# EthanD11/RS-VIO

Measured on AMD Instinct MI355X. Metric: stereo frames/sec (tracker+BA) on 752×480 EuRoC stream; BA ms/iter at window=10, higher is better.
Workload: dtype f32 (tracker) / f64 (BA)

## Files before the change

### rs-vio_amd/csrc/ba.hip

```cpp
#include <rccl/rccl.h>

#include <algorithm>
#include <chrono>
#include <cmath>
#include <cstdlib>
#include <cstring>
#include <string>
#include <sys/resource.h>
#include <numeric>
#include <stdexcept>
#include <vector>

#include "common.hpp"

#include "obs_pass.hpp"
#include "se3.hpp"
#include "wave.hpp"

#pragma clang fp contract(fast)

namespace rsvio {

namespace {

// ... 292 lines not shown
    __hip_atomic_store(w + 1, (b >> 32) | t, __ATOMIC_RELAXED, __HIP_MEMORY_SCOPE_SYSTEM);
}


__global__ void ba_reset(Geometry G, Work Wk, double lambda0) {
    const int i = blockIdx.x * blockDim.x + threadIdx.x;
    if (i < 7 * G.n_kf) {
        Wk.pose[0][i] = Wk.pose_init[i];
        Wk.pose[1][i] = Wk.pose_init[i];
    }
    if (i < 3 * G.n_lm) {
        Wk.pw[0][i] = Wk.pw_init[i];
        Wk.pw[1][i] = Wk.pw_init[i];
    }
    if (i == 0) {
        Wk.tick[1] = wall_clock64();
        *Wk.singular = 0;
        LmState s{};
        s.lambda = lambda0;
        s.nu = 2.0;
        *Wk.st = s;
    }
}

struct SlotLin {
    double V[6], gp[3], Wr[9], Ur[6], gr[3], cost;
};

__device__ __forceinline__ void slot_linearize(const Geometry& G, const Pose& P, const double p[3], int nobs,
                                               int cams, const double2 (&uvq)[2], bool fr, SlotLin& L) {
#pragma unroll
    for (int i = 0; i < 6; ++i) L.V[i] = 0.0;
#pragma unroll
    for (int i = 0; i < 3; ++i) L.gp[i] = 0.0;
#pragma unroll
    for (int i = 0; i < 9; ++i) L.Wr[i] = 0.0;
#pragma unroll
    for (int i = 0; i < 6; ++i) L.Ur[i] = 0.0;
#pragma unroll
    for (int i = 0; i < 3; ++i) L.gr[i] = 0.0;
    L.cost = 0.0;
#pragma unroll
    for (int o = 0; o < 2; ++o) {
        if (o >= nobs) break;
        double r[2], J[2][9];
        const double uv[2] = {uvq[o].x, uvq[o].y};
        linearize(p, P, G.TCB[(cams >> o) & 1].m, uv, r, J, true);
        double sq = r[0] * r[0] + r[1] * r[1], rho, wt;
        huber(sq, G.huber_delta, &rho, &wt);
        L.cost += 0.5 * rho;
        const double wr0 = wt * r[0], wr1 = wt * r[1];
        int k = 0;
#pragma unroll
        for (int a = 0; a < 3; ++a) {
#pragma unroll
            for (int c = a; c < 3; ++c) L.V[k++] += wt * (J[0][a] * J[0][c] + J[1][a] * J[1][c]);
            L.gp[a] += J[0][a] * wr0 + J[1][a] * wr1;
        }
        if (fr) {
            int u = 0;
#pragma unroll
            for (int a = 0; a < 3; ++a) {
#pragma unroll
                for (int c = 0; c < 3; ++c) L.Wr[a * 3 + c] += wt * (J[0][6 + a] * J[0][c] + J[1][6 + a] * J[1][c]);
#pragma unroll
                for (int c = a; c < 3; ++c) L.Ur[u++] += wt * (J[0][6 + a] * J[0][6 + c] + J[1][6 + a] * J[1][6 + c]);
                L.gr[a] += J[0][6 + a] * wr0 + J[1][6 + a] * wr1;
            }
        }
    }
}

__device__ __forceinline__ void wave_sync() {
    __builtin_amdgcn_fence(__ATOMIC_SEQ_CST, "wavefront");
    __builtin_amdgcn_wave_barrier();
}

template <bool WAVE = false>
__device__ void store_linearization(const Work& Wk, int buf, int s, int lane, bool act, bool fr, int first, int nk,
                                    int l, const SlotLin& L, double (*sh)[64]) {
    if (act && fr) {
        double rec[kRawF];
#pragma unroll
        for (int i = 0; i < 6; ++i) rec[RV + i] = L.V[i];
#pragma unroll
        for (int i = 0; i < 3; ++i) rec[RGP + i] = L.gp[i];
#pragma unroll
        for (int i = 0; i < 9; ++i) rec[RWR + i] = L.Wr[i];
#pragma unroll
        for (int i = 0; i < 6; ++i) rec[RUR + i] = L.Ur[i];
#pragma unroll
        for (int i = 0; i < 3; ++i) rec[RGR + i] = L.gr[i];
        rec[27] = 0.0;
        double2* dst = reinterpret_cast<double2*>(Wk.raws[buf] + (size_t)s * kRawF);
#pragma unroll
        for (int i = 0; i < kRawF / 2; ++i) dst[i] = make_double2(rec[2 * i], rec[2 * i + 1]);
    }
#pragma unroll
    for (int i = 0; i < 6; ++i) sh[i][lane] = L.V[i];
#pragma unroll
    for (int i = 0; i < 3; ++i) sh[6 + i][lane] = L.gp[i];
    if constexpr (WAVE) wave_sync(); else __syncthreads();
    if (act && lane == first) {
        double Vl[6] = {0, 0, 0, 0, 0, 0}, gl[3] = {0, 0, 0};
        for (int k = 0; k < nk; ++k) {
#pragma unroll
            for (int i = 0; i < 6; ++i) Vl[i] += sh[i][first + k];
#pragma unroll
            for (int i = 0; i < 3; ++i) gl[i] += sh[6 + i][first + k];
        }
        double rec[kLmF] = {Vl[0], Vl[1], Vl[2], Vl[3], Vl[4], Vl[5], gl[0], gl[1], gl[2], 0.0, 0.0, 0.0};
        double2* dst = reinterpret_cast<double2*>(Wk.rawl[buf] + (size_t)l * kLmF);
#pragma unroll
        for (int i = 0; i < kLmF / 2; ++i) dst[i] = make_double2(rec[2 * i], rec[2 * i + 1]);
    }
}

__device__ __forceinline__ bool chol_inv3(const double A[3][3], double X[3][3]) {
    const double d0 = A[0][0];
    if (!(d0 > 0.0) || !isfinite(d0)) return false;
    const double l00 = sqrt(d0), l10 = A[1][0] / l00, l20 = A[2][0] / l00;
    const double d1 = A[1][1] - l10 * l10;
    if (!(d1 > 0.0) || !isfinite(d1)) return false;
    const double l11 = sqrt(d1), l21 = (A[2][1] - l20 * l10) / l11;
    const double d2 = (A[2][2] - l20 * l20) - l21 * l21;
    if (!(d2 > 0.0) || !isfinite(d2)) return false;
    const double l22 = sqrt(d2);
    const double m00 = 1.0 / l00, m11 = 1.0 / l11, m22 = 1.0 / l22;
    const double m10 = -(l10 * m00) * m11, m21 = -(l21 * m11) * m22;
    const double m20 = -(l20 * m00 + l21 * m10) * m22;
    X[0][0] = (m00 * m00 + m10 * m10) + m20 * m20;
    X[0][1] = X[1][0] = m10 * m11 + m20 * m21;
    X[0][2] = X[2][0] = m20 * m22;
    X[1][1] = m11 * m11 + m21 * m21;
    X[1][2] = X[2][1] = m21 * m22;
    X[2][2] = m22 * m22;
    return true;
}

__device__ __forceinline__ bool landmark_inverse(const double* Vp, double lambda, double Vi[3][3], int chol) {
    double A[3][3] = {{Vp[0] + lambda, Vp[1], Vp[2]}, {Vp[1], Vp[3] + lambda, Vp[4]}, {Vp[2], Vp[4], Vp[5] + lambda}};
    const bool ok = chol ? chol_inv3(A, Vi) : inv3(A, Vi);
    if (!ok)
#pragma unroll
        for (int a = 0; a < 3; ++a)
#pragma unroll
            for (int c = 0; c < 3; ++c) Vi[a][c] = 0.0;
    return ok;
}

struct SlotSrc {
    const unsigned long long* mask;
    const int* lm_base;
    const int* wave_fill;
    const int* wave_lm;
    const unsigned* key;
    const double2* uv;
    int nb_lm, nb_pad;
    int uv32;
};
constexpr unsigned long long kEvenBits = 0x5555555555555555ull;

__device__ void build_slots_body(const Geometry& G, const Prob& Pr, const SlotSrc& S, int4* hdr, double2* huv,
                                 int b) {
    const int t = threadIdx.x;
    const double2 z2 = make_double2(0.0, 0.0);
    if (b < S.nb_lm) {
        const int l = 256 * b + t;
        if (l >= G.n_lm) return;
        const int base = S.lm_base[l];
        if (base < 0) return;
        const unsigned long long m = S.mask[l];
        unsigned long long kb = (m | (m >> 1)) & kEvenBits;
        const int ns = __popcll(kb);
        for (size_t ps = (size_t)base; kb; kb &= kb - 1, ++ps) {
            const int k = (__ffsll((long long)kb) - 1) >> 1;
            const int c0 = (int)(m >> (2 * k)) & 1, c1 = (int)(m >> (2 * k + 1)) & 1;
            const int no = c0 + c1;
            hdr[2 * ps] = make_int4(k, l, base & 63, ns);
            hdr[2 * ps + 1] = make_int4(Pr.free_idx[k], no, no == 2 ? 2 : c1, 0);
            if (no == 1) huv[2 * ps + 1] = z2;
        }
    } else if (b < S.nb_lm + S.nb_pad) {
        const int ps = 256 * (b - S.nb_lm) + t;
        if (ps >= 64 * G.n_wave || (ps & 63) < S.wave_fill[ps >> 6]) return;
        hdr[2 * (size_t)ps] = make_int4(0, 0, 0, 0);
        hdr[2 * (size_t)ps + 1] = make_int4(-1, 0, 0, 0);
        huv[2 * (size_t)ps] = z2;
        huv[2 * (size_t)ps + 1] = z2;
    } else {
        const int i = 256 * (b - S.nb_lm - S.nb_pad) + t;
        if (i >= G.n_obs) return;
        const unsigned key = S.key[i];
        const int l = (int)(key >> 6), k = (int)(key >> 1) & 31, c = (int)(key & 1);
        const unsigned long long m = S.mask[l];
        const unsigned long long below = ((m | (m >> 1)) & kEvenBits) & ((1ull << (2 * k)) - 1ull);
        const size_t q = (size_t)S.lm_base[l] + __popcll(below);
        const int sub = (c == 1 && ((m >> (2 * k)) & 1)) ? 1 : 0;
        if (S.uv32) {
            const float2 f = reinterpret_cast<const float2*>(S.uv)[i];
            huv[2 * q + sub] = make_double2((double)f.x, (double)f.y);
        } else {
            huv[2 * q + sub] = S.uv[i];
        }
    }
}

constexpr int kPairU = 8;

__device__ void build_pairs_body(const Geometry& G, const Prob& Pr, const SlotSrc& S, int4* pairs, int c) {
    __shared__ int cnt[4];
    const int pb = c / kGrp, x = c % kGrp;
    const int fa = Pr.pb_fa[pb], fb = Pr.pb_fb[pb];
    int kfa = 0, kfb = 0;
    for (int k = 0; k < G.n_kf; ++k) {
        const int f = Pr.free_idx[k];
        if (f == fa) kfa = k;
        if (f == fb) kfb = k;
    }
    const unsigned long long ma = 3ull << (2 * kfa), mb = 3ull << (2 * kfb);
    const unsigned long long below_a = (1ull << (2 * kfa)) - 1ull, below_b = (1ull << (2 * kfb)) - 1ull;
    const int tid = threadIdx.x, lane = tid & 63, wave = tid >> 6;
    const int nw = G.n_wave > x ? (G.n_wave - x + kGrp - 1) / kGrp : 0;
    const int k0 = nw * wave / 4, k1 = nw * (wave + 1) / 4;
    int4* out = pairs + (size_t)c * G.pair_stride;
    struct Round {
        int l0[kPairU], l1[kPairU], lbs[kPairU];
        unsigned long long m[kPairU];
    };
    auto load = [&](int kb, Round& R) {
#pragma unroll
        for (int u = 0; u < kPairU; ++u) {
            const int w = x + kGrp * (kb + u);
            const bool in = kb + u < k1;
            R.l0[u] = in ? S.wave_lm[w] : 0;
            R.l1[u] = in ? S.wave_lm[w + 1] : 0;
        }
#pragma unroll
        for (int u = 0; u < kPairU; ++u) {
            const bool in = R.l0[u] + lane < R.l1[u];
            R.m[u] = in ? S.mask[R.l0[u] + lane] : 0ull;
            R.lbs[u] = in ? S.lm_base[R.l0[u] + lane] : 0;
        }
    };
    auto scan = [&](const Round& R, bool write, int& acc) {
#pragma unroll
        for (int u = 0; u < kPairU; ++u) {
            for (int l = R.l0[u] + lane; l - lane < R.l1[u]; l += 64) {
                const bool first = l == R.l0[u] + lane;
                const unsigned long long mm = first ? R.m[u] : (l < R.l1[u] ? S.mask[l] : 0ull);
                const bool has = (mm & ma) && (mm & mb);
                const unsigned long long bal = __ballot(has);
                if (write && has) {
                    const unsigned long long kbits = (mm | (mm >> 1)) & kEvenBits;
                    const int lb = first ? R.lbs[u] : S.lm_base[l];
                    out[acc + __popcll(bal & ((1ull << lane) - 1ull))] =
                        make_int4(lb + __popcll(kbits & below_a), lb + __popcll(kbits & below_b), l, 0);
                }
                acc += __popcll(bal);
            }
        }
    };
    Round R0;
    load(k0, R0);
    int n = 0;
    scan(R0, false, n);
    for (int kb = k0 + kPairU; kb < k1; kb += kPairU) {
        Round R;
        load(kb, R);
        scan(R, false, n);
    }
    if (lane == 0) cnt[wave] = n;
    __syncthreads();
    int base = 0;
    for (int v = 0; v < wave; ++v) base += cnt[v];
    const int total = cnt[0] + cnt[1] + cnt[2] + cnt[3];
    scan(R0, true, base);
    for (int kb = k0 + kPairU; kb < k1; kb += kPairU) {
        Round R;
        load(kb, R);
        scan(R, true, base);
    }
    for (int i = total + tid; i < G.pair_stride; i += 256) out[i] = make_int4(-1, 0, 0, 0);
}

__global__ __launch_bounds__(256) void ba_stage_in(const uint4* src, uint4* __restrict__ dst, int n_words) {
    const int t = (int)(blockIdx.x * 256 + threadIdx.x), st = (int)(gridDim.x * 256);
    const int i0 = t, i1 = t + st;
    uint4 a, b;
    host_load2x16(src + min(i0, n_words - 1), src + min(i1, n_words - 1), a, b);
    if (i0 < n_words) dst[i0] = a;
    if (i1 < n_words) dst[i1] = b;
}

__global__ __launch_bounds__(256) void ba_build_layout(Geometry G, Prob Pr, SlotSrc S, int nb_slots, int4* hdr,
                                                       double2* huv, int4* pairs) {
    const int b = blockIdx.x;
    if (b < nb_slots)
        build_slots_body(G, Pr, S, hdr, huv, b);
    else
        build_pairs_body(G, Pr, S, pairs, b - nb_slots);
}

__device__ void linearize_body(const Geometry& G, const Prob& Pr, const Work& Wk, int w, int with_reset,
                               double lambda0) {
    __shared__ double sh[10][64];
    const int lane = threadIdx.x;
    const int s = 64 * w + lane;
    if (with_reset) {
        const int nt = G.n_wave * 64;
        for (int i = s; i < 7 * G.n_kf; i += nt) {
            Wk.pose[0][i] = Wk.pose_init[i];
            Wk.pose[1][i] = Wk.pose_init[i];
        }
        for (int i = s; i < 3 * G.n_lm; i += nt) {
            Wk.pw[0][i] = Wk.pw_init[i];
            Wk.pw[1][i] = Wk.pw_init[i];
        }
        if (s == 0) {
            Wk.tick[1] = wall_clock64();
            *Wk.singular = 0;
            LmState st{};
            st.lambda = lambda0;
            st.nu = 2.0;
            *Wk.st = st;
        }
    }
    const double* pose0 = with_reset ? Wk.pose_init : Wk.pose[0];
    const double* pw0 = with_reset ? Wk.pw_init : Wk.pw[0];
    const int4 h0 = Pr.slot_hdr[2 * s], h1 = Pr.slot_hdr[2 * s + 1];
    const double2 uvq[2] = {Pr.slot_uv[2 * s], Pr.slot_uv[2 * s + 1]};
    STAMP(11);
    const bool act = h1.y > 0;
    const int kf = h0.x, l = h0.y, first = act ? h0.z : lane, nk = act ? h0.w : 1;
    const bool fr = h1.x >= 0;
    SlotLin L;
    if (act) {
        const Pose P = pose_from7(pose0 + 7 * kf);
        const double* pwp = pw0 + 3 * l;
        const double p[3] = {pwp[0], pwp[1], pwp[2]};
        slot_linearize(G, P, p, h1.y, h1.z, uvq, fr, L);
    } else {
        const Pose P{};
        const double p[3] = {0.0, 0.0, 1.0};
        slot_linearize(G, P, p, 0, 0, uvq, false, L);
    }
    STAMP(12);
    store_linearization(Wk, 0, s, lane, act, fr, first, nk, l, L, sh);
    const double c = wave_sum_det(L.cost);
    if (lane == 0) {
        Wk.partA[w * kPartA] = c;
        Wk.partA[w * kPartA + 1] = 0.0;
    }
    STAMP(14);
}

__global__ __launch_bounds__(64) void ba_linearize(Geometry G, Prob Pr, Work Wk, double lambda0) {
    linearize_body(G, Pr, Wk, blockIdx.x, 1, lambda0);
}

__device__ void trial_scalars_wave(const Geometry& G, const Prob& Pr, const Work& Wk, const LmState& s,
                                   int include_poses, double out[4]) {
    const int lane = threadIdx.x & 63;
    constexpr int kU = 8;
    double4 pv[kU];
    const int wl = max(G.n_wave - 1, 0), el = 7 * G.n_kf - 1;
#pragma unroll
    for (int k = 0; k < kU; ++k)
        pv[k] = *reinterpret_cast<const double4*>(Wk.partD + (size_t)min(lane + 64 * k, wl) * kPartD);
    double p0[3], p1[3];
    int fi[3];
#pragma unroll
    for (int k = 0; k < 3; ++k) {
        const int e = min(lane + 64 * k, el);
        fi[k] = Pr.free_idx[e / 7];
        p0[k] = Wk.pose[0][e];
        p1[k] = Wk.pose[1][e];
    }
#pragma unroll
    for (int k = 0; k < kU; ++k)
        if (lane + 64 * k >= G.n_wave) pv[k] = make_double4(0.0, 0.0, 0.0, 0.0);
    bool fr[3];
#pragma unroll
    for (int k = 0; k < 3; ++k) fr[k] = include_poses && lane + 64 * k <= el && fi[k] >= 0;
    double acc[kPartD] = {0.0, 0.0, 0.0, 0.0};
#pragma unroll
    for (int k = 0; k < kU; ++k) {
        acc[0] += pv[k].x;
        acc[1] += pv[k].y;
        acc[2] += pv[k].z;
        acc[3] += pv[k].w;
    }
    for (int i = lane + 64 * kU; i < G.n_wave; i += 64) {
        const double4 v = *reinterpret_cast<const double4*>(Wk.partD + (size_t)i * kPartD);
        acc[0] += v.x;
        acc[1] += v.y;
        acc[2] += v.z;
        acc[3] += v.w;
    }
    double sq[2] = {0.0, 0.0};
#pragma unroll
    for (int k = 0; k < 3; ++k)
        if (fr[k]) {
            sq[0] += p0[k] * p0[k];
            sq[1] += p1[k] * p1[k];
        }
    if (!s.solve_ok)
#pragma unroll
        for (int k = 0; k < kPartD; ++k) acc[k] = 0.0;
    acc[3] += sq[s.cur];
#pragma unroll
    for (int k = 0; k < kPartD; ++k) out[k] = wave_sum_det(acc[k]);
}

__device__ void trial_scalars_p2p(const Geometry& G, const Prob& Pr, const Work& Wk, const LmState& s, const P2P& P,
                                  unsigned long long gen, int* err, double out[4]) {
    const int lane = threadIdx.x & 63, par = (int)(gen & 1);
    double* own = P.peer[P.rank];
    const int el = 7 * G.n_kf - 1;
    double p0[3], p1[3];
    int fi[3];
#pragma unroll
    for (int k = 0; k < 3; ++k) {
        const int e = min(lane + 64 * k, el);
        fi[k] = Pr.free_idx[e / 7];
        p0[k] = Wk.pose[0][e];
        p1[k] = Wk.pose[1][e];
    }
    double sq[2] = {0.0, 0.0};
#pragma unroll
    for (int k = 0; k < 3; ++k)
        if (lane + 64 * k <= el && fi[k] >= 0) {
            sq[0] += p0[k] * p0[k];
            sq[1] += p1[k] * p1[k];
        }
    for (int j = 0; j < 4; ++j) out[j] = 0.0;
    bool late = false;
    for (int r = 0; r < P.nranks; ++r) {
        const int nw = P.xnw[r];
        double acc[kPartD] = {0.0, 0.0, 0.0, 0.0};
        for (int w = lane; w < max(nw, 512); w += 64) {
            double4 v = make_double4(0.0, 0.0, 0.0, 0.0);
            if (w < nw) {
                const unsigned long long* f = p2p_tflag(own, par, r, w);
                long long spins = 0;
                while (__hip_atomic_load(f, __ATOMIC_RELAXED, __HIP_MEMORY_SCOPE_SYSTEM) < gen) {
                    __builtin_amdgcn_s_sleep(1);
                    if (++spins > (1ll << 25)) {
                        late = true;
                        break;
                    }
                }
                __builtin_amdgcn_fence(__ATOMIC_ACQUIRE, "");
                const double* q = p2p_tval(own, par, r, w);
                v.x = __hip_atomic_load(q, __ATOMIC_RELAXED, __HIP_MEMORY_SCOPE_SYSTEM);
                v.y = __hip_atomic_load(q + 1, __ATOMIC_RELAXED, __HIP_MEMORY_SCOPE_SYSTEM);
                v.z = __hip_atomic_load(q + 2, __ATOMIC_RELAXED, __HIP_MEMORY_SCOPE_SYSTEM);
                v.w = __hip_atomic_load(q + 3, __ATOMIC_RELAXED, __HIP_MEMORY_SCOPE_SYSTEM);
            }
            acc[0] += v.x;
            acc[1] += v.y;
            acc[2] += v.z;
            acc[3] += v.w;
        }
        if (r == 0) acc[3] += sq[s.cur];
#pragma unroll
        for (int k = 0; k < kPartD; ++k) out[k] += wave_sum_det(acc[k]);
    }
    if (late) atomicExch(err, 1);
}

__device__ void lm_update(LmState& s, double cost, const double tv[4], int max_iter, double cost_tol,
                          double param_tol) {
    if (s.iter == 0) s.initial_cost = cost;
    s.cost = cost;
    s.iter += 1;
    s.accepted = 0;
    if (!isfinite(cost)) {
        s.status = RSVIO_LM_NUMERICAL_FAILURE;
        s.done = 1;
    } else if (!s.solve_ok) {
        s.status = RSVIO_LM_LINEAR_SOLVE_FAILED;
        s.done = 1;
    } else {
        s.new_cost = tv[0];
        s.dp2 = tv[1];
        s.gpdp = tv[2];
        s.x2 = tv[3];
        const double dx2 = s.dc2 + s.dp2;
        const double dxn = sqrt(dx2), xn = sqrt(s.x2);
        if (dxn <= param_tol * (xn + param_tol)) {
            s.status = RSVIO_LM_PARAMETER_TOLERANCE;
            s.done = 1;
        } else {
            const double pred = 0.5 * (s.lambda * dx2 - (s.gcdc + s.gpdp));
            const double dcost = cost - s.new_cost;
            const double rho = dcost / pred;
            if (isfinite(s.new_cost) && fabs(dcost) <= cost_tol * cost) {
                s.status = RSVIO_LM_COST_TOLERANCE;
                s.done = 1;
            } else if (isfinite(s.new_cost) && rho > 0.0) {
                s.accepted = 1;
                s.cur = 1 - s.cur;
                const double f = 2.0 * rho - 1.0;
                s.lambda *= fmax(1.0 / 3.0, 1.0 - f * f * f);
                s.nu = 2.0;
                s.cost = s.new_cost;
            } else {
                s.lambda *= s.nu;
                s.nu *= 2.0;
                if (s.lambda > 1e32) {
                    s.status = RSVIO_LM_TRUST_REGION;
                    s.done = 1;
                }
            }
        }
    }
    if (!s.done && s.iter >= max_iter) {
        s.status = RSVIO_LM_MAX_ITERATIONS;
        s.done = 1;
    }
}

struct LmArgs {
    int max_iter;
    double cost_tol, param_tol;
};

__device__ LmState lm_decide(const Geometry& G, const Prob& Pr, const Work& Wk, const LmState* src, int pre_reduced,
                             const LmArgs& la, const P2P* PP = nullptr, const unsigned long long* xgen = nullptr,
                             int* err = nullptr) {
    LmState s = *src;
    double tv[4];
    if (pre_reduced == 4) {
        const int lane = threadIdx.x & 63, r = lane >> 2, i = lane & 3, nr = PP->nranks;
        const unsigned long long gen = *xgen;
        const unsigned g32 = (unsigned)gen;
        const unsigned long long* wv = p2p_ll(PP->peer[PP->rank], (int)(gen & 1), min(r, nr - 1)) + 2 * i;
        unsigned long long a = __hip_atomic_load(wv, __ATOMIC_RELAXED, __HIP_MEMORY_SCOPE_SYSTEM);
        unsigned long long b = __hip_atomic_load(wv + 1, __ATOMIC_RELAXED, __HIP_MEMORY_SCOPE_SYSTEM);
        for (int k = 0; k < 4; ++k) tv[k] = 0.0;
        if (s.pending && !s.done && s.solve_ok) {
            long long spins = 0;
            bool late = false;
            while (r < nr && !((unsigned)(a >> 32) == g32 && (unsigned)(b >> 32) == g32)) {
                if (++spins > (1ll << 25)) {
                    late = true;
                    break;
                }
                __builtin_amdgcn_s_sleep(1);
                a = __hip_atomic_load(wv, __ATOMIC_RELAXED, __HIP_MEMORY_SCOPE_SYSTEM);
                b = __hip_atomic_load(wv + 1, __ATOMIC_RELAXED, __HIP_MEMORY_SCOPE_SYSTEM);
            }
            if (late) atomicExch(err, 1);
            const double got = late ? 0.0 : __longlong_as_double((long long)((a & 0xffffffffull) | (b << 32)));
            for (int k = 0; k < 4; ++k) {
                double v = 0.0;
                for (int q = 0; q < nr; ++q) v += rl64(got, 4 * q + k);
                tv[k] = v;
            }
        }
    } else if (pre_reduced == 2) {
        const unsigned long long gen = *xgen;
        for (int k = 0; k < 4; ++k) tv[k] = 0.0;
        if (s.pending && !s.done && s.solve_ok) trial_scalars_p2p(G, Pr, Wk, s, *PP, gen, err, tv);
    } else if (pre_reduced) {
        for (int k = 0; k < 4; ++k) tv[k] = Wk.trial4[k];
    } else {
        trial_scalars_wave(G, Pr, Wk, s, 1, tv);
    }
    const double cost0 = Wk.sys[(size_t)G.n_pb * 36 + 12 * G.n_free];
    __asm__ volatile("" ::"v"(tv[0]), "v"(tv[1]), "v"(tv[2]), "v"(tv[3]), "v"(cost0));
    STAMP(29);
    if (s.pending && !s.done) {
        const double cost = s.iter == 0 ? cost0 : s.cost;
        lm_update(s, cost, tv, la.max_iter, la.cost_tol, la.param_tol);
        s.pending = 0;
    }
    return s;
}

__device__ __forceinline__ void slot_w(const double* rec, double W[18]) {
    const double* v = rec + RV;
    const double Vs[9] = {v[0], v[1], v[2], v[1], v[3], v[4], v[2], v[4], v[5]};
#pragma unroll
    for (int i = 0; i < 9; ++i) W[i] = Vs[i];
#pragma unroll
    for (int i = 0; i < 9; ++i) W[9 + i] = rec[RWR + i];
}

template <bool DIAG>
__device__ __forceinline__ void schur_pair(const Work& Wk, int cur, double lambda, int chol, int sa, int sb, int l,
                                           double (&acc)[kBlockF]) {
    const double2* ra = reinterpret_cast<const double2*>(Wk.raws[cur] + (size_t)sa * kRawF);
    const double2* rb = reinterpret_cast<const double2*>(Wk.raws[cur] + (size_t)sb * kRawF);
    const double2* rl = reinterpret_cast<const double2*>(Wk.rawl[cur] + (size_t)l * kLmF);
    constexpr int NA = DIAG ? kRawF / 2 : 9;
    double Ra[2 * NA], Rb[18], Lm[10];
#pragma unroll
    for (int i = 0; i < NA; ++i) {
        const double2 x = ra[i];
        Ra[2 * i] = x.x; Ra[2 * i + 1] = x.y;
    }
    if constexpr (!DIAG)
#pragma unroll
        for (int i = 0; i < 9; ++i) {
            const double2 y = rb[i];
            Rb[2 * i] = y.x; Rb[2 * i + 1] = y.y;
        }
#pragma unroll
    for (int i = 0; i < 5; ++i) {
        const double2 x = rl[i];
        Lm[2 * i] = x.x; Lm[2 * i + 1] = x.y;
    }
    double Wa[18], Wb[18];
    slot_w(Ra, Wa);
    if constexpr (DIAG) {
#pragma unroll
        for (int i = 0; i < 18; ++i) Wb[i] = Wa[i];
    } else {
        slot_w(Rb, Wb);
    }
    double Vi[3][3];
    if (!landmark_inverse(Lm + LV, lambda, Vi, chol)) *Wk.singular = 1;
    double Ya[18];
#pragma unroll
    for (int a = 0; a < 6; ++a)
#pragma unroll
        for (int k = 0; k < 3; ++k)
            Ya[a * 3 + k] = fma(Wa[a * 3 + 2], Vi[2][k], fma(Wa[a * 3 + 1], Vi[1][k], Wa[a * 3] * Vi[0][k]));
#pragma unroll
    for (int a = 0; a < 6; ++a)
#pragma unroll
        for (int k = 0; k < 6; ++k)
            acc[a * 6 + k] -= fma(Ya[a * 3 + 2], Wb[k * 3 + 2], fma(Ya[a * 3 + 1], Wb[k * 3 + 1], Ya[a * 3] * Wb[k * 3]));
    if constexpr (DIAG) {
        double U[36];
#pragma unroll
        for (int a = 0; a < 3; ++a)
#pragma unroll
            for (int c = 0; c < 3; ++c) {
                U[a * 6 + c] = Wa[a * 3 + c];
                U[(3 + a) * 6 + c] = Wa[(3 + a) * 3 + c];
                U[c * 6 + 3 + a] = Wa[(3 + a) * 3 + c];
            }
        const double* ur = Ra + RUR;
        const double Ur[9] = {ur[0], ur[1], ur[2], ur[1], ur[3], ur[4], ur[2], ur[4], ur[5]};
#pragma unroll
        for (int a = 0; a < 3; ++a)
#pragma unroll
            for (int c = 0; c < 3; ++c) U[(3 + a) * 6 + 3 + c] = Ur[a * 3 + c];
#pragma unroll
        for (int i = 0; i < 36; ++i) acc[i] += U[i];
#pragma unroll
        for (int a = 0; a < 6; ++a) {
            const double gca = a < 3 ? Ra[RGP + a] : Ra[RGR + a - 3];
            const double yg = fma(Ya[a * 3 + 2], Lm[LG + 2], fma(Ya[a * 3 + 1], Lm[LG + 1], Ya[a * 3] * Lm[LG]));
            acc[36 + a] += yg - gca;
            acc[42 + a] += gca;
        }
    }
}

template <bool DIAG>
__device__ __forceinline__ void schur_chunk_pairs(const Geometry& G, const Work& Wk, const LmState& s, const int4* pr,
                                                  int4 p1, int tid, double (&acc)[kBlockF]) {
    if (p1.x >= 0) schur_pair<DIAG>(Wk, s.cur, s.lambda, G.chol, p1.x, p1.y, p1.z, acc);
    for (int p = tid + kSchurThreads; p < G.pair_stride; p += kSchurThreads) {
        const int4 q = pr[p];
        if (q.x >= 0) schur_pair<DIAG>(Wk, s.cur, s.lambda, G.chol, q.x, q.y, q.z, acc);
    }
}

__device__ void schur_chunks_body(const Geometry& G, const Prob& Pr, const Work& Wk, const LmArgs& la,
                                  int pre_reduced, int c, const P2P* PP = nullptr,
                                  const unsigned long long* xgen = nullptr, int* err = nullptr) {
    __shared__ double red[kSchurThreads / 64][kBlockF];
    const int tid = threadIdx.x, lane = tid & 63, wave = tid >> 6;
    const int pb = c / kGrp, x = c % kGrp;
    RTSTAMP(0);
    STAMP(26);
    if (G.env_on) {
        int a = 0, r = pb;
        while (a < G.n_free && r >= G.n_free - a) {
            r -= G.n_free - a;
            ++a;
        }
        if (a < G.n_free && a + r > (int)G.env[a]) {
            if (tid < 36) Wk.cpart[(size_t)x * sys_len(G) + pb * 36 + tid] = 0.0;
            return;
        }
    }
    const int4* pr = Pr.pairs + (size_t)c * G.pair_stride;
    const int4 p1 = tid < G.pair_stride ? pr[tid] : make_int4(-1, 0, 0, 0);
    const int fa = Pr.pb_fa[pb];
    const bool diag = fa == Pr.pb_fb[pb];
    __shared__ LmState sd;
    STAMP(27);
    if (wave == 0) {
        const LmState d = lm_decide(G, Pr, Wk, Wk.st_prev, pre_reduced, la, PP, xgen, err);
        STAMP(28);
        if (lane == 0) {
            sd = d;
            if (c == 0) *Wk.st = d;
        }
    }
    __syncthreads();
    const LmState s = sd;
    if (s.done) return;
    STAMP(16);
    RTSTAMP(1);
    double acc[kBlockF];
#pragma unroll
    for (int i = 0; i < kBlockF; ++i) acc[i] = 0.0;
    if (diag)
        schur_chunk_pairs<true>(G, Wk, s, pr, p1, tid, acc);
    else
        schur_chunk_pairs<false>(G, Wk, s, pr, p1, tid, acc);
    STAMP(17);
    wave_reduce_scatter<3>(acc, lane);
    if ((lane & 3) == 0)
#pragma unroll
        for (int j = 0; j < 3; ++j) red[wave][3 * (lane >> 2) + j] = acc[j];
    __syncthreads();
    if (tid < (diag ? kBlockF : 36)) {
        double v = red[0][tid];
#pragma unroll
        for (int w = 1; w < kSchurThreads / 64; ++w) v += red[w][tid];
        const int SB0 = G.n_pb * 36, SG0 = SB0 + 6 * G.n_free;
        const int e = tid < 36 ? pb * 36 + tid : (tid < 42 ? SB0 + 6 * fa + tid - 36 : SG0 + 6 * fa + tid - 42);
        Wk.cpart[(size_t)x * sys_len(G) + e] = v;
    }
    STAMP(18);
    RTSTAMP(2);
}

__global__ __launch_bounds__(kSchurThreads) void ba_schur_chunks(Geometry G, Prob Pr, Work Wk, LmArgs la,
                                                                  int pre_reduced) {
    schur_chunks_body(G, Pr, Wk, la, pre_reduced, blockIdx.x);
}

__global__ __launch_bounds__(kSchurThreads) void ba_schur_chunks_p2p(Geometry G, Prob Pr, Work Wk, LmArgs la, P2P P,
                                                                      const unsigned long long* xgen, int* err,
                                                                      int mode) {
    schur_chunks_body(G, Pr, Wk, la, mode, blockIdx.x, &P, xgen, err);
}

template <int T>
__device__ void combine_system(const Geometry& G, const Prob& Pr, const Work& Wk, double* dst, double lambda,
                               bool add_lambda) {
    const int n_e = G.n_pb * 36 + 12 * G.n_free;
    const size_t L = sys_len(G);
    constexpr int kU = 16;
    const int lane = threadIdx.x;
    double pa[kU];
    int sing = 0;
    if (lane < 64) {
#pragma unroll
        for (int k = 0; k < kU; ++k) pa[k] = lane + 64 * k < G.n_wave ? Wk.partA[(lane + 64 * k) * kPartA] : 0.0;
        sing = *Wk.singular;
    }
    constexpr int kE = 8;
    for (int e0 = 0; e0 < n_e; e0 += T * kE) {
        double v[kE][kGrp];
#pragma unroll
        for (int i = 0; i < kE; ++i) {
            const int e = e0 + threadIdx.x + T * i;
#pragma unroll
            for (int x = 0; x < kGrp; ++x) v[i][x] = e < n_e ? Wk.cpart[(size_t)x * L + e] : 0.0;
        }
#pragma unroll
        for (int i = 0; i < kE; ++i) {
            const int e = e0 + threadIdx.x + T * i;
            if (e >= n_e) break;
            double a = v[i][0];
#pragma unroll
            for (int x = 1; x < kGrp; ++x) a += v[i][x];
            dst[e] = a;
        }
    }
    if (add_lambda) {
        __syncthreads();
        for (int t = threadIdx.x; t < 6 * G.n_free; t += T) {
            const int f = t / 6, k = t % 6;
            dst[(f * G.n_free - f * (f - 1) / 2) * 36 + 7 * k] += lambda;
        }
    }
    if (lane < 64) {
        double c = 0.0;
#pragma unroll
        for (int k = 0; k < kU; ++k) c += pa[k];
        for (int w = lane + 64 * kU; w < G.n_wave; w += 64) c += Wk.partA[w * kPartA];
        c = wave_sum_det(c);
        if (lane == 0) {
            dst[n_e] = c;
            dst[n_e + 1] = sing ? 1.0 : 0.0;
            Wk.sys[n_e] = c;
        }
    }
}

__global__ __launch_bounds__(256) void ba_schur_combine(Geometry G, Prob Pr, Work Wk, int lambda_owner) {
    const LmState* st = Wk.st;
    if (st->done) return;
    STAMP(19);
    combine_system<256>(G, Pr, Wk, Wk.sys, st->lambda, lambda_owner != 0);
    __syncthreads();
    if (threadIdx.x == 0) *Wk.singular = 0;
}

__global__ __launch_bounds__(256) void ba_schur_combine_wide(Geometry G, Prob Pr, Work Wk) {
    const LmState* st = Wk.st;
    if (st->done) return;
    const int n_e = G.n_pb * 36 + 12 * G.n_free;
    const size_t L = sys_len(G);
    const int e = blockIdx.x * 256 + threadIdx.x;
    constexpr int kU = 16;
    const int lane = threadIdx.x;
    double pa[kU];
    int sing = 0;
    if (blockIdx.x == 0 && lane < 64) {
#pragma unroll
        for (int k = 0; k < kU; ++k) pa[k] = lane + 64 * k < G.n_wave ? Wk.partA[(lane + 64 * k) * kPartA] : 0.0;
        sing = *Wk.singular;
    }
    const double lambda = st->lambda;
    if (e < n_e) {
        double v[kGrp];
#pragma unroll
        for (int x = 0; x < kGrp; ++x) v[x] = Wk.cpart[(size_t)x * L + e];
        double a = v[0];
#pragma unroll
        for (int x = 1; x < kGrp; ++x) a += v[x];
        const int pb = e / 36, k = e % 36;
        if (pb < G.n_pb && k % 7 == 0 && Pr.pb_fa[pb] == Pr.pb_fb[pb]) a += lambda;
        Wk.sys[e] = a;
    }
    if (blockIdx.x == 0 && lane < 64) {
        double c = 0.0;
#pragma unroll
        for (int k = 0; k < kU; ++k) c += pa[k];
        for (int w = lane + 64 * kU; w < G.n_wave; w += 64) c += Wk.partA[w * kPartA];
        c = wave_sum_det(c);
        if (lane == 0) {
            Wk.sys[n_e] = c;
            Wk.sys[n_e + 1] = sing ? 1.0 : 0.0;
        }
    }
}





constexpr int kLcLd = 65;

template <int NP, int CW, int WV, int K>
__device__ __forceinline__ void chol_pipe_step(double (&a)[CW], int lane, double* Lc, double* Uc, int* progress,
                                               int& seen, bool& bad, double inv, double (&uq)[CW], double lp) {
    constexpr int c0 = WV * CW;
    constexpr int c1 = (c0 + CW < NP) ? c0 + CW : NP;
    constexpr int KN = (K + 1 < c0) ? K + 2 : K + 1;
    if constexpr (K < c0) {
        if (seen < KN) {
            do {
                seen = __hip_atomic_load(progress, __ATOMIC_ACQUIRE, __HIP_MEMORY_SCOPE_WORKGROUP);
                if (seen >= KN) break;
                __builtin_amdgcn_s_sleep(1);
            } while (true);
        }
        const double lr = Lc[K * kLcLd + lane];
        const double* u = Uc + K * kLcLd;
        if constexpr (KN == K + 2) {
            const double lr2 = Lc[(K + 1) * kLcLd + lane];
            const double* u2 = Uc + (K + 1) * kLcLd;
            double v1[CW], v2[CW];
#pragma unroll
            for (int jj = 0; jj < CW; ++jj) {
                v1[jj] = u[c0 + jj];
                v2[jj] = u2[c0 + jj];
            }
#pragma unroll
            for (int jj = 0; jj < CW; ++jj)
                if (c0 + jj < NP) a[jj] = fma(-lr2, v2[jj], fma(-lr, v1[jj], a[jj]));
        } else {
#pragma unroll
            for (int jj = 0; jj < CW; ++jj)
                if (c0 + jj < NP) a[jj] = fma(-lr, u[c0 + jj], a[jj]);
        }
        if constexpr (KN == c0) {
            const double piv = rl64(a[0], c0);
            bad |= !(piv > 0.0) || !isfinite(piv);
            inv = rcp_f64(piv);
        }
    } else if constexpr (K < c1) {
        constexpr int j = K - c0;
#ifdef RSVIO_STAMPS
        if (K == c0 && lane == 0) g_dbg[28 + WV] = (unsigned long long)clock64();
#endif
        if constexpr (K > c0) {
            __asm__ volatile("" ::: "memory");
            __hip_atomic_store(progress, K, __ATOMIC_RELAXED, __HIP_MEMORY_SCOPE_WORKGROUP);
        }
        const double uk = a[j];
        const double l = uk * inv;
        a[j] = l;
        Lc[K * kLcLd + lane] = l;
        Uc[K * kLcLd + lane] = uk;
        double piv = 1.0;
        if constexpr (j + 1 < CW && K + 1 < NP) {
            a[j + 1] = fma(-l, rl64(uk, K + 1), a[j + 1]);
            piv = rl64(a[j + 1], K + 1);
        }
        if constexpr (j + 2 < CW && K + 2 < NP) a[j + 2] = fma(-l, rl64(uk, K + 2), a[j + 2]);
        if constexpr (j + 1 < CW && K + 1 < NP) {
            bad |= !(piv > 0.0) || !isfinite(piv);
            inv = rcp_f64(piv);
        }
        __builtin_amdgcn_sched_barrier(0);
        if constexpr (K > c0) {
#pragma unroll
            for (int jj = j + 2; jj < CW; ++jj)
                if (c0 + jj < NP) a[jj] = fma(-lp, uq[jj], a[jj]);
        }
        {
            const double* uK = Uc + K * kLcLd;
#pragma unroll
            for (int jj = j + 3; jj < CW; ++jj) uq[jj] = c0 + jj < NP ? uK[c0 + jj] : 0.0;
        }
        lp = l;
        if constexpr (K + 1 == c1) {
            __asm__ volatile("" ::: "memory");
            __hip_atomic_store(progress, K + 1, __ATOMIC_RELAXED, __HIP_MEMORY_SCOPE_WORKGROUP);
        }
    }
    if constexpr (K < c0) {
#pragma unroll
        for (int jj = 0; jj < CW; ++jj) __asm__ volatile("" : "+v"(a[jj]));
    }
    constexpr int KNEXT = (K < c0) ? KN : K + 1;
    if constexpr (KNEXT < c1) chol_pipe_step<NP, CW, WV, KNEXT>(a, lane, Lc, Uc, progress, seen, bad, inv, uq, lp);
}

template <int NF>
__device__ __forceinline__ const double* sys_lower(const double* sys, int r, int c) {
    constexpr int n = 6 * NF;
    if (r == n) return sys + (NF * (NF + 1) / 2) * 36 + c;
    const int a = c / 6, b = r / 6;
    const int pb = a * NF - a * (a - 1) / 2 + (b - a);
    const int k = (a == b) ? (r % 6) * 6 + (c % 6) : (c % 6) * 6 + (r % 6);
    return sys + pb * 36 + k;
}

template <int NP, int CW, int WV>
__device__ void chol_pipe(const double* sys, double* Lc, double* Uc, int* progress, int* badw, int lane) {
    constexpr int c0 = WV * CW;
    double a[CW];
#pragma unroll
    for (int jj = 0; jj < CW; ++jj) {
        const int c = c0 + jj;
        a[jj] = (c < NP && lane <= NP && (c <= lane || lane == NP)) ? *sys_lower<NP / 6>(sys, lane, c) : 0.0;
    }
    bool bad = false;
    if constexpr (c0 < NP) {
        double inv = 0.0;
        if constexpr (c0 == 0) {
            const double piv = rl64(a[0], 0);
            bad = !(piv > 0.0) || !isfinite(piv);
            inv = rcp_f64(piv);
        }
        int seen = 0;
        double uq[CW];
#pragma unroll
        for (int jj = 0; jj < CW; ++jj) uq[jj] = 0.0;
        chol_pipe_step<NP, CW, WV, 0>(a, lane, Lc, Uc, progress, seen, bad, inv, uq, 0.0);
    }
    if (lane == 0) badw[WV] = bad ? 1 : 0;
#ifdef RSVIO_STAMPS
    if (lane == 0) g_dbg[24 + WV] = (unsigned long long)clock64();
#endif
}

__device__ __forceinline__ void k5_result(LmState* st, int ok, double d2, double gd) {
    st->solve_ok = ok;
    st->dc2 = d2;
    st->gcdc = gd;
    st->pending = 1;
}

template <int NF>
__device__ void k5_finish(const Geometry& G, const Work& Wk, double* A, double x, double gcl_v, int n, int lane,
                          const double (&p7)[7], int fidx) {
    LmState* st = Wk.st;
    const double d2 = wave_sum_det(x * x);
    const double gd = wave_sum_det(lane < n ? gcl_v * x : 0.0);
    __builtin_amdgcn_wave_barrier();
    if (lane < n) {
        Wk.dc[lane] = x;
        A[lane] = x;
    }
    __builtin_amdgcn_s_waitcnt(0xc07f);
    __builtin_amdgcn_wave_barrier();
    STAMP(4);
    if (lane < G.n_kf) {
        double* q = Wk.pose[1 - st->cur] + 7 * lane;
        if (fidx < 0) {
#pragma unroll
            for (int i = 0; i < 7; ++i) q[i] = p7[i];
        } else {
            double qv[7];
            se3_plus(p7, A + 6 * fidx, qv);
#pragma unroll
            for (int i = 0; i < 7; ++i) q[i] = qv[i];
        }
    }
    STAMP(5);
    if (lane == 0) k5_result(st, 1, d2, gd);
    STAMP(6);
}

template <int NF>
__device__ void camera_solve_w4(const Geometry& G, const Prob& Pr, const Work& Wk, const double* sys, double* A,
                                int* badw, int* progress, int n, int tid, const double (&p7)[7], int fidx) {
    constexpr int NP = 6 * NF, CW = (NP + 3) / 4;
    const int lane = tid & 63, wave = tid >> 6;
    LmState* st = Wk.st;
    const double gcl_v = (wave == 0 && lane < n) ? sys[(NF * (NF + 1) / 2) * 36 + 6 * NF + lane] : 0.0;
    double* Lc = A + 128;
    double* Uc = Lc + NP * kLcLd;
    switch (wave) {
        case 0: chol_pipe<NP, CW, 0>(sys, Lc, Uc, progress, badw, lane); break;
        case 1: chol_pipe<NP, CW, 1>(sys, Lc, Uc, progress, badw, lane); break;
        case 2: chol_pipe<NP, CW, 2>(sys, Lc, Uc, progress, badw, lane); break;
        default: chol_pipe<NP, CW, 3>(sys, Lc, Uc, progress, badw, lane); break;
    }
    __syncthreads();
    if (wave != 0) return;
    if (badw[0] | badw[1] | badw[2] | badw[3]) {
        if (lane == 0) k5_result(st, 0, 0.0, 0.0);
        return;
    }
// ... 1057 lines not shown
    double x[2];
#pragma unroll
    for (int q = 0; q < 2; ++q) x[q] = lane + 64 * q < n ? yv[q] : 0.0;
    const double d2 = wave_sum_det(x[0] * x[0] + x[1] * x[1]);
    const double gd = wave_sum_det(gcl[0] * x[0] + gcl[1] * x[1]);
#pragma unroll
    for (int q = 0; q < 2; ++q) {
        const int i = lane + 64 * q;
        if (i < n) {
            Wk.dc[i] = x[q];
            dcs[i] = x[q];
        }
    }
    __builtin_amdgcn_s_waitcnt(0xc07f);
    __builtin_amdgcn_wave_barrier();
    if (lane < G.n_kf) {
        double* qd = Wk.pose[1 - cur] + 7 * lane;
        if (fidx < 0) {
#pragma unroll
            for (int i = 0; i < 7; ++i) qd[i] = p7[i];
        } else {
            double qv[7];
            se3_plus(p7, dcs + 6 * fidx, qv);
#pragma unroll
            for (int i = 0; i < 7; ++i) qd[i] = qv[i];
        }
    }
    if (lane == 0) k5_result(st, 1, d2, gd);
    STAMP(5);
}

template <int NF>
__global__ __launch_bounds__(64 * kBkWaves) void ba_camera_solve_blk(Geometry G, Prob Pr, Work Wk, int combine) {
    camera_solve_blk_body<NF>(G, Pr, Wk, combine);
}

constexpr int kX2Waves = 8;
constexpr int kUcLd = kMaxN + 1;

__device__ __forceinline__ const double* sys_lower_rt(const double* sys, int nf, int r, int c) {
    const int n = 6 * nf;
    if (r == n) return sys + (nf * (nf + 1) / 2) * 36 + c;
    const int a = c / 6, b = r / 6;
    const int pb = a * nf - a * (a - 1) / 2 + (b - a);
    const int k = (a == b) ? (r % 6) * 6 + (c % 6) : (c % 6) * 6 + (r % 6);
    return sys + pb * 36 + k;
}

template <int NP, int CW, int WV, int K>
__device__ __forceinline__ void chol2_step(double (&a)[2][CW], int lane, double* Uc, double* dinv, double* sink,
                                           int* progress, int& seen, bool& bad, double inv) {
    constexpr int c0 = WV * CW;
    constexpr int c1 = (c0 + CW < NP) ? c0 + CW : NP;
    constexpr int Q0 = (c0 < 64) ? 0 : 1;
    constexpr int KN = (K + 1 < c0) ? K + 2 : K + 1;
    if constexpr (K < c0) {
        if (seen < KN) {
            do {
                seen = __hip_atomic_load(progress, __ATOMIC_ACQUIRE, __HIP_MEMORY_SCOPE_WORKGROUP);
                if (seen >= KN) break;
                __builtin_amdgcn_s_sleep(1);
            } while (true);
        }
        const double* u = Uc + K * kUcLd;
        const double di = dinv[K];
        double lr[2];
#pragma unroll
        for (int q = Q0; q < 2; ++q) lr[q] = u[min(lane + 64 * q, NP)] * di;
        if constexpr (KN == K + 2) {
            const double* u2 = Uc + (K + 1) * kUcLd;
            const double di2 = dinv[K + 1];
            double lr2[2];
#pragma unroll
            for (int q = Q0; q < 2; ++q) lr2[q] = u2[min(lane + 64 * q, NP)] * di2;
            double v1[CW], v2[CW];
#pragma unroll
            for (int jj = 0; jj < CW; ++jj) {
                v1[jj] = u[c0 + jj];
                v2[jj] = u2[c0 + jj];
            }
#pragma unroll
            for (int q = Q0; q < 2; ++q)
#pragma unroll
                for (int jj = 0; jj < CW; ++jj)
                    if (c0 + jj < NP) a[q][jj] = fma(-lr2[q], v2[jj], fma(-lr[q], v1[jj], a[q][jj]));
        } else {
#pragma unroll
            for (int q = Q0; q < 2; ++q)
#pragma unroll
                for (int jj = 0; jj < CW; ++jj)
                    if (c0 + jj < NP) a[q][jj] = fma(-lr[q], u[c0 + jj], a[q][jj]);
        }
        if constexpr (KN == c0) {
            const double piv = rl64(a[c0 >> 6][0], c0 & 63);
            bad |= !(piv > 0.0) || !isfinite(piv);
            inv = rcp_f64(piv);
        }
    } else if constexpr (K < c1) {
        constexpr int j = K - c0;
        if constexpr (K > c0) __hip_atomic_store(progress, K, __ATOMIC_RELEASE, __HIP_MEMORY_SCOPE_WORKGROUP);
        double uk[2], l[2];
#pragma unroll
        for (int q = Q0; q < 2; ++q) {
            uk[q] = a[q][j];
            l[q] = uk[q] * inv;
            a[q][j] = l[q];
            double* dst = (q == 0 || lane + 64 <= NP) ? Uc + K * kUcLd + lane + 64 * q : sink + lane;
            *dst = uk[q];
        }
        dinv[K] = inv;
        double piv = 1.0;
        if constexpr (j + 1 < CW && K + 1 < NP) {
            constexpr int qn = (K + 1) >> 6, ln = (K + 1) & 63;
            const double ukn = rl64(uk[qn], ln);
#pragma unroll
            for (int q = Q0; q < 2; ++q) a[q][j + 1] = fma(-l[q], ukn, a[q][j + 1]);
            piv = rl64(a[qn][j + 1], ln);
        }
#pragma unroll
        for (int jj = j + 2; jj < CW; ++jj) {
            if (c0 + jj < NP) {
                const double v = rl64(uk[(c0 + jj) >> 6], (c0 + jj) & 63);
#pragma unroll
                for (int q = Q0; q < 2; ++q) a[q][jj] = fma(-l[q], v, a[q][jj]);
            }
        }
        if constexpr (j + 1 < CW && K + 1 < NP) {
            bad |= !(piv > 0.0) || !isfinite(piv);
            inv = rcp_f64(piv);
        }
        if constexpr (K + 1 == c1) __hip_atomic_store(progress, K + 1, __ATOMIC_RELEASE, __HIP_MEMORY_SCOPE_WORKGROUP);
    }
    if constexpr (K < c0) {
#pragma unroll
        for (int q = Q0; q < 2; ++q)
#pragma unroll
            for (int jj = 0; jj < CW; ++jj) __asm__ volatile("" : "+v"(a[q][jj]));
    }
    constexpr int KNEXT = (K < c0) ? KN : K + 1;
    if constexpr (KNEXT < c1) chol2_step<NP, CW, WV, KNEXT>(a, lane, Uc, dinv, sink, progress, seen, bad, inv);
}

template <int NP, int CW, int WV>
__device__ __forceinline__ void chol2_pipe(const double* sys, int nf, double* Uc, double* dinv, double* sink, int* progress,
                                           int* badw, int lane) {
    constexpr int c0 = WV * CW;
    constexpr int Q0 = (c0 < 64) ? 0 : 1;
    const int n = 6 * nf;
    double a[2][CW];
#pragma unroll
    for (int q = 0; q < 2; ++q) {
        const int r = lane + 64 * q;
#pragma unroll
        for (int jj = 0; jj < CW; ++jj) {
            const int c = c0 + jj;
            double v = 0.0;
            if (q >= Q0 && c < NP && r <= NP && (c <= r || r == NP)) {
                if (r == NP) v = c < n ? *sys_lower_rt(sys, nf, n, c) : 0.0;
                else if (r < n) v = *sys_lower_rt(sys, nf, r, c);
                else v = (r == c) ? 1.0 : 0.0;
            }
            a[q][jj] = v;
        }
    }
    bool bad = false;
    if constexpr (c0 < NP) {
        double inv = 0.0;
        if constexpr (c0 == 0) {
            const double piv = rl64(a[0][0], 0);
            bad = !(piv > 0.0) || !isfinite(piv);
            inv = rcp_f64(piv);
        }
        int seen = 0;
        chol2_step<NP, CW, WV, 0>(a, lane, Uc, dinv, sink + 64 * WV, progress, seen, bad, inv);
    }
    if (lane == 0) badw[WV] = bad ? 1 : 0;
}

template <int NF>
__global__ __launch_bounds__(64 * kX2Waves) void ba_camera_solve_x2(Geometry G, Prob Pr, Work Wk, int combine) {
    constexpr int NP = 6 * NF, CW = (NP + kX2Waves - 1) / kX2Waves;
    static_assert(NP <= kMaxN && NP + 1 <= kUcLd && NP < 128, "padded system too large");
    __shared__ double Uc[NP * kUcLd];
    __shared__ double dinv[NP];
    __shared__ double dcs[128];
    __shared__ double sink[64 * kX2Waves];
    __shared__ int badw[kX2Waves];
    __shared__ int progress;
    __shared__ int fail;
    LmState* st = Wk.st;
    if (st->done) return;
    const int tid = threadIdx.x, lane = tid & 63, wave = tid >> 6;
    const int nF = G.n_free, n = 6 * nF;
    const double* sys = Wk.sys;
    const int SG0 = G.n_pb * 36 + 6 * nF, SC0 = SG0 + 6 * nF;
    const int cur = st->cur;
    double p7[7] = {0, 0, 0, 1, 0, 0, 0};
    int fidx = -1;
    double gcl[2] = {0.0, 0.0};
    if (wave == 0 && lane < G.n_kf) {
        fidx = Pr.free_idx[lane];
#pragma unroll
        for (int i = 0; i < 7; ++i) p7[i] = Wk.pose[cur][7 * lane + i];
    }
    if (combine) {
        combine_system<64 * kX2Waves>(G, Pr, Wk, Wk.sys, st->lambda, true);
        __builtin_amdgcn_s_waitcnt(0);
        __syncthreads();
    }
    if (wave == 0)
#pragma unroll
        for (int q = 0; q < 2; ++q)
            if (lane + 64 * q < n) gcl[q] = sys[SG0 + lane + 64 * q];
    if (tid == 0) {
        fail = (sys[SC0 + 1] != 0.0 || *Wk.singular) ? 1 : 0;
        *Wk.singular = 0;
        progress = 0;
    }
    __syncthreads();
    if (fail) {
        if (tid == 0) k5_result(st, 0, 0.0, 0.0);
        return;
    }
    switch (wave) {
        case 0: chol2_pipe<NP, CW, 0>(sys, nF, Uc, dinv, sink, &progress, badw, lane); break;
        case 1: chol2_pipe<NP, CW, 1>(sys, nF, Uc, dinv, sink, &progress, badw, lane); break;
        case 2: chol2_pipe<NP, CW, 2>(sys, nF, Uc, dinv, sink, &progress, badw, lane); break;
        case 3: chol2_pipe<NP, CW, 3>(sys, nF, Uc, dinv, sink, &progress, badw, lane); break;
        case 4: chol2_pipe<NP, CW, 4>(sys, nF, Uc, dinv, sink, &progress, badw, lane); break;
        case 5: chol2_pipe<NP, CW, 5>(sys, nF, Uc, dinv, sink, &progress, badw, lane); break;
        case 6: chol2_pipe<NP, CW, 6>(sys, nF, Uc, dinv, sink, &progress, badw, lane); break;
        default: chol2_pipe<NP, CW, 7>(sys, nF, Uc, dinv, sink, &progress, badw, lane); break;
    }
    __syncthreads();
    if (wave != 0) return;
    bool anybad = false;
#pragma unroll
    for (int w = 0; w < kX2Waves; ++w) anybad |= badw[w] != 0;
    if (anybad) {
        if (lane == 0) k5_result(st, 0, 0.0, 0.0);
        return;
    }
    double yv[2], di[2];
#pragma unroll
    for (int q = 0; q < 2; ++q) {
        const int i = min(lane + 64 * q, NP - 1);
        di[q] = dinv[i];
        yv[q] = Uc[i * kUcLd + NP] * di[q];
    }
    constexpr int kBs = 8;
    for (int j0 = n - 1; j0 >= 0; j0 -= kBs) {
        double lt[kBs][2];
#pragma unroll
        for (int t = 0; t < kBs; ++t) {
            const int j = max(j0 - t, 0);
#pragma unroll
            for (int q = 0; q < 2; ++q) lt[t][q] = Uc[min(lane + 64 * q, NP - 1) * kUcLd + j];
        }
#pragma unroll
        for (int t = 0; t < kBs; ++t) {
            const int j = j0 - t;
            if (j < 0) break;
            const double xj = j >= 64 ? rl64(yv[1], j - 64) : rl64(yv[0], j);
#pragma unroll
            for (int q = 0; q < 2; ++q) {
                const double l = lt[t][q] * di[q];
                const double upd = fma(-l, xj, yv[q]);
                yv[q] = lane + 64 * q < j ? upd : yv[q];
            }
        }
    }
    STAMP(4);
    double x[2];
#pragma unroll
    for (int q = 0; q < 2; ++q) x[q] = lane + 64 * q < n ? yv[q] : 0.0;
    const double d2 = wave_sum_det(x[0] * x[0] + x[1] * x[1]);
    const double gd = wave_sum_det(gcl[0] * x[0] + gcl[1] * x[1]);
#pragma unroll
    for (int q = 0; q < 2; ++q) {
        const int i = lane + 64 * q;
        if (i < n) {
            Wk.dc[i] = x[q];
            dcs[i] = x[q];
        }
    }
    __builtin_amdgcn_s_waitcnt(0xc07f);
    __builtin_amdgcn_wave_barrier();
    if (lane < G.n_kf) {
        double* qd = Wk.pose[1 - st->cur] + 7 * lane;
        if (fidx < 0) {
#pragma unroll
            for (int i = 0; i < 7; ++i) qd[i] = p7[i];
        } else {
            double qv[7];
            se3_plus(p7, dcs + 6 * fidx, qv);
#pragma unroll
            for (int i = 0; i < 7; ++i) qd[i] = qv[i];
        }
    }
    if (lane == 0) k5_result(st, 1, d2, gd);
    STAMP(5);
}

template <bool FUSED>
__device__ void k6_body(const Geometry& G, const Prob& Pr, const Work& Wk, int w, int lane, double (*sh)[64],
                        double (*shp)[64], double (*shs)[64], const P2P* PP = nullptr,
                        unsigned long long gen = 0, unsigned long long* k6tag = nullptr,
                        unsigned long long* k6part = nullptr) {
    const int s = 64 * w + lane;
    const int4 h0 = Pr.slot_hdr[2 * s], h1 = Pr.slot_hdr[2 * s + 1];
    const double2 uvq[2] = {Pr.slot_uv[2 * s], Pr.slot_uv[2 * s + 1]};
    const LmState* st = Wk.st;
    const bool act = h1.y > 0;
    const int kf = h0.x, l = h0.y, first = act ? h0.z : lane, nk = act ? h0.w : 1;
    const bool fr = h1.x >= 0;
    const int kfc = act ? kf : 0, lc = act ? l : 0, fc = (act && fr) ? h1.x : 0;
    double recb[2][18], Lmb[2][10], pcb[2][3], p7b[2][7], d6[6];
#pragma unroll
    for (int b = 0; b < 2; ++b) {
        const double2* wr = reinterpret_cast<const double2*>(Wk.raws[b] + (size_t)s * kRawF);
#pragma unroll
        for (int i = 0; i < 9; ++i) {
            const double2 x = wr[i];
            recb[b][2 * i] = x.x; recb[b][2 * i + 1] = x.y;
        }
        const double2* lr = reinterpret_cast<const double2*>(Wk.rawl[b] + (size_t)lc * kLmF);
#pragma unroll
        for (int i = 0; i < 5; ++i) {
            const double2 x = lr[i];
            Lmb[b][2 * i] = x.x; Lmb[b][2 * i + 1] = x.y;
        }
#pragma unroll
        for (int i = 0; i < 3; ++i) pcb[b][i] = Wk.pw[b][3 * lc + i];
#pragma unroll
        for (int i = 0; i < 7; ++i) p7b[b][i] = Wk.pose[b][7 * kfc + i];
    }
#pragma unroll
    for (int i = 0; i < 6; ++i) d6[i] = Wk.dc[6 * fc + i];
    const int done = st->done, solve_ok = st->solve_ok, cur = st->cur;
    const double lambda = st->lambda;
#pragma unroll
    for (int b = 0; b < 2; ++b) {
#pragma unroll
        for (int i = 0; i < 18; ++i) __asm__ volatile("" ::"v"(recb[b][i]));
#pragma unroll
        for (int i = 0; i < 10; ++i) __asm__ volatile("" ::"v"(Lmb[b][i]));
#pragma unroll
        for (int i = 0; i < 3; ++i) __asm__ volatile("" ::"v"(pcb[b][i]));
#pragma unroll
        for (int i = 0; i < 7; ++i) __asm__ volatile("" ::"v"(p7b[b][i]));
    }
    if (done || !solve_ok) return;
    STAMP(20);
    RTSTAMP(7);
    double Wv[18], Lm[10], pc[3], p7[7];
    {
        double rec[18];
#pragma unroll
        for (int i = 0; i < 18; ++i) rec[i] = cur ? recb[1][i] : recb[0][i];
        slot_w(rec, Wv);
#pragma unroll
        for (int i = 0; i < 10; ++i) Lm[i] = cur ? Lmb[1][i] : Lmb[0][i];
#pragma unroll
        for (int i = 0; i < 3; ++i) pc[i] = cur ? pcb[1][i] : pcb[0][i];
#pragma unroll
        for (int i = 0; i < 7; ++i) p7[i] = cur ? p7b[0][i] : p7b[1][i];
    }
    double t3[3] = {0.0, 0.0, 0.0};
    if (act && fr) {
#pragma unroll
        for (int c = 0; c < 3; ++c) {
            double acc = 0.0;
#pragma unroll
            for (int a = 0; a < 6; ++a) acc += Wv[a * 3 + c] * d6[a];
            t3[c] = acc;
        }
    }
#pragma unroll
    for (int c = 0; c < 3; ++c) sh[c][lane] = t3[c];
#pragma unroll
    for (int i = 0; i < 4; ++i) shs[i][lane] = 0.0;
    if constexpr (FUSED) wave_sync(); else __syncthreads();
    STAMP(22);
    if (act && lane == first) {
        double Vi[3][3];
        landmark_inverse(Lm + LV, lambda, Vi, G.chol);
        double rhs[3] = {-Lm[LG], -Lm[LG + 1], -Lm[LG + 2]};
        for (int k = 0; k < nk; ++k)
#pragma unroll
            for (int c = 0; c < 3; ++c) rhs[c] -= sh[c][first + k];
        double* pt = Wk.pw[1 - cur] + 3 * l;
        double dp2 = 0.0, gpdp = 0.0, p2 = 0.0;
#pragma unroll
        for (int c = 0; c < 3; ++c) {
            const double dp = (Vi[c][0] * rhs[0] + Vi[c][1] * rhs[1]) + Vi[c][2] * rhs[2];
            const double p = pc[c];
            const double q = p + dp;
            shp[c][lane] = q;
            pt[c] = q;
            dp2 += dp * dp;
            gpdp += Lm[LG + c] * dp;
            p2 += p * p;
        }
        shs[1][lane] = dp2;
        shs[2][lane] = gpdp;
        shs[3][lane] = p2;
    }
    if constexpr (FUSED) wave_sync(); else __syncthreads();
    STAMP(23);
    SlotLin L;
    if (act) {
        const Pose P = pose_from7(p7);
        const double q[3] = {shp[0][first], shp[1][first], shp[2][first]};
        slot_linearize(G, P, q, h1.y, h1.z, uvq, fr, L);
    } else {
        const Pose P{};
        const double q[3] = {0.0, 0.0, 1.0};
        slot_linearize(G, P, q, 0, 0, uvq, false, L);
    }
    shs[0][lane] = L.cost;
    if constexpr (FUSED) wave_sync(); else __syncthreads();
    STAMP(24);
    store_linearization<FUSED>(Wk, 1 - cur, s, lane, act, fr, first, nk, l, L, sh);
    STAMP(25);
    {
        double v[kPartD];
#pragma unroll
        for (int i = 0; i < kPartD; ++i) v[i] = wave_sum_det(shs[i][lane]);
        if (lane == 0)
#pragma unroll
            for (int i = 0; i < kPartD; ++i) Wk.partD[w * kPartD + i] = v[i];
        if (k6tag && lane < kPartD) {
            double vl = v[0];
#pragma unroll
            for (int i = 1; i < kPartD; ++i) vl = lane == i ? v[i] : vl;
            const unsigned long long b = (unsigned long long)__double_as_longlong(vl), t = gen << 32;
            const size_t nw = (size_t)G.n_wave;
            __hip_atomic_store(k6tag + (2 * lane) * nw + w, (b & 0xffffffffull) | t, __ATOMIC_RELAXED,
                               __HIP_MEMORY_SCOPE_AGENT);
            __hip_atomic_store(k6tag + (2 * lane + 1) * nw + w, (b >> 32) | t, __ATOMIC_RELAXED,
                               __HIP_MEMORY_SCOPE_AGENT);
        }
        if (k6part && lane < kPartD) {
            double vl = v[0];
#pragma unroll
            for (int i = 1; i < kPartD; ++i) vl = lane == i ? v[i] : vl;
            __hip_atomic_store(k6part + (size_t)w * kPartD + lane, (unsigned long long)__double_as_longlong(vl),
                               __ATOMIC_RELAXED, __HIP_MEMORY_SCOPE_AGENT);
        }
        if (PP && lane < PP->nranks) {
            const int par = (int)(gen & 1);
            double* q = p2p_tval(PP->peer[lane], par, PP->rank, w);
            q[0] = v[0]; q[1] = v[1]; q[2] = v[2]; q[3] = v[3];
            __threadfence_system();
            __hip_atomic_store(p2p_tflag(PP->peer[lane], par, PP->rank, w), gen, __ATOMIC_RELEASE,
                               __HIP_MEMORY_SCOPE_SYSTEM);
        }
    }
    STAMP(21);
    RTSTAMP(8);
}

__global__ __launch_bounds__(64) void ba_backsub_relinearize(Geometry G, Prob Pr, Work Wk) {
    __shared__ double sh[10][64];
    __shared__ double shp[3][64];
    __shared__ double shs[4][64];
    RTSTAMP(6);
    k6_body<false>(G, Pr, Wk, blockIdx.x, threadIdx.x, sh, shp, shs);
    RTSTAMP(9);
}

__global__ __launch_bounds__(64) void ba_backsub_relinearize_p2p(Geometry G, Prob Pr, Work Wk, P2P P,
                                                                 const unsigned long long* xgen) {
    __shared__ double sh[10][64];
    __shared__ double shp[3][64];
    __shared__ double shs[4][64];
    unsigned long long gen = *xgen;
    __asm__ volatile("" : "+s"(gen));
    k6_body<false>(G, Pr, Wk, blockIdx.x, threadIdx.x, sh, shp, shs, &P, gen);
}

template <int KU>
__device__ void k6_reduce_p2p(const Geometry& G, const Prob& Pr, const Work& Wk, const P2P& P,
                              unsigned long long* xgen, int* err, const unsigned long long* k6tag) {
    const int lane = threadIdx.x & 63;
    const LmState s = *Wk.st;
    const unsigned long long gen = *xgen + 1;
    if (s.done) return;
    const unsigned g32 = (unsigned)gen;
    const int nr = P.nranks, me = P.rank, par = (int)(gen & 1);
    const int el = 7 * G.n_kf - 1;
    double p0[3], p1[3];
    int fi[3];
#pragma unroll
    for (int k = 0; k < 3; ++k) {
        const int e = min(lane + 64 * k, el);
        fi[k] = Pr.free_idx[e / 7];
        p0[k] = Wk.pose[0][e];
        p1[k] = Wk.pose[1][e];
    }
    constexpr int kU = KU;
    double acc[kPartD] = {0.0, 0.0, 0.0, 0.0};
    bool late = false;
    if (s.solve_ok) {
        for (int i0 = 0; i0 < max(G.n_wave, 64 * kU); i0 += 64 * kU) {
            unsigned long long wd[kU][kPartD][2];
            unsigned pend = 0;
#pragma unroll
            for (int k = 0; k < kU; ++k)
                if (i0 + lane + 64 * k < G.n_wave) pend |= 1u << k;
            long long spins = 0;
            const size_t nw = (size_t)G.n_wave;
            for (;;) {
#pragma unroll
                for (int k = 0; k < kU; ++k)
                    if (pend & (1u << k)) {
                        const unsigned long long* a = k6tag + (i0 + lane + 64 * k);
#pragma unroll
                        for (int j = 0; j < kPartD; ++j) {
                            wd[k][j][0] = __hip_atomic_load(a + (2 * j) * nw, __ATOMIC_RELAXED, __HIP_MEMORY_SCOPE_AGENT);
                            wd[k][j][1] = __hip_atomic_load(a + (2 * j + 1) * nw, __ATOMIC_RELAXED, __HIP_MEMORY_SCOPE_AGENT);
                        }
                    }
#pragma unroll
                for (int k = 0; k < kU; ++k)
                    if (pend & (1u << k)) {
                        bool ok = true;
#pragma unroll
                        for (int j = 0; j < kPartD; ++j)
                            ok &= (unsigned)(wd[k][j][0] >> 32) == g32 && (unsigned)(wd[k][j][1] >> 32) == g32;
                        if (ok) pend &= ~(1u << k);
                    }
                if (__all(pend == 0)) break;
                if (++spins > (1ll << 25)) {
                    late = true;
                    break;
                }
                __builtin_amdgcn_s_sleep(1);
            }
#pragma unroll
            for (int k = 0; k < kU; ++k)
                if (i0 + lane + 64 * k < G.n_wave)
#pragma unroll
                    for (int j = 0; j < kPartD; ++j)
                        acc[j] += __longlong_as_double((long long)((wd[k][j][0] & 0xffffffffull) | (wd[k][j][1] << 32)));
        }
    }
    double sq[2] = {0.0, 0.0};
#pragma unroll
    for (int k = 0; k < 3; ++k)
        if (me == 0 && lane + 64 * k <= el && fi[k] >= 0) {
            sq[0] += p0[k] * p0[k];
            sq[1] += p1[k] * p1[k];
        }
    acc[3] += sq[s.cur];
    double out[kPartD];
#pragma unroll
    for (int k = 0; k < kPartD; ++k) out[k] = wave_sum_det(acc[k]);
    const int r = lane >> 2, i = lane & 3;
    double mv = out[0];
#pragma unroll
    for (int k = 1; k < kPartD; ++k) mv = i == k ? out[k] : mv;
    double got = mv;
    if (r < nr && r != me) {
        ll_put(p2p_ll(P.peer[r], par, me) + 2 * i, mv, g32);
        const unsigned long long* w = p2p_ll(P.peer[me], par, r) + 2 * i;
        long long spins = 0;
        for (;;) {
            const unsigned long long a = __hip_atomic_load(w, __ATOMIC_RELAXED, __HIP_MEMORY_SCOPE_SYSTEM);
            const unsigned long long b = __hip_atomic_load(w + 1, __ATOMIC_RELAXED, __HIP_MEMORY_SCOPE_SYSTEM);
            if ((unsigned)(a >> 32) == g32 && (unsigned)(b >> 32) == g32) {
                got = __longlong_as_double((long long)((a & 0xffffffffull) | (b << 32)));
                break;
            }
            if (++spins > (1ll << 25)) {
                late = true;
                got = 0.0;
                break;
            }
            __builtin_amdgcn_s_sleep(1);
        }
    }
    if (late) atomicExch(err, 1);
    double v4[kPartD];
#pragma unroll
    for (int k = 0; k < kPartD; ++k) {
        double v = 0.0;
        for (int q = 0; q < nr; ++q) v += rl64(got, 4 * q + k);
        v4[k] = v;
    }
    if (lane == 0) {
#pragma unroll
        for (int k = 0; k < kPartD; ++k) Wk.trial4[k] = v4[k];
        *xgen = gen;
    }
}

__global__ __launch_bounds__(64) void ba_backsub_relinearize_p2p3(Geometry G, Prob Pr, Work Wk, P2P P,
                                                                  unsigned long long* xgen, int* err,
                                                                  unsigned long long* k6tag) {
    __shared__ double sh[10][64];
    __shared__ double shp[3][64];
    __shared__ double shs[4][64];
    if ((int)blockIdx.x == G.n_wave) {
        if (G.n_wave <= 256)
            k6_reduce_p2p<4>(G, Pr, Wk, P, xgen, err, k6tag);
        else
            k6_reduce_p2p<8>(G, Pr, Wk, P, xgen, err, k6tag);
        return;
    }
    unsigned long long gen = *xgen + 1;
    __asm__ volatile("" : "+s"(gen));
    k6_body<false>(G, Pr, Wk, blockIdx.x, threadIdx.x, sh, shp, shs, nullptr, gen, k6tag);
}

__device__ void k6_last_push(const Geometry& G, const Prob& Pr, const Work& Wk, const P2P& P,
                             unsigned long long* xgen, unsigned long long gen, const unsigned long long* k6part,
                             const LmState& s) {
    const int lane = threadIdx.x & 63;
    constexpr int kU = 8;
    const int wl = max(G.n_wave - 1, 0), el = 7 * G.n_kf - 1;
    unsigned long long pw[kU][kPartD];
#pragma unroll
    for (int k = 0; k < kU; ++k)
#pragma unroll
        for (int j = 0; j < kPartD; ++j)
            pw[k][j] = __hip_atomic_load(k6part + (size_t)min(lane + 64 * k, wl) * kPartD + j, __ATOMIC_RELAXED,
                                         __HIP_MEMORY_SCOPE_AGENT);
    double p0[3], p1[3];
    int fi[3];
#pragma unroll
    for (int k = 0; k < 3; ++k) {
        const int e = min(lane + 64 * k, el);
        fi[k] = Pr.free_idx[e / 7];
        p0[k] = Wk.pose[0][e];
        p1[k] = Wk.pose[1][e];
    }
    double acc[kPartD] = {0.0, 0.0, 0.0, 0.0};
#pragma unroll
    for (int k = 0; k < kU; ++k)
#pragma unroll
        for (int j = 0; j < kPartD; ++j)
            acc[j] += lane + 64 * k < G.n_wave ? __longlong_as_double((long long)pw[k][j]) : 0.0;
    for (int i = lane + 64 * kU; i < G.n_wave; i += 64)
#pragma unroll
        for (int j = 0; j < kPartD; ++j)
            acc[j] += __longlong_as_double((long long)__hip_atomic_load(k6part + (size_t)i * kPartD + j, __ATOMIC_RELAXED,
                                                                        __HIP_MEMORY_SCOPE_AGENT));
    double sq[2] = {0.0, 0.0};
#pragma unroll
    for (int k = 0; k < 3; ++k)
        if (P.rank == 0 && lane + 64 * k <= el && fi[k] >= 0) {
            sq[0] += p0[k] * p0[k];
            sq[1] += p1[k] * p1[k];
        }
    acc[3] += sq[s.cur];
    double out[kPartD];
#pragma unroll
    for (int k = 0; k < kPartD; ++k) out[k] = wave_sum_det(acc[k]);
    const int r = lane >> 2, i = lane & 3, par = (int)(gen & 1);
    double mv = out[0];
#pragma unroll
    for (int k = 1; k < kPartD; ++k) mv = i == k ? out[k] : mv;
    if (r < P.nranks) ll_put(p2p_ll(P.peer[r], par, P.rank) + 2 * i, mv, (unsigned)gen);
    if (lane == 0) *xgen = gen;
}

__global__ __launch_bounds__(64) void ba_backsub_relinearize_p2p4(Geometry G, Prob Pr, Work Wk, P2P P,
                                                                  unsigned long long* xgen, unsigned* k6cnt,
                                                                  unsigned long long* k6part) {
    __shared__ double sh[10][64];
    __shared__ double shp[3][64];
    __shared__ double shs[4][64];
    unsigned long long gen = *xgen + 1;
    __asm__ volatile("" : "+s"(gen));
    if (G.n_wave > 0) {
        k6_body<false>(G, Pr, Wk, blockIdx.x, threadIdx.x, sh, shp, shs, nullptr, gen, nullptr, k6part);
        const LmState s = *Wk.st;
        if (s.done || !s.solve_ok) return;
        __builtin_amdgcn_s_waitcnt(kWaitStores);
        __builtin_amdgcn_fence(__ATOMIC_RELEASE, "agent");
        unsigned t = 0;
        if (threadIdx.x == 0) t = __hip_atomic_fetch_add(k6cnt, 1u, __ATOMIC_ACQ_REL, __HIP_MEMORY_SCOPE_AGENT);
        t = __builtin_amdgcn_readfirstlane(t);
        if (t != (unsigned)G.n_wave - 1) return;
        __builtin_amdgcn_fence(__ATOMIC_ACQUIRE, "agent");
        if (threadIdx.x == 0) __hip_atomic_store(k6cnt, 0u, __ATOMIC_RELAXED, __HIP_MEMORY_SCOPE_AGENT);
        k6_last_push(G, Pr, Wk, P, xgen, gen, k6part, s);
    } else {
        const LmState s = *Wk.st;
        if (s.done || !s.solve_ok) return;
        k6_last_push(G, Pr, Wk, P, xgen, gen, k6part, s);
    }
}

__global__ __launch_bounds__(64) void ba_reduce_trial(Geometry G, Prob Pr, Work Wk, int include_poses) {
    const LmState s = *Wk.st;
    if (s.done) return;
    double v[4];
    trial_scalars_wave(G, Pr, Wk, s, include_poses, v);
    if (threadIdx.x == 0)
        for (int k = 0; k < 4; ++k) Wk.trial4[k] = v[k];
}

constexpr int kK7Threads = 256;
#ifndef RSVIO_K7_BLOCKS
#define RSVIO_K7_BLOCKS 16
#endif
constexpr int kK7Blocks = RSVIO_K7_BLOCKS;
__device__ __forceinline__ void lm_decide_body(const Geometry& G, const Prob& Pr, const Work& Wk, int pre_reduced,
                                               const LmArgs& la, LmState* host, unsigned long long* htick,
                                               double* hout, const P2P* PP = nullptr,
                                               const unsigned long long* xgen = nullptr, int* err = nullptr) {
    STAMP(8);
    __shared__ LmState sd;
    if (threadIdx.x < 64) {
        const LmState d = lm_decide(G, Pr, Wk, Wk.st_prev, pre_reduced, la, PP, xgen, err);
        if (threadIdx.x == 0) {
            sd = d;
            if (blockIdx.x == 0) {
                LmState h = d;
                h.p2p_err = Wk.p2p_err ? *Wk.p2p_err : 0;
                *Wk.st = d;
                *host = h;
            }
        }
    }
    __syncthreads();
    const LmState s = sd;
    if (hout && s.done) {
        const double* pose = Wk.pose[s.cur];
        const double* pw = Wk.pw[s.cur];
        const int np = 7 * G.n_kf, n = np + 3 * G.n_lm;
        const int per = (((n + (int)gridDim.x - 1) / (int)gridDim.x) + 1) & ~1;
        const int i0 = (int)blockIdx.x * per, i1 = min(n, i0 + per);
        for (int i = i0 + 2 * (int)threadIdx.x; i < i1; i += 2 * kK7Threads) {
            const double a = i < np ? pose[i] : pw[i - np];
            if (i + 1 < i1) {
                const double b = i + 1 < np ? pose[i + 1] : pw[i + 1 - np];
                *reinterpret_cast<double2*>(hout + i) = make_double2(a, b);
            } else {
                hout[i] = a;
            }
        }
        __threadfence_system();
        __syncthreads();
        if (threadIdx.x == 0)
            __hip_atomic_store(htick + 4 + blockIdx.x, Wk.tick[1], __ATOMIC_RELEASE, __HIP_MEMORY_SCOPE_SYSTEM);
    }
    if (blockIdx.x == 0 && threadIdx.x == 0) {
        const unsigned long long t = Wk.tick[0] + 1;
        Wk.tick[0] = t;
        htick[1] = Wk.tick[1];
        htick[2] = wall_clock64();
        __threadfence_system();
        __hip_atomic_store(htick, t, __ATOMIC_RELEASE, __HIP_MEMORY_SCOPE_SYSTEM);
    }
    STAMP(10);
}

__global__ __launch_bounds__(kK7Threads) void ba_lm_decide(Geometry G, Prob Pr, Work Wk, int pre_reduced, LmArgs la,
                                                           LmState* host, unsigned long long* htick, double* hout) {
    lm_decide_body(G, Pr, Wk, pre_reduced, la, host, htick, hout);
}

__global__ __launch_bounds__(kK7Threads) void ba_lm_decide_p2p(Geometry G, Prob Pr, Work Wk, LmArgs la, LmState* host,
                                                               unsigned long long* htick, double* hout, P2P P,
                                                               const unsigned long long* xgen, int* err, int mode) {
    lm_decide_body(G, Pr, Wk, mode, la, host, htick, hout, &P, xgen, err);
}

struct WinDesc {
    Geometry G;
    Prob Pr;
    Work W[4];
    int skip;
};

__device__ __forceinline__ void desc_touch1(const void* p) { __asm__ volatile("" ::"s"(p)); }
template <class... T>
__device__ __forceinline__ void desc_touch(const T*... p) {
    (desc_touch1(p), ...);
}


__global__ __launch_bounds__(64) void bab_linearize(const WinDesc* __restrict__ D, double lambda0) {
    const WinDesc& d = D[blockIdx.y];
    const int skip = d.skip, bound = d.G.n_wave;
    const Prob Pr = d.Pr;
    const Work& Wk = d.W[2];
    desc_touch(Pr.slot_hdr, Pr.slot_uv, Wk.pose_init, Wk.pw_init, Wk.st);
    if (skip | ((int)blockIdx.x >= bound)) return;
    linearize_body(d.G, Pr, Wk, blockIdx.x, 1, lambda0);
}

__global__ __launch_bounds__(kSchurThreads) void bab_schur_chunks(const WinDesc* __restrict__ D, int wi, LmArgs la) {
    const WinDesc& d = D[blockIdx.y];
    const int skip = d.skip, bound = d.G.n_chunk;
    const Prob Pr = d.Pr;
    const Work& Wk = d.W[wi];
    desc_touch(Pr.pairs, Wk.partD, Wk.pose[0], Wk.pose[1], Wk.st_prev, Wk.st);
    if (skip | ((int)blockIdx.x >= bound)) return;
    schur_chunks_body(d.G, Pr, Wk, la, 0, blockIdx.x);
}

template <int NF>
__global__ __launch_bounds__(kK5Threads) void bab_camera_solve(const WinDesc* __restrict__ D, int wi) {
    const WinDesc& d = D[blockIdx.x];
    const int skip = d.skip, nkf = d.G.n_kf, nf = d.G.n_free, npb = d.G.n_pb, nw = d.G.n_wave;
    const Prob Pr = d.Pr;
    const Work& Wk = d.W[wi];
    desc_touch(Pr.free_idx, Pr.dmap, Wk.pose[0], Wk.pose[1], Wk.cpart, Wk.partA, Wk.singular, Wk.st);
    __asm__ volatile("" ::"s"(nkf), "s"(nf), "s"(npb), "s"(nw));
    if (skip) return;
    camera_solve_mfma_body<NF>(d.G, Pr, Wk, 1);
}

template <int NF>
__global__ __launch_bounds__(64 * kBkWaves) void bab_camera_solve_blk(const WinDesc* __restrict__ D, int wi) {
    const WinDesc& d = D[blockIdx.x];
    const int skip = d.skip;
    const Prob Pr = d.Pr;
    const Work& Wk = d.W[wi];
    desc_touch(Pr.free_idx, Pr.dmap, Wk.pose[0], Wk.pose[1], Wk.cpart, Wk.partA, Wk.singular, Wk.st);
    if (skip) return;
    camera_solve_blk_body<NF>(d.G, Pr, Wk, 1);
}

__global__ __launch_bounds__(64) void bab_backsub_relinearize(const WinDesc* __restrict__ D, int wi) {
    const WinDesc& d = D[blockIdx.y];
    const int skip = d.skip, bound = d.G.n_wave;
    const Prob Pr = d.Pr;
    const Work& Wk = d.W[wi];
    desc_touch(Pr.slot_hdr, Pr.slot_uv, Wk.st, Wk.raws[0], Wk.raws[1], Wk.rawl[0], Wk.rawl[1], Wk.pw[0], Wk.pw[1],
               Wk.pose[0], Wk.pose[1], Wk.dc);
    if (skip | ((int)blockIdx.x >= bound)) return;
    __shared__ double sh[10][64];
    __shared__ double shp[3][64];
    __shared__ double shs[4][64];
    k6_body<false>(d.G, Pr, Wk, blockIdx.x, threadIdx.x, sh, shp, shs);
}

__global__ __launch_bounds__(kK7Threads) void bad_lm_decide(const WinDesc* __restrict__ D, int wi, LmArgs la,
                                                            LmState* host, unsigned long long* htick, double* hout) {
    const WinDesc& d = D[0];
    const Prob Pr = d.Pr;
    const Work& Wk = d.W[wi];
    lm_decide_body(d.G, Pr, Wk, 0, la, host, htick, hout);
}

__global__ __launch_bounds__(64) void bab_lm_decide(const WinDesc* __restrict__ D, int wi, LmArgs la, LmState* host) {
    const WinDesc& d = D[blockIdx.x];
    if (d.skip) return;
    const LmState s = lm_decide(d.G, d.Pr, d.W[wi], d.W[wi].st, 0, la);
    if (threadIdx.x == 0) {
        *d.W[wi].st = s;
        host[blockIdx.x] = s;
    }
}


__device__ void p2p_exchange(const double* msg, int n, const P2P& P, unsigned long long* xgen, int* err, double* out,
                             unsigned long long gen_pre = 0) {
    __shared__ unsigned long long sgen;
    const int tid = threadIdx.x, nr = P.nranks, me = P.rank;
    if (!gen_pre) {
        if (tid == 0) sgen = *xgen + 1;
        __syncthreads();
    }
    const unsigned long long gen = gen_pre ? gen_pre : sgen;
    const int par = (int)(gen & 1);
    if (n <= kP2PLLMax) {
        const unsigned g32 = (unsigned)gen;
        const int r = tid / kP2PLLMax, i = tid % kP2PLLMax;
        if (r < nr && i < n) ll_put(p2p_ll(P.peer[r], par, me) + 2 * i, msg[i], g32);
        __shared__ double got[kP2PMax][kP2PLLMax];
        if (r < nr && i < n) {
            const unsigned long long* w = p2p_ll(P.peer[me], par, r) + 2 * i;
            long long spins = 0;
            for (;;) {
                const unsigned long long a = __hip_atomic_load(w, __ATOMIC_RELAXED, __HIP_MEMORY_SCOPE_SYSTEM);
                const unsigned long long b = __hip_atomic_load(w + 1, __ATOMIC_RELAXED, __HIP_MEMORY_SCOPE_SYSTEM);
                if ((unsigned)(a >> 32) == g32 && (unsigned)(b >> 32) == g32) {
                    got[r][i] = __longlong_as_double((long long)((a & 0xffffffffull) | (b << 32)));
                    break;
                }
                if (++spins > (1ll << 25)) {
                    atomicExch(err, 1);
                    got[r][i] = 0.0;
                    break;
                }
                __builtin_amdgcn_s_sleep(1);
            }
        }
        __syncthreads();
        if (tid < n) {
            double v = 0.0;
            for (int q = 0; q < nr; ++q) v += got[q][tid];
            out[tid] = v;
        }
        if (tid == 0) *xgen = gen;
        return;
    }
    for (int r = 0; r < nr; ++r) {
        double* dst = P.peer[r] + (size_t)(par * kP2PMax + me) * kP2PMsg;
        for (int i = tid; i < n; i += 256) dst[i] = msg[i];
    }
    __threadfence_system();
    __syncthreads();
    if (tid < nr)
        __hip_atomic_store(p2p_flags(P.peer[tid]) + par * kP2PMax + me, gen, __ATOMIC_RELEASE,
                           __HIP_MEMORY_SCOPE_SYSTEM);
    if (tid < nr) {
        const unsigned long long* f = p2p_flags(P.peer[me]) + par * kP2PMax + tid;
        long long spins = 0;
        while (__hip_atomic_load(f, __ATOMIC_RELAXED, __HIP_MEMORY_SCOPE_SYSTEM) < gen) {
            __builtin_amdgcn_s_sleep(2);
            if (++spins > (1ll << 25)) {
                atomicExch(err, 1);
                break;
            }
        }
        __builtin_amdgcn_fence(__ATOMIC_ACQUIRE, "");
    }
    __syncthreads();
    const double* mine = P.peer[me] + (size_t)(par * kP2PMax) * kP2PMsg;
    for (int i0 = tid; i0 < n; i0 += 4 * 256) {
        double v[4][kP2PMax];
#pragma unroll
        for (int q = 0; q < 4; ++q)
#pragma unroll
            for (int r = 0; r < kP2PMax; ++r)
                v[q][r] = __hip_atomic_load(mine + (size_t)min(r, nr - 1) * kP2PMsg + min(i0 + 256 * q, n - 1),
                                            __ATOMIC_RELAXED, __HIP_MEMORY_SCOPE_SYSTEM);
#pragma unroll
        for (int q = 0; q < 4; ++q) {
            double a = 0.0;
#pragma unroll
            for (int r = 0; r < kP2PMax; ++r)
                if (r < nr) a += v[q][r];
            if (i0 + 256 * q < n) out[i0 + 256 * q] = a;
        }
    }
    if (tid == 0) *xgen = gen;
}

__global__ __launch_bounds__(256) void ba_p2p_allreduce(double* buf, int n, P2P P, unsigned long long* xgen,
                                                        int* err) {
    p2p_exchange(buf, n, P, xgen, err, buf);
}

__global__ __launch_bounds__(256) void ba_p2p_sys(Geometry G, Prob Pr, Work Wk, P2P P, unsigned long long* xgen,
                                                  int* err) {
    __shared__ double msg[kP2PMsg];
    const LmState* st = Wk.st;
    if (st->done) return;
    combine_system<256>(G, Pr, Wk, msg, st->lambda, P.rank == 0);
    __syncthreads();
    if (threadIdx.x == 0) *Wk.singular = 0;
    p2p_exchange(msg, (int)sys_len(G), P, xgen, err, Wk.sys);
}

__global__ __launch_bounds__(256) void ba_p2p_trial(Geometry G, Prob Pr, Work Wk, P2P P, unsigned long long* xgen,
                                                    int* err) {
    __shared__ double msg[4];
    const unsigned long long gen = *xgen + 1;
    const LmState s = *Wk.st;
    if (s.done) return;
    if (threadIdx.x < 64) {
        double v[4];
        trial_scalars_wave(G, Pr, Wk, s, P.rank == 0 ? 1 : 0, v);
        if (threadIdx.x == 0)
            for (int k = 0; k < 4; ++k) msg[k] = v[k];
    }
    __syncthreads();
    p2p_exchange(msg, 4, P, xgen, err, Wk.trial4, gen);
}

}

RSVIO_DBG_READER(rsvio_dbg_ba_stamps)
RSVIO_RT_READER(rsvio_dbg_ba_rt)

using rsvio_obs::observation_pass;

__attribute__((target("popcnt"))) static inline int slot_count(unsigned long long m) {
    return __builtin_popcountll((m | (m >> 1)) & kEvenBits);
}

struct BundleAdjuster {
    rsvio_ba_params P{};
    hipStream_t stream = nullptr;
    bool own_stream = true;
    hipEvent_t ev0 = nullptr, ev1 = nullptr;
    Geometry G{};
    bool has_problem = false;
    int iter_chunk = 2;
    struct GraphSlot {
        hipGraphExec_t exec = nullptr;
        int k = -1;
        rsvio_lm_cfg cfg{};
        bool exp = false, stale = false;
        int nf = -1, coll = -1, wcap = 0, chunk = -1;
        const void* dptr = nullptr;
        hipEvent_t ev_launch = nullptr;
    };
    GraphSlot gv, gd;
    int solves_of_problem = 0;
    bool graphs_ok = true;
    int k5_variant = 2;
    std::vector<hipGraphExec_t> retired;
    void drop_slot(GraphSlot& sl) {
        if (sl.exec) {
            if (!settled) {
                if (hipStreamQuery(stream) == hipSuccess)
                    settled = true;
                else
                    (void)hipGetLastError();
            }
            if (settled) {
                destroy_retired();
                (void)hipGraphExecDestroy(sl.exec);
            } else {
                retired.push_back(sl.exec);
                if (retired.size() > 4) settle();
            }
        }
        sl.exec = nullptr;
        sl.k = -1;
        sl.stale = false;
    }
    void drop_graph() {
        drop_slot(gv);
        drop_slot(gd);
    }
    void destroy_retired() {
        for (hipGraphExec_t g : retired) (void)hipGraphExecDestroy(g);
        retired.clear();
    }
    static bool same_cfg(const rsvio_lm_cfg& a, const rsvio_lm_cfg& b) {
        return a.max_iterations == b.max_iterations && a.cost_tolerance == b.cost_tolerance &&
               a.parameter_tolerance == b.parameter_tolerance && a.huber_delta == b.huber_delta &&
               a.lambda_init == b.lambda_init && a.linear_solver == b.linear_solver;
    }
    bool graph_update = true;
    bool desc_on = true;
    WinDesc hdesc{};
    double desc_huber = std::nan("");
    int desc_chol = -1;
    HostBuf<WinDesc> h_desc1;
    hipEvent_t ev_desc = nullptr;
    bool desc_pending = false;
    bool desc_mode() const { return desc_on && coll == 0 && k5_variant == 2 && G.n_free <= 10 && G.n_wave > 0; }
    int fold_lvl = 3;
    int fold_req = 3;
    bool p2p_shared_gpu = false;
    bool p2p_fold() const { return fold_lvl >= 1 && coll == 2 && k5_variant == 2 && G.n_free <= 10; }
    bool p2p_fold2() const { return fold_lvl == 2 && p2p_fold(); }
    bool p2p_fold3() const { return fold_lvl == 3 && p2p_fold() && k6_fits(); }
    int k6_cap = 0;
    bool k6_fits() const { return G.n_wave + 1 <= k6_cap; }
    int p2p_share = 1;
    bool p2p_fold4() const { return fold_lvl == 4 && p2p_fold(); }
    const WinDesc* dptr() const { return reinterpret_cast<const WinDesc*>(d_arena.p + lay.desc); }
    void fill_desc(WinDesc& d) const {
        d = WinDesc{};
        d.G = G;
        d.G.huber_delta = desc_huber;
        d.G.chol = desc_chol;
        d.Pr = prob();
        d.W[0] = work(0);
        d.W[1] = work(1);
        d.W[2] = work_at(0);
        d.W[3] = work_at(1);
        d.skip = 0;
    }
    void refresh_desc() {
        if (desc_pending && hipEventQuery(ev_desc) != hipSuccess) {
            (void)hipGetLastError();
            RSVIO_HIP(hipEventSynchronize(ev_desc));
        }
        desc_pending = false;
        desc_huber = G.huber_delta;
        desc_chol = G.chol;
        hdesc.G.huber_delta = desc_huber;
        hdesc.G.chol = desc_chol;
        if (!h_desc1.p) h_desc1.alloc(1);
        *h_desc1.p = hdesc;
        settled = false;
        RSVIO_HIP(hipMemcpyAsync(d_arena.p + lay.desc, h_desc1.p, sizeof(WinDesc), hipMemcpyHostToDevice, stream));
        RSVIO_HIP(hipEventRecord(ev_desc, stream));
        desc_pending = true;
    }
    bool start_graph(const rsvio_lm_cfg& cfg, int& k) {
        if (coll == 1 || !graphs_ok) return false;
        const bool dm = desc_mode() && solves_of_problem == 0;
        ++solves_of_problem;
        GraphSlot& sl = dm ? gd : gv;
        if (dm && (G.huber_delta != desc_huber || G.chol != desc_chol)) refresh_desc();
        const int wcap = (G.n_wave + G.n_wave / 4 + kGrp - 1) / kGrp * kGrp;
        const bool k_ok = sl.k == k || (dm && sl.k > k && sl.k <= k + 2);
        const bool topo = sl.exec && k_ok && same_cfg(sl.cfg, cfg) && sl.exp == export_on && sl.nf == G.n_free &&
                          sl.coll == coll;
        const bool hit = topo && (dm ? (sl.dptr == dptr() && sl.chunk == G.n_chunk && G.n_wave <= sl.wcap &&
                                        2 * G.n_wave > sl.wcap)
                                     : !sl.stale);
        if (hit) k = sl.k;
        if (!hit) {
            const auto tg0 = std::chrono::steady_clock::now();
            bool try_update = topo && sl.k == k && graph_update;
            if (try_update && hipEventQuery(sl.ev_launch) != hipSuccess) {
                (void)hipGetLastError();
                try_update = false;
            }
            if (!try_update) drop_slot(sl);
            if (hipStreamBeginCapture(stream, hipStreamCaptureModeThreadLocal) != hipSuccess) {
                (void)hipGetLastError();
                graphs_ok = false;
                return false;
            }
            bool ok = true;
            try {
                if (dm) {
                    enqueue_start_d(cfg.lambda_init, wcap);
                    for (int i = 0; i < k; ++i) enqueue_iteration_d(cfg, i, wcap);
                    enqueue_decide_d(cfg, k);
                } else {
                    enqueue_start(cfg.lambda_init);
                    for (int i = 0; i < k; ++i) enqueue_iteration(cfg, i);
                    enqueue_decide(cfg, k);
                }
            } catch (...) {
                ok = false;
            }
            hipGraph_t g = nullptr;
            if (hipStreamEndCapture(stream, &g) != hipSuccess) ok = false;
            const auto tg1 = std::chrono::steady_clock::now();
            bool updated = false;
            if (ok && try_update) {
                hipGraphNode_t err_node = nullptr;
                hipGraphExecUpdateResult r = hipGraphExecUpdateError;
                updated = hipGraphExecUpdate(sl.exec, g, &err_node, &r) == hipSuccess && r == hipGraphExecUpdateSuccess;
                if (!updated) {
                    (void)hipGetLastError();
                    drop_slot(sl);
                }
            }
            if (ok && !updated && hipGraphInstantiate(&sl.exec, g, nullptr, nullptr, 0) != hipSuccess) {
                sl.exec = nullptr;
                ok = false;
            }
            const auto tg2 = std::chrono::steady_clock::now();
            if (g) (void)hipGraphDestroy(g);
            if (prof_env)
                fprintf(stderr, "[rsvio] graph us (%s): drop+capture %.1f %s %.1f destroy %.1f\n", dm ? "desc" : "value",
                        std::chrono::duration<double, std::micro>(tg1 - tg0).count(),
                        updated ? "update" : "instantiate",
                        std::chrono::duration<double, std::micro>(tg2 - tg1).count(),
                        std::chrono::duration<double, std::micro>(std::chrono::steady_clock::now() - tg2).count());
            if (!ok) {
                (void)hipGetLastError();
                graphs_ok = false;
                return false;
            }
            sl.k = k;
            sl.cfg = cfg;
            sl.exp = export_on;
            sl.nf = G.n_free;
            sl.coll = coll;
            sl.stale = false;
            sl.wcap = wcap;
            sl.chunk = G.n_chunk;
            sl.dptr = dm ? static_cast<const void*>(dptr()) : nullptr;
        }
        settled = false;
        RSVIO_HIP(hipGraphLaunch(sl.exec, stream));
        if (graph_update) RSVIO_HIP(hipEventRecord(sl.ev_launch, stream));
        return true;
    }
    int last_iterations = 3;
    DevBuf<double> d_pose2, d_pw2;
    DevBuf<uint8_t> d_arena;
    HostBuf<uint8_t> h_arena;
    bool up_pending = false;
    struct ArenaLayout {
        size_t desc, pose_init, pw_init, free_idx, pb_fa, pb_fb, dmap, mask, lm_base, wave_fill, wave_lm, key, ouv, upload;
        size_t hdr, uv, pairs, total;
    } lay{};
    bool prof_env = false;
    bool prof_slow = false;
    std::string prof_maps;
    bool uv_env = true;
    bool early_env = false;
    bool stage_kernel = true;
    bool stage_split = true;
    const void* h_arena_dev = nullptr;
    HostBuf<double> h_out;
    bool state_export = false, export_on = false;
    bool state_fresh = false;
    std::vector<int> hs_free, hs_pb_fa, hs_pb_fb;
    DevBuf<double> d_raws, d_rawl, d_partA, d_partD, d_cpart, d_sys, d_dc, d_trial4;
    DevBuf<int> d_singular;
    size_t n_pad = 0;
    DevBuf<LmState> d_state;
    HostBuf<LmState> h_state;
    DevBuf<unsigned long long> d_tick;
    unsigned long long* h_tick = nullptr;
    unsigned long long n_tick = 0;
    bool settled = true, tick_wait = true;
    double wclk_khz = 1.0e5;
    ncclComm_t comm = nullptr;
    int nranks = 1, rank = 0;
    int coll = 0;
    bool sharded() const { return coll != 0; }
    double* xbuf = nullptr;
    P2P p2p{};
    bool p2p_opened[kP2PMax] = {};
    DevBuf<int> d_p2p_err;
    DevBuf<unsigned long long> d_xgen;
    DevBuf<int> d_xnw;
    DevBuf<unsigned long long> d_k6tag;
    DevBuf<unsigned> d_k6cnt;

    void init(const rsvio_ba_params& p) {
        P = p;
        if (P.max_keyframes < 2 || P.max_keyframes > kMaxFree + 1 || P.max_landmarks < 1 ||
            P.max_landmarks > (1 << 26) || P.max_observations < 1)
            throw std::invalid_argument("invalid BA capacities (max_keyframes in [2, 21], max_landmarks <= 2^26)");
        RSVIO_HIP(hipSetDevice(P.device));
        RSVIO_HIP(hipStreamCreateWithFlags(&stream, hipStreamNonBlocking));
        RSVIO_HIP(hipEventCreate(&ev0));
        RSVIO_HIP(hipEventCreate(&ev1));
        RSVIO_HIP(hipEventCreateWithFlags(&gv.ev_launch, hipEventDisableTiming));
        RSVIO_HIP(hipEventCreateWithFlags(&gd.ev_launch, hipEventDisableTiming));
        RSVIO_HIP(hipEventCreateWithFlags(&ev_desc, hipEventDisableTiming));
        const char* fv = std::getenv("RSVIO_P2P_FOLD");
        if (fv && fv[0] >= '0' && fv[0] <= '4') fold_lvl = fold_req = fv[0] - '0';
        const char* dv = std::getenv("RSVIO_BA_DESC");
        desc_on = !(dv && dv[0] == '0');
        const char* gu = std::getenv("RSVIO_BA_GRAPH_UPDATE");
        graph_update = !(gu && gu[0] == '0');
        h_state.alloc(1, hipHostMallocCoherent);
        h_out.alloc((size_t)7 * P.max_keyframes + (size_t)3 * P.max_landmarks, hipHostMallocCoherent);
        d_tick.alloc(2);
        RSVIO_HIP(hipMemset(d_tick.p, 0, 2 * sizeof(unsigned long long)));
        RSVIO_HIP(hipHostMalloc(reinterpret_cast<void**>(&h_tick), (4 + kK7Blocks) * sizeof(unsigned long long),
                                hipHostMallocCoherent));
        std::memset(h_tick, 0, (4 + kK7Blocks) * sizeof(unsigned long long));
        {
            int khz = 0;
            if (hipDeviceGetAttribute(&khz, hipDeviceAttributeWallClockRate, P.device) == hipSuccess && khz > 0)
                wclk_khz = khz;
        }
        const char* wv = std::getenv("RSVIO_BA_WAIT");
        tick_wait = !(wv && std::strcmp(wv, "sync") == 0);
        const char* ge = std::getenv("RSVIO_BA_GRAPHS");
        graphs_ok = !(ge && ge[0] == '0');
        const char* pv = std::getenv("RSVIO_BA_PROFILE");
        prof_env = pv != nullptr;
        prof_slow = pv && std::strcmp(pv, "slow") == 0;
        const char* u32v = std::getenv("RSVIO_BA_UV32");
        uv_env = !(u32v && u32v[0] == '0');
        const char* ecv = std::getenv("RSVIO_BA_EARLY_COPY");
        early_env = ecv && ecv[0] == '1';
        const char* stv = std::getenv("RSVIO_BA_STAGE");
        stage_kernel = !(stv && std::strcmp(stv, "sdma") == 0);
        if (stage_kernel) early_env = false;
        const char* ssv = std::getenv("RSVIO_BA_STAGE_SPLIT");
        stage_split = stage_kernel && !(ssv && ssv[0] == '0');
        const char* kv = std::getenv("RSVIO_K5");
        if (kv && std::strcmp(kv, "gj1") == 0) k5_variant = 1;
        if (kv && std::strcmp(kv, "pipe4") == 0) k5_variant = 0;
        if (kv && std::strcmp(kv, "mfma") == 0) k5_variant = 2;
    }
    ~BundleAdjuster() {
        if (stream) (void)hipStreamSynchronize(stream);
        settled = true;
        if (h_tick) (void)hipHostFree(h_tick);
        drop_graph();
        destroy_retired();
        if (comm) ncclCommDestroy(comm);
        for (int r = 0; r < kP2PMax; ++r)
            if (p2p_opened[r]) (void)hipIpcCloseMemHandle(p2p.peer[r]);
        if (xbuf) (void)hipFree(xbuf);
        if (ev0) (void)hipEventDestroy(ev0);
        if (ev1) (void)hipEventDestroy(ev1);
        if (gv.ev_launch) (void)hipEventDestroy(gv.ev_launch);
        if (gd.ev_launch) (void)hipEventDestroy(gd.ev_launch);
        if (ev_desc) (void)hipEventDestroy(ev_desc);
        if (stream && own_stream) (void)hipStreamDestroy(stream);
    }

    template <class T>
    static void grow(DevBuf<T>& b, size_t n) {
        if (b.n < n) b.alloc(std::max<size_t>(n, 1));
    }
    Prob prob() const {
        Prob p;
        p.free_idx = reinterpret_cast<const int*>(d_arena.p + lay.free_idx);
        p.slot_hdr = reinterpret_cast<const int4*>(d_arena.p + lay.hdr);
        p.slot_uv = reinterpret_cast<const double2*>(d_arena.p + lay.uv);
        p.pairs = reinterpret_cast<const int4*>(d_arena.p + lay.pairs);
        p.pb_fa = reinterpret_cast<const int*>(d_arena.p + lay.pb_fa);
        p.pb_fb = reinterpret_cast<const int*>(d_arena.p + lay.pb_fb);
        p.dmap = reinterpret_cast<const int*>(d_arena.p + lay.dmap);
        return p;
    }
    Work work(int it) const {
        Work w = work_at((it + 1) & 1);
        w.st_prev = d_state.p + (it & 1);
        return w;
    }
    Work work_at(int si) const {
        Work w;
        w.pose[0] = d_pose2.p; w.pose[1] = d_pose2.p + 7 * (size_t)G.n_kf;
        w.pw[0] = d_pw2.p; w.pw[1] = d_pw2.p + 3 * (size_t)std::max(G.n_lm, 1);
        w.pose_init = reinterpret_cast<const double*>(d_arena.p + lay.pose_init);
        w.pw_init = reinterpret_cast<const double*>(d_arena.p + lay.pw_init);
        w.raws[0] = d_raws.p; w.raws[1] = d_raws.p + (size_t)kRawF * std::max<size_t>(n_pad, 1);
        w.rawl[0] = d_rawl.p; w.rawl[1] = d_rawl.p + (size_t)kLmF * std::max(G.n_lm, 1);
        w.singular = d_singular.p;
        w.p2p_err = coll == 2 ? d_p2p_err.p : nullptr;
        w.partA = d_partA.p; w.partD = d_partD.p;
        w.cpart = d_cpart.p;
        w.sys = d_sys.p; w.dc = d_dc.p; w.trial4 = d_trial4.p;
        w.st = d_state.p + si;
        w.st_prev = w.st;
        w.tick = d_tick.p;
        return w;
    }

    void grow_buffers() {
        const int n_kf = G.n_kf, n_lm = G.n_lm, n_pb = G.n_pb, n_free = G.n_free, n_wave = G.n_wave;
        grow(d_pose2, 14 * (size_t)n_kf);
        grow(d_pw2, 6 * (size_t)std::max(n_lm, 1));
        {
            const size_t nc = (size_t)kGrp * ((size_t)36 * n_pb + 12 * n_free + 2);
            if (d_cpart.n < nc) {
                grow(d_cpart, nc);
                RSVIO_HIP(hipMemsetAsync(d_cpart.p, 0, sizeof(double) * d_cpart.n, stream));
            }
        }
        grow(d_raws, (size_t)2 * kRawF * std::max<size_t>(n_pad, 1));
        grow(d_rawl, (size_t)2 * kLmF * std::max(n_lm, 1));
        grow(d_singular, 1);
        grow(d_partA, (size_t)kPartA * std::max(n_wave, 1));
        grow(d_partD, (size_t)kPartD * std::max(n_wave, 1));
        grow(d_sys, (size_t)36 * n_pb + 12 * n_free + 2);
        grow(d_dc, (size_t)6 * n_free);
        grow(d_trial4, 4);
        grow(d_state, 2);
        if (d_k6tag.n < (size_t)2 * kPartD * std::max(n_wave, 1)) {
            grow(d_k6tag, (size_t)2 * kPartD * std::max(n_wave, 1));
            RSVIO_HIP(hipMemsetAsync(d_k6tag.p, 0, sizeof(unsigned long long) * d_k6tag.n, stream));
        }
        if (d_k6cnt.n < 1) {
            grow(d_k6cnt, 1);
            RSVIO_HIP(hipMemsetAsync(d_k6cnt.p, 0, sizeof(unsigned), stream));
        }
    }

    void set_problem(int n_kf, const double* pose7, const uint8_t* kf_fixed, int n_lm, const double* pW, int n_obs,
                     const int32_t* obs_lm, const int32_t* obs_kf, const uint8_t* obs_cam, const double* obs_uv,
                     const double* TCB2) {
        const bool prof = prof_env;
        auto tp0 = std::chrono::steady_clock::now();
        double tms[12];
        long flt[12];
        int ntm = 0;
        auto faults = [] {
            struct rusage ru;
            getrusage(RUSAGE_THREAD, &ru);
            return (long)ru.ru_minflt;
        };
        long f0 = prof ? faults() : 0;
        auto mark = [&] {
            if (!prof) return;
            const auto t = std::chrono::steady_clock::now();
            const long f = faults();
            tms[ntm] = std::chrono::duration<double, std::micro>(t - tp0).count();
            flt[ntm++] = f - f0;
            tp0 = t;
            f0 = f;
        };
        if (pend.active) throw CallOrderError("set_problem: a solve is in flight (call rsvio_ba_wait first)");
        if (graph_update && gv.exec)
            gv.stale = true;
        else
            drop_slot(gv);
        solves_of_problem = 0;
        state_export = false;
        if (n_kf < 1 || n_kf > P.max_keyframes || n_lm < 0 || n_lm > P.max_landmarks || n_obs < 0 ||
            n_obs > P.max_observations)
            throw std::invalid_argument("problem exceeds the handle's capacities");
        auto& free_idx = hs_free;
        free_idx.assign(n_kf, -1);
        int n_free = 0;
        for (int k = 0; k < n_kf; ++k)
            if (!kf_fixed[k]) free_idx[k] = n_free++;
        if (n_free > kMaxFree) throw std::invalid_argument("too many free keyframes");
        if (n_free < 1) throw std::invalid_argument("no free keyframe");
        auto &pb_fa = hs_pb_fa, &pb_fb = hs_pb_fb;
        pb_fa.clear();
        pb_fb.clear();
        for (int a = 0; a < n_free; ++a)
            for (int b = a; b < n_free; ++b) {
                pb_fa.push_back(a);
                pb_fb.push_back(b);
            }
        const int n_pb = (int)pb_fa.size();
        const int n_chunk = kGrp * n_pb;
        auto al = [](size_t b) { return (b + 255) & ~(size_t)255; };
        const size_t nl1 = (size_t)std::max(n_lm, 1);
        ArenaLayout L{};
        size_t off = 0;
        L.desc = off;      off += al(sizeof(WinDesc));
        L.pose_init = off; off += al(sizeof(double) * 7 * (size_t)n_kf);
        L.pw_init = off;   off += al(sizeof(double) * 3 * nl1);
        L.free_idx = off;  off += al(sizeof(int) * (size_t)n_kf);
        L.pb_fa = off;     off += al(sizeof(int) * (size_t)n_pb);
        L.pb_fb = off;     off += al(sizeof(int) * (size_t)n_pb);
        L.dmap = off;      off += al(sizeof(int) * ((size_t)36 * n_pb + 12 * n_free));
        L.lm_base = off;   off += al(sizeof(int) * nl1);
        L.wave_fill = off; off += al(sizeof(int) * nl1);
        L.wave_lm = off;   off += al(sizeof(int) * (nl1 + 1));
        L.mask = off;      off += al(sizeof(unsigned long long) * nl1);
        L.key = off;       off += al(sizeof(unsigned) * std::max(n_obs, 1));
        L.ouv = off;       off += al(sizeof(double2) * std::max(n_obs, 1));
        L.upload = off;
        mark();
        if (up_pending) settle();
        if (h_arena.n < L.upload) {
            h_arena.alloc(L.upload + L.upload / 4, hipHostMallocCoherent);
            void* dp = nullptr;
            RSVIO_HIP(hipHostGetDevicePointer(&dp, h_arena.p, 0));
            h_arena_dev = dp;
        }
        uint8_t* hb = h_arena.p;
        mark();
        auto* m2 = reinterpret_cast<unsigned long long*>(hb + L.mask);
        auto* key = reinterpret_cast<unsigned*>(hb + L.key);
        bool uv32 = false;
        if (!observation_pass(n_obs, obs_lm, obs_kf, obs_cam, obs_uv, n_lm, n_kf, key, m2,
                              uv_env ? reinterpret_cast<float*>(hb + L.ouv) : nullptr, &uv32)) {
            std::memset(m2, 0, sizeof(unsigned long long) * (size_t)n_lm);
            int cl = -1;
            unsigned long long cm = 0;
            for (int i = 0; i < n_obs; ++i) {
                const int l = obs_lm[i], k = obs_kf[i], c = obs_cam[i];
                if (l < 0 || l >= n_lm || k < 0 || k >= n_kf || c > 1)
                    throw std::invalid_argument("observation index out of range");
                if (l != cl) {
                    if (cl >= 0) m2[cl] = cm;
                    cl = l;
                    cm = m2[l];
                }
                const unsigned long long b = 1ull << (2 * k + c);
                if (cm & b)
                    throw std::invalid_argument("more than one observation of a landmark per camera and keyframe");
                cm |= b;
                key[i] = (unsigned)l << 6 | (unsigned)k << 1 | (unsigned)c;
            }
            if (cl >= 0) m2[cl] = cm;
            uv32 = uv_env && rsvio_obs::uv_narrow(2 * (size_t)n_obs, obs_uv, reinterpret_cast<float*>(hb + L.ouv));
        }
        if (!uv32) std::memcpy(hb + L.ouv, obs_uv, sizeof(double2) * (size_t)n_obs);
        L.upload = L.ouv + al((uv32 ? sizeof(float2) : sizeof(double2)) * std::max(n_obs, 1));
        if (d_arena.n < L.upload) {
            d_arena.alloc(2 * L.upload);
        }
        settled = false;
        auto stage = [&](size_t off0, size_t off1) {
            const int nw = (int)((off1 - off0) / 16);
            if (nw <= 0) return;
            hipLaunchKernelGGL(ba_stage_in, dim3((nw + 511) / 512), dim3(256), 0, stream,
                               reinterpret_cast<const uint4*>(static_cast<const uint8_t*>(h_arena_dev) + off0),
                               reinterpret_cast<uint4*>(d_arena.p + off0), nw);
            RSVIO_HIP(hipGetLastError());
        };
        if (stage_split) stage(L.mask, L.upload);
        if (early_env)
            RSVIO_HIP(hipMemcpyAsync(d_arena.p + L.mask, hb + L.mask, L.upload - L.mask, hipMemcpyHostToDevice, stream));
        mark();
        auto* lm_base = reinterpret_cast<int*>(hb + L.lm_base);
        auto* wave_fill = reinterpret_cast<int*>(hb + L.wave_fill);
        auto* wave_lm = reinterpret_cast<int*>(hb + L.wave_lm);
        int n_wave = 0, fill = 0;
        int gl[kGrp] = {0, 0, 0, 0, 0, 0, 0, 0};
        const bool want_env = n_free > 10;
        unsigned long long freebits = 0;
        for (int k = 0; k < n_kf; ++k)
            if (free_idx[k] >= 0) freebits |= 1ull << (2 * k);
        int cand[kMaxFree];
        for (int k = 0; k < kMaxFree; ++k) cand[k] = -1;
        for (int l = 0; l < n_lm; ++l) {
            const int ns = slot_count(m2[l]);
            if (!ns) {
                lm_base[l] = -1;
                continue;
            }
            if (want_env) {
                const unsigned long long kb = (m2[l] | (m2[l] >> 1)) & freebits;
                if (kb) {
                    const int a = free_idx[__builtin_ctzll(kb) >> 1], b = free_idx[(63 - __builtin_clzll(kb)) >> 1];
                    cand[a] = std::max(cand[a], b);
                }
            }
            if (n_wave == 0 || fill + ns > 64) {
                if (n_wave) wave_fill[n_wave - 1] = fill;
                wave_lm[n_wave] = l;
                ++n_wave;
                fill = 0;
            }
            lm_base[l] = 64 * (n_wave - 1) + fill;
            gl[(n_wave - 1) % kGrp] += 1;
            fill += ns;
        }
        if (n_wave) wave_fill[n_wave - 1] = fill;
        wave_lm[n_wave] = n_lm;
        int stride = 1;
        for (int x = 0; x < kGrp; ++x) stride = std::max(stride, gl[x]);
        n_pad = (size_t)64 * n_wave;
        if (coll == 2 && fold_lvl == 2 && n_wave > kP2PWaves)
            throw std::invalid_argument("shard exceeds the folded P2P trial exchange (16384 waves): RSVIO_P2P_FOLD=1");
        mark();
        L.hdr = off;   off += al(sizeof(int4) * 2 * std::max<size_t>(n_pad, 1));
        L.uv = off;    off += al(sizeof(double2) * 2 * std::max<size_t>(n_pad, 1));
        L.pairs = off; off += al(sizeof(int4) * (size_t)n_chunk * stride);
        L.total = off;
        if (d_arena.n < L.total) {
            d_arena.alloc(L.total + L.total / 4);
            if (stage_split) stage(L.mask, L.upload);
            if (early_env)
                RSVIO_HIP(hipMemcpyAsync(d_arena.p + L.mask, hb + L.mask, L.upload - L.mask, hipMemcpyHostToDevice,
                                         stream));
        }
        lay = L;
        std::memcpy(hb + L.pose_init, pose7, sizeof(double) * 7 * (size_t)n_kf);
        if (n_lm) std::memcpy(hb + L.pw_init, pW, sizeof(double) * 3 * (size_t)n_lm);
        std::memcpy(hb + L.free_idx, free_idx.data(), sizeof(int) * (size_t)n_kf);
        std::memcpy(hb + L.pb_fa, pb_fa.data(), sizeof(int) * (size_t)n_pb);
        std::memcpy(hb + L.pb_fb, pb_fb.data(), sizeof(int) * (size_t)n_pb);
        if (n_free <= 10)
            mf_dense_map(n_free, n_pb, pb_fa.data(), pb_fb.data(), reinterpret_cast<int*>(hb + L.dmap));
        else
            mf_dense_map(n_free, n_pb, pb_fa.data(), pb_fb.data(), reinterpret_cast<int*>(hb + L.dmap),
                         6 * bk_template_nf(n_free), kBkLd);
        G.n_kf = n_kf; G.n_free = n_free; G.n_lm = n_lm; G.n_obs = n_obs; G.n_slot = (int)n_pad;
        G.n_pb = n_pb; G.n_wave = n_wave; G.n_chunk = n_chunk; G.pair_stride = stride;
        for (int k = 0, run = -1; k < kMaxFree; ++k) {
            run = std::max(run, cand[k]);
            G.env[k] = (unsigned char)(k >= n_free ? k : want_env ? std::max(k, run) : n_free - 1);
        }
        G.env_on = want_env ? 1 : 0;
        for (int c = 0; c < 2; ++c)
            for (int i = 0; i < 16; ++i) G.TCB[c].m[i] = TCB2[16 * c + i];
        grow_buffers();
        fill_desc(hdesc);
        std::memcpy(hb + L.desc, &hdesc, sizeof(WinDesc));
        mark();
        if (stage_kernel) {
            stage(0, stage_split ? L.mask : L.upload);
        } else {
            RSVIO_HIP(hipMemcpyAsync(d_arena.p, hb, early_env ? L.mask : L.upload, hipMemcpyHostToDevice, stream));
        }
        up_pending = true;
        {
            SlotSrc S;
            S.mask = reinterpret_cast<const unsigned long long*>(d_arena.p + L.mask);
            S.lm_base = reinterpret_cast<const int*>(d_arena.p + L.lm_base);
            S.wave_fill = reinterpret_cast<const int*>(d_arena.p + L.wave_fill);
            S.key = reinterpret_cast<const unsigned*>(d_arena.p + L.key);
            S.uv = reinterpret_cast<const double2*>(d_arena.p + L.ouv);
            S.uv32 = uv32 ? 1 : 0;
            S.wave_lm = reinterpret_cast<const int*>(d_arena.p + L.wave_lm);
            S.nb_lm = (n_lm + 255) / 256;
            S.nb_pad = (int)((n_pad + 255) / 256);
            const int nb = S.nb_lm + S.nb_pad + (n_obs + 255) / 256;
            hipLaunchKernelGGL(ba_build_layout, dim3(nb + n_chunk), dim3(256), 0, stream, G, prob(), S, nb,
                               reinterpret_cast<int4*>(d_arena.p + L.hdr), reinterpret_cast<double2*>(d_arena.p + L.uv),
                               reinterpret_cast<int4*>(d_arena.p + L.pairs));
            RSVIO_HIP(hipGetLastError());
        }
        mark();
        *h_state.p = LmState{};
        state_fresh = true;
        has_problem = true;
        mark();
        if (prof) {
            double tot = 0.0;
            long ftot = 0;
            for (int i = 0; i < ntm; ++i) tot += tms[i], ftot += flt[i];
            if (!prof_slow || tot > 1000.0 || ftot > 100)
                fprintf(stderr, "[rsvio] set_problem us: checks+layout %.1f upload wait %.1f observations %.1f waves %.1f "
                        "tables %.1f enqueue %.1f grow %.1f (upload %zu B, arena %zu B); minor faults %ld %ld %ld %ld "
                        "%ld %ld %ld\n",
                        tms[0], tms[1], tms[2], tms[3], tms[4], tms[5], tms[6], L.upload, L.total, flt[0], flt[1],
                        flt[2], flt[3], flt[4], flt[5], flt[6]);
            if (prof_slow && (tot > 1000.0 || ftot > 100)) {
                std::string maps;
                if (FILE* fm = std::fopen("/proc/self/maps", "r")) {
                    char buf[4096];
                    size_t n;
                    while ((n = std::fread(buf, 1, sizeof buf, fm)) > 0) maps.append(buf, n);
                    std::fclose(fm);
                }
                std::vector<std::string> now, was;
                auto split = [](const std::string& t, std::vector<std::string>& out) {
                    size_t a = 0;
                    while (a < t.size()) {
                        size_t b = t.find('\n', a);
                        if (b == std::string::npos) b = t.size();
                        out.emplace_back(t, a, b - a);
                        a = b + 1;
                    }
                };
                split(maps, now);
                split(prof_maps, was);
                std::sort(was.begin(), was.end());
                for (const auto& l : now)
                    if (!std::binary_search(was.begin(), was.end(), l)) fprintf(stderr, "[rsvio]   new map: %s\n", l.c_str());
                prof_maps.swap(maps);
            }
        }
    }

    void allreduce(double* buf, size_t n) {
        if (!sharded() || n == 0) return;
        if (coll == 2) {
            if (n > kP2PMsg) throw std::runtime_error("message exceeds the P2P slot");
            hipLaunchKernelGGL(ba_p2p_allreduce, dim3(1), dim3(256), 0, stream, buf, (int)n, p2p, d_xgen.p,
                               d_p2p_err.p);
            RSVIO_HIP(hipGetLastError());
            return;
        }
        if (ncclAllReduce(buf, buf, n, ncclDouble, ncclSum, comm, stream) != ncclSuccess)
            throw std::runtime_error("RCCL all-reduce failed");
    }

    void enqueue_reset(double lambda0) {
        settled = false;
        const int n = std::max(std::max(7 * G.n_kf, 3 * G.n_lm), 1);
        hipLaunchKernelGGL(ba_reset, dim3((n + 255) / 256), dim3(256), 0, stream, G, work_at(0), lambda0);
        RSVIO_HIP(hipGetLastError());
    }

    void enqueue_start(double lambda0) {
        settled = false;
        if (G.n_wave)
            hipLaunchKernelGGL(ba_linearize, dim3(G.n_wave), dim3(64), 0, stream, G, prob(), work_at(0), lambda0);
        else
            enqueue_reset(lambda0);
        RSVIO_HIP(hipGetLastError());
    }

    void enqueue_linear_system(int it, const LmArgs& la, bool materialise) {
        const Prob pr = prob();
        const Work wk = work(it);
        hipLaunchKernelGGL(ba_schur_chunks, dim3(G.n_chunk), dim3(kSchurThreads), 0, stream, G, pr, wk, la,
                           sharded() ? 1 : 0);
        RSVIO_HIP(hipGetLastError());
        if (!sharded() && !materialise) {
            if (wide_combine()) {
                hipLaunchKernelGGL(ba_schur_combine_wide, dim3((36 * G.n_pb + 12 * G.n_free + 255) / 256), dim3(256),
                                   0, stream, G, pr, wk);
                RSVIO_HIP(hipGetLastError());
            }
            return;
        }
        if (coll == 2) {
            hipLaunchKernelGGL(ba_p2p_sys, dim3(1), dim3(256), 0, stream, G, pr, wk, p2p, d_xgen.p, d_p2p_err.p);
            RSVIO_HIP(hipGetLastError());
            return;
        }
        hipLaunchKernelGGL(ba_schur_combine, dim3(1), dim3(256), 0, stream, G, pr, wk, rank == 0 ? 1 : 0);
        RSVIO_HIP(hipGetLastError());
        allreduce(d_sys.p, (size_t)36 * G.n_pb + 12 * G.n_free + 2);
    }

    bool wide_combine() const { return !sharded() && k5_variant == 2 && G.n_free > 10; }
    void launch_camera_solve(const Prob& pr, const Work& wk, int combine) {
        if (combine && wide_combine()) combine = 0;
        const dim3 g(1), b(kK5Threads);
        if (k5_variant == 2 && G.n_free <= 10) {
            switch (G.n_free) {
#define RSVIO_CAMM(NF) \
    case NF: hipLaunchKernelGGL(ba_camera_solve_mfma<NF>, g, b, 0, stream, G, pr, wk, combine); break;
                RSVIO_CAMM(1) RSVIO_CAMM(2) RSVIO_CAMM(3) RSVIO_CAMM(4) RSVIO_CAMM(5)
                RSVIO_CAMM(6) RSVIO_CAMM(7) RSVIO_CAMM(8) RSVIO_CAMM(9) RSVIO_CAMM(10)
#undef RSVIO_CAMM
                default: break;
            }
            RSVIO_HIP(hipGetLastError());
            return;
        }
        switch (G.n_free <= 10 ? G.n_free : 0) {
#define RSVIO_CAM(NF) \
    case NF: hipLaunchKernelGGL(ba_camera_solve<NF>, g, b, 0, stream, G, pr, wk, combine, k5_variant); break;
            RSVIO_CAM(1) RSVIO_CAM(2) RSVIO_CAM(3) RSVIO_CAM(4) RSVIO_CAM(5)
            RSVIO_CAM(6) RSVIO_CAM(7) RSVIO_CAM(8) RSVIO_CAM(9) RSVIO_CAM(10)
#undef RSVIO_CAM
            default: {
                if (k5_variant == 2) {
                    const dim3 b3(64 * kBkWaves);
                    switch (bk_template_nf(G.n_free)) {
                        case 13: hipLaunchKernelGGL(ba_camera_solve_blk<13>, g, b3, 0, stream, G, pr, wk, combine); break;
                        case 16: hipLaunchKernelGGL(ba_camera_solve_blk<16>, g, b3, 0, stream, G, pr, wk, combine); break;
                        default: hipLaunchKernelGGL(ba_camera_solve_blk<20>, g, b3, 0, stream, G, pr, wk, combine); break;
                    }
                    break;
                }
                const dim3 b2(64 * kX2Waves);
                if (G.n_free <= 13) hipLaunchKernelGGL(ba_camera_solve_x2<13>, g, b2, 0, stream, G, pr, wk, combine);
                else if (G.n_free <= 16) hipLaunchKernelGGL(ba_camera_solve_x2<16>, g, b2, 0, stream, G, pr, wk, combine);
                else hipLaunchKernelGGL(ba_camera_solve_x2<20>, g, b2, 0, stream, G, pr, wk, combine);
                break;
            }
        }
        RSVIO_HIP(hipGetLastError());
    }

    static LmArgs lm_args(const rsvio_lm_cfg& cfg) {
        return LmArgs{cfg.max_iterations, cfg.cost_tolerance, cfg.parameter_tolerance};
    }

    void enqueue_iteration(const rsvio_lm_cfg& cfg, int it) {
        const Prob pr = prob();
        const Work wk = work(it);
        if (p2p_fold()) {
            if (p2p_fold2() || p2p_fold4())
                hipLaunchKernelGGL(ba_schur_chunks_p2p, dim3(G.n_chunk), dim3(kSchurThreads), 0, stream, G, pr, wk,
                                   lm_args(cfg), p2p, d_xgen.p, d_p2p_err.p, p2p_fold4() ? 4 : 2);
            else
                hipLaunchKernelGGL(ba_schur_chunks, dim3(G.n_chunk), dim3(kSchurThreads), 0, stream, G, pr, wk,
                                   lm_args(cfg), 1);
            RSVIO_HIP(hipGetLastError());
            switch (G.n_free) {
#define RSVIO_CAMP(NF) \
    case NF:                                                                                                            \
        if (p2p.ll)                                                                                                     \
            hipLaunchKernelGGL((ba_camera_solve_mfma_p2p<NF, true>), dim3(1), dim3(kK5Threads), 0, stream, G, pr, wk,  \
                               p2p, d_xgen.p, d_p2p_err.p);                                                            \
        else                                                                                                            \
            hipLaunchKernelGGL((ba_camera_solve_mfma_p2p<NF, false>), dim3(1), dim3(kK5Threads), 0, stream, G, pr, wk, \
                               p2p, d_xgen.p, d_p2p_err.p);                                                            \
        break;
                RSVIO_CAMP(1) RSVIO_CAMP(2) RSVIO_CAMP(3) RSVIO_CAMP(4) RSVIO_CAMP(5)
                RSVIO_CAMP(6) RSVIO_CAMP(7) RSVIO_CAMP(8) RSVIO_CAMP(9) RSVIO_CAMP(10)
#undef RSVIO_CAMP
                default: throw std::logic_error("p2p_fold: more than 10 free keyframes");
            }
            RSVIO_HIP(hipGetLastError());
        } else {
            enqueue_linear_system(it, lm_args(cfg), false);
            launch_camera_solve(pr, wk, sharded() ? 0 : 1);
        }
        if (p2p_fold2()) {
            if (G.n_wave)
                hipLaunchKernelGGL(ba_backsub_relinearize_p2p, dim3(G.n_wave), dim3(64), 0, stream, G, pr, wk, p2p,
                                   d_xgen.p);
            RSVIO_HIP(hipGetLastError());
            return;
        }
        if (p2p_fold4()) {
            hipLaunchKernelGGL(ba_backsub_relinearize_p2p4, dim3(std::max(G.n_wave, 1)), dim3(64), 0, stream, G, pr,
                               wk, p2p, d_xgen.p, d_k6cnt.p, d_k6tag.p);
            RSVIO_HIP(hipGetLastError());
            return;
        }
        if (p2p_fold3()) {
            hipLaunchKernelGGL(ba_backsub_relinearize_p2p3, dim3(G.n_wave + 1), dim3(64), 0, stream, G, pr, wk, p2p,
                               d_xgen.p, d_p2p_err.p, d_k6tag.p);
            RSVIO_HIP(hipGetLastError());
            return;
        }
        if (G.n_wave) hipLaunchKernelGGL(ba_backsub_relinearize, dim3(G.n_wave), dim3(64), 0, stream, G, pr, wk);
        RSVIO_HIP(hipGetLastError());
        if (coll == 2) {
            hipLaunchKernelGGL(ba_p2p_trial, dim3(1), dim3(256), 0, stream, G, pr, wk, p2p, d_xgen.p, d_p2p_err.p);
            RSVIO_HIP(hipGetLastError());
        } else if (sharded()) {
            hipLaunchKernelGGL(ba_reduce_trial, dim3(1), dim3(64), 0, stream, G, pr, wk, rank == 0 ? 1 : 0);
            RSVIO_HIP(hipGetLastError());
            allreduce(d_trial4.p, 4);
        }
    }

    void enqueue_decide(const rsvio_lm_cfg& cfg, int it) {
        if (p2p_fold2() || p2p_fold4()) {
            hipLaunchKernelGGL(ba_lm_decide_p2p, dim3(export_on ? kK7Blocks : 1), dim3(kK7Threads), 0, stream, G,
                               prob(), work(it), lm_args(cfg), h_state.p, h_tick, export_on ? h_out.p : nullptr, p2p,
                               d_xgen.p, d_p2p_err.p, p2p_fold4() ? 4 : 2);
            RSVIO_HIP(hipGetLastError());
            return;
        }
        hipLaunchKernelGGL(ba_lm_decide, dim3(export_on ? kK7Blocks : 1), dim3(kK7Threads), 0, stream, G, prob(),
                           work(it), sharded() ? 1 : 0, lm_args(cfg), h_state.p, h_tick, export_on ? h_out.p : nullptr);
        RSVIO_HIP(hipGetLastError());
    }

    void enqueue_start_d(double lambda0, int wcap) {
        hipLaunchKernelGGL(bab_linearize, dim3(wcap, 1), dim3(64), 0, stream, dptr(), lambda0);
        RSVIO_HIP(hipGetLastError());
    }
    void enqueue_iteration_d(const rsvio_lm_cfg& cfg, int it, int wcap) {
        const int wi = it & 1;
        hipLaunchKernelGGL(bab_schur_chunks, dim3(G.n_chunk, 1), dim3(kSchurThreads), 0, stream, dptr(), wi, lm_args(cfg));
        RSVIO_HIP(hipGetLastError());
        switch (G.n_free) {
#define RSVIO_CAMD(NF) \
    case NF: hipLaunchKernelGGL(bab_camera_solve<NF>, dim3(1), dim3(kK5Threads), 0, stream, dptr(), wi); break;
            RSVIO_CAMD(1) RSVIO_CAMD(2) RSVIO_CAMD(3) RSVIO_CAMD(4) RSVIO_CAMD(5)
            RSVIO_CAMD(6) RSVIO_CAMD(7) RSVIO_CAMD(8) RSVIO_CAMD(9) RSVIO_CAMD(10)
#undef RSVIO_CAMD
            default: throw std::logic_error("descriptor mode: more than 10 free keyframes");
        }
        RSVIO_HIP(hipGetLastError());
        hipLaunchKernelGGL(bab_backsub_relinearize, dim3(wcap, 1), dim3(64), 0, stream, dptr(), wi);
        RSVIO_HIP(hipGetLastError());
    }
    void enqueue_decide_d(const rsvio_lm_cfg& cfg, int it) {
        hipLaunchKernelGGL(bad_lm_decide, dim3(export_on ? kK7Blocks : 1), dim3(kK7Threads), 0, stream, dptr(), it & 1,
                           lm_args(cfg), h_state.p, h_tick, export_on ? h_out.p : nullptr);
        RSVIO_HIP(hipGetLastError());
    }

    struct Pending {
        bool active = false, skipped = false;
        bool by_tick = false;
        rsvio_lm_cfg cfg{};
        int enq = 0, max_it = 0;
    } pend;

    void enqueue_chunk(int k) {
        settled = false;
        for (int i = 0; i < k; ++i) enqueue_iteration(pend.cfg, pend.enq + i);
        pend.enq += k;
        enqueue_decide(pend.cfg, pend.enq);
        ++n_tick;
        if (!pend.by_tick) RSVIO_HIP(hipEventRecord(ev1, stream));
    }

    void resync_ticks() noexcept {
        (void)hipStreamSynchronize(stream);
        (void)hipGetLastError();
        settled = true;
        unsigned long long t = 0;
        if (hipMemcpy(&t, d_tick.p, sizeof t, hipMemcpyDeviceToHost) == hipSuccess) n_tick = t;
        pend.active = false;
    }

    void start(const rsvio_lm_cfg& cfg) {
        if (!has_problem) throw std::invalid_argument("no problem uploaded");
        if (pend.active) throw CallOrderError("a solve is already in flight (call finish first)");
        try {
            start_impl(cfg);
        } catch (...) {
            resync_ticks();
            throw;
        }
    }

    void start_impl(const rsvio_lm_cfg& cfg) {
        G.huber_delta = cfg.huber_delta;
        G.chol = cfg.linear_solver == RSVIO_SOLVER_CHOLESKY ? 1 : 0;
        pend = Pending{};
        pend.active = true;
        pend.cfg = cfg;
        pend.by_tick = by_tick();
        state_export = false;
        if (!sharded() && (G.n_obs < 6 || G.n_obs < G.n_kf + G.n_lm)) {
            pend.skipped = true;
            return;
        }
        pend.max_it = std::max(cfg.max_iterations, 1);
        settled = false;
        state_fresh = false;
        if (!pend.by_tick) RSVIO_HIP(hipEventRecord(ev0, stream));
        int k = std::min(std::max(last_iterations, 1), pend.max_it);
        if (start_graph(cfg, k)) {
            ++n_tick;
            pend.enq += k;
            if (!pend.by_tick) RSVIO_HIP(hipEventRecord(ev1, stream));
        } else {
            enqueue_start(cfg.lambda_init);
            enqueue_chunk(k);
        }
    }

    void finish(rsvio_ba_result* res) {
        if (!pend.active) throw CallOrderError("no solve in flight");
        try {
            finish_impl(res);
        } catch (...) {
            resync_ticks();
            throw;
        }
    }

    void finish_impl(rsvio_ba_result* res) {
        pend.active = false;
        res->iterations = 0;
        if (pend.skipped) {
            res->status = RSVIO_LM_SKIPPED;
            res->initial_cost = res->final_cost = 0.0;
            res->solve_ms = 0.0;
            return;
        }
        const bool by_tick = pend.by_tick;
        while (true) {
            if (by_tick)
                wait_tick();
            else
                RSVIO_HIP(hipStreamSynchronize(stream));
            if (h_state.p->done || pend.enq >= pend.max_it) break;
            enqueue_chunk(std::min(iter_chunk, pend.max_it - pend.enq));
        }
        up_pending = false;
        last_iterations = h_state.p->iter;
        if (coll == 2) {
            if (by_tick) {
                if (h_state.p->p2p_err) {
                    settle();
                    throw std::runtime_error("P2P all-reduce: a peer did not arrive");
                }
            } else {
                p2p_check();
            }
        }
        state_export = export_on && h_state.p->done != 0;
        float ms = 0.0f;
        if (by_tick) {
            ms = (float)((double)(h_tick[2] - h_tick[1]) / wclk_khz);
        } else {
            settled = true;
            RSVIO_HIP(hipEventElapsedTime(&ms, ev0, ev1));
        }
        const LmState& s = *h_state.p;
        res->status = s.status;
        res->iterations = s.iter;
        res->initial_cost = s.initial_cost;
        res->final_cost = s.cost;
        res->solve_ms = ms;
    }

    void p2p_export(int nr, hipIpcMemHandle_t* h) {
        if (nr < 1 || nr > kP2PMax) throw std::invalid_argument("P2P: 1..8 ranks");
        if (!xbuf) {
            const size_t bytes = kP2PBytes;
            RSVIO_HIP(hipExtMallocWithFlags(reinterpret_cast<void**>(&xbuf), bytes, hipDeviceMallocUncached));
            RSVIO_HIP(hipMemset(xbuf, 0, bytes));
            d_p2p_err.alloc(1);
            RSVIO_HIP(hipMemset(d_p2p_err.p, 0, sizeof(int)));
            d_xgen.alloc(1);
            RSVIO_HIP(hipMemset(d_xgen.p, 0, sizeof(unsigned long long)));
            d_xnw.alloc(kP2PMax);
            RSVIO_HIP(hipMemset(d_xnw.p, 0, sizeof(int) * kP2PMax));
        }
        RSVIO_HIP(hipIpcGetMemHandle(h, xbuf));
    }

    void p2p_check() {
        int err = 0;
        RSVIO_HIP(hipMemcpy(&err, d_p2p_err.p, sizeof(int), hipMemcpyDeviceToHost));
        if (err) throw std::runtime_error("P2P all-reduce: a peer did not arrive");
    }

    void p2p_attach(int nr, int rk, const hipIpcMemHandle_t* hs) {
        require_idle("rsvio_ba_attach_p2p");
        if (nr < 1 || nr > kP2PMax || rk < 0 || rk >= nr) throw std::invalid_argument("P2P: bad rank layout");
        if (!xbuf) throw CallOrderError("P2P: export the buffer first");
        P2P P{};
        P.nranks = nr;
        P.rank = rk;
        P.xnw = d_xnw.p;
        const char* llv = std::getenv("RSVIO_P2P_LL");
        P.ll = llv && llv[0] == '1';
        for (int r = 0; r < nr; ++r) {
            if (r == rk) {
                P.peer[r] = xbuf;
                continue;
            }
            void* ptr = nullptr;
            RSVIO_HIP(hipIpcOpenMemHandle(&ptr, hs[r], hipIpcMemLazyEnablePeerAccess));
            P.peer[r] = static_cast<double*>(ptr);
            p2p_opened[r] = true;
        }
        int pci_dom = 0, pci_bus = 0, pci_dev = 0;
        RSVIO_HIP(hipDeviceGetAttribute(&pci_dom, hipDeviceAttributePciDomainID, this->P.device));
        RSVIO_HIP(hipDeviceGetAttribute(&pci_bus, hipDeviceAttributePciBusId, this->P.device));
        RSVIO_HIP(hipDeviceGetAttribute(&pci_dev, hipDeviceAttributePciDeviceId, this->P.device));
        constexpr int kSelf = 6 + kP2PMax;
        static_assert(kSelf <= kP2PLLMax, "the self-test is one flag-in-word message");
        double tv[kSelf] = {};
        const double fl = (double)fold_req, lv = P.ll ? 1.0 : 0.0;
        tv[0] = rk + 1; tv[1] = 1.0; tv[2] = fl; tv[3] = fl * fl; tv[4] = lv; tv[5] = lv * lv;
        tv[6 + rk] = 1.0 + (double)(((long long)pci_dom << 16) | (pci_bus << 8) | pci_dev);
        const int n_self = 6 + nr;
        DevBuf<double> t(kSelf);
        RSVIO_HIP(hipMemcpy(t.p, tv, sizeof(double) * n_self, hipMemcpyHostToDevice));
        hipLaunchKernelGGL(ba_p2p_allreduce, dim3(1), dim3(256), 0, stream, t.p, n_self, P, d_xgen.p, d_p2p_err.p);
        RSVIO_HIP(hipGetLastError());
        double out[kSelf] = {};
        RSVIO_HIP(hipMemcpyAsync(out, t.p, sizeof(double) * n_self, hipMemcpyDeviceToHost, stream));
        RSVIO_HIP(hipStreamSynchronize(stream));
        p2p_check();
        if (out[0] != nr * (nr + 1) / 2.0 || out[1] != (double)nr)
            throw std::runtime_error("P2P all-reduce self-test returned wrong sums");
        if (out[2] != nr * fl || out[3] != nr * fl * fl || out[4] != nr * lv || out[5] != nr * lv)
            throw std::runtime_error("P2P: the ranks disagree on RSVIO_P2P_FOLD / RSVIO_P2P_LL");
        bool shared_gpu = false;
        for (int a = 0; a < nr; ++a)
            for (int b = a + 1; b < nr; ++b) shared_gpu |= out[6 + a] == out[6 + b];
        const char* fsv = std::getenv("RSVIO_P2P_FOLD_SHARED");
        const bool keep2 = fsv && fsv[0] == '1';
        fold_lvl = shared_gpu && !keep2 && (fold_req == 2 || fold_req == 4) ? fold_req - 1 : fold_req;
        p2p_shared_gpu = shared_gpu;
        p2p_share = 0;
        for (int a = 0; a < nr; ++a) p2p_share += out[6 + a] == out[6 + rk];
        refresh_k6_cap();
        p2p = P;
        nranks = nr;
        rank = rk;
        coll = 2;
        drop_graph();
    }

    void refresh_k6_cap() {
        int per_cu = 0;
        RSVIO_HIP(hipOccupancyMaxActiveBlocksPerMultiprocessor(
            &per_cu, reinterpret_cast<const void*>(ba_backsub_relinearize_p2p3), 64, 0));
        int n_cu = 0;
        RSVIO_HIP(hipDeviceGetAttribute(&n_cu, hipDeviceAttributeMultiprocessorCount, P.device));
        uint32_t mask[32] = {};
        if (hipExtStreamGetCUMask(stream, 32, mask) == hipSuccess) {
            int c = 0;
            for (uint32_t w : mask) c += __builtin_popcount(w);
            if (c > 0) n_cu = std::min(n_cu, c);
        } else {
            (void)hipGetLastError();
        }
        const char* ov = std::getenv("RSVIO_K6_CAP");
        k6_cap = per_cu * n_cu / std::max(p2p_share, 1);
        if (ov && ov[0]) k6_cap = std::min(k6_cap, std::atoi(ov));
    }
    int p2p_level() const {
        if (coll != 2) return -1;
        if (!p2p_fold()) return 0;
        return p2p_fold2() ? 2 : p2p_fold3() ? 3 : p2p_fold4() ? 4 : 1;
    }

    double p2p_latency(int reps, int n) {
        require_idle("rsvio_ba_p2p_latency");
        if (coll != 2) throw CallOrderError("P2P latency: the P2P exchange is not attached");
        if (reps < 1 || n < 1 || n > kP2PMsg) throw std::invalid_argument("P2P latency: bad reps or size");
        DevBuf<double> t(n);
        RSVIO_HIP(hipMemsetAsync(t.p, 0, (size_t)n * sizeof(double), stream));
        hipEvent_t a, b;
        RSVIO_HIP(hipEventCreate(&a));
        RSVIO_HIP(hipEventCreate(&b));
        for (int k = 0; k <= reps; ++k) {
            if (k == 1) RSVIO_HIP(hipEventRecord(a, stream));
            hipLaunchKernelGGL(ba_p2p_allreduce, dim3(1), dim3(256), 0, stream, t.p, n, p2p, d_xgen.p, d_p2p_err.p);
        }
        RSVIO_HIP(hipGetLastError());
        RSVIO_HIP(hipEventRecord(b, stream));
        RSVIO_HIP(hipEventSynchronize(b));
        float ms = 0.f;
        RSVIO_HIP(hipEventElapsedTime(&ms, a, b));
        RSVIO_HIP(hipEventDestroy(a));
        RSVIO_HIP(hipEventDestroy(b));
        p2p_check();
        return 1e3 * (double)ms / reps;
    }

    void p2p_detach() {
        require_idle("rsvio_ba_detach_p2p");
        if (coll == 2) coll = comm ? 1 : 0;
        drop_graph();
    }

    void set_stream(hipStream_t s) {
        if (pend.active) throw CallOrderError("a solve is in flight");
        RSVIO_HIP(hipStreamSynchronize(stream));
        if (s) {
            if (own_stream) RSVIO_HIP(hipStreamDestroy(stream));
            stream = s;
            own_stream = false;
        } else if (!own_stream) {
            RSVIO_HIP(hipStreamCreateWithFlags(&stream, hipStreamNonBlocking));
            own_stream = true;
        }
        if (coll == 2) {
            refresh_k6_cap();
            drop_graph();
        }
    }

    void run(const rsvio_lm_cfg& cfg, rsvio_ba_result* res) {
        start(cfg);
        finish(res);
    }

    bool by_tick() const { return tick_wait; }

    void require_idle(const char* what) {
        if (pend.active) throw CallOrderError(std::string(what) + ": a solve is in flight (call rsvio_ba_wait first)");
        settle();
    }

    void settle() {
        if (!settled) {
            RSVIO_HIP(hipStreamSynchronize(stream));
            settled = true;
        }
        up_pending = false;
        destroy_retired();
    }

    void wait_tick() {
        const unsigned long long want = n_tick;
// ... 496 lines not shown
```

### rs-vio_amd/csrc/obs_pass.hpp

```cpp
#pragma once

#include <immintrin.h>

#include <algorithm>
#include <atomic>
#include <chrono>
#include <condition_variable>
#include <cstdint>
#include <cstdlib>
#include <cstring>
#include <mutex>
#include <thread>
#include <vector>

namespace rsvio_obs {

__attribute__((target("avx2"))) static bool uv_narrow_avx2(size_t n2, const double* uv, float* out) {
    size_t i = 0;
    __m256d bad = _mm256_setzero_pd();
    for (; i + 4 <= n2; i += 4) {
        const __m256d d = _mm256_loadu_pd(uv + i);
        const __m128 f = _mm256_cvtpd_ps(d);
        bad = _mm256_or_pd(bad, _mm256_cmp_pd(_mm256_cvtps_pd(f), d, _CMP_NEQ_UQ));
        _mm_storeu_ps(out + i, f);
    }
    bool ok = _mm256_movemask_pd(bad) == 0;
    for (; i < n2; ++i) {
        out[i] = (float)uv[i];
        ok &= (double)out[i] == uv[i];
    }
    return ok;
}
static bool uv_narrow(size_t n2, const double* uv, float* out) {
    static const bool avx2 = __builtin_cpu_supports("avx2");
    if (avx2) return uv_narrow_avx2(n2, uv, out);
    bool ok = true;
    for (size_t i = 0; i < n2; ++i) {
        out[i] = (float)uv[i];
        ok &= (double)out[i] == uv[i];
    }
    return ok;
}

__attribute__((target("avx2"))) static bool obs_keys_avx2(int n_obs, const int32_t* lm, const int32_t* kf,
                                                        const uint8_t* cam, int n_lm, int n_kf, unsigned* key) {
    const __m256i nl1 = _mm256_set1_epi32(n_lm - 1), nk1 = _mm256_set1_epi32(n_kf - 1), one = _mm256_set1_epi32(1);
    __m256i bad = _mm256_setzero_si256();
    int i = 0;
    for (; i + 8 <= n_obs; i += 8) {
        const __m256i l = _mm256_loadu_si256(reinterpret_cast<const __m256i*>(lm + i));
        const __m256i k = _mm256_loadu_si256(reinterpret_cast<const __m256i*>(kf + i));
        const __m256i c = _mm256_cvtepu8_epi32(_mm_loadl_epi64(reinterpret_cast<const __m128i*>(cam + i)));
        bad = _mm256_or_si256(bad, _mm256_xor_si256(_mm256_max_epu32(l, nl1), nl1));
        bad = _mm256_or_si256(bad, _mm256_xor_si256(_mm256_max_epu32(k, nk1), nk1));
        bad = _mm256_or_si256(bad, _mm256_xor_si256(_mm256_max_epu32(c, one), one));
        const __m256i kk = _mm256_or_si256(_mm256_or_si256(_mm256_slli_epi32(l, 6), _mm256_slli_epi32(k, 1)), c);
        _mm256_storeu_si256(reinterpret_cast<__m256i*>(key + i), kk);
    }
    unsigned bad_t = 0;
    for (; i < n_obs; ++i) {
        const unsigned l = (unsigned)lm[i], k = (unsigned)kf[i], c = cam[i];
        bad_t |= (unsigned)(l >= (unsigned)n_lm) | (unsigned)(k >= (unsigned)n_kf) | (unsigned)(c > 1);
        key[i] = l << 6 | k << 1 | c;
    }
    return _mm256_testz_si256(bad, bad) && !bad_t;
}

static bool obs_keys(int n_obs, const int32_t* lm, const int32_t* kf, const uint8_t* cam, int n_lm, int n_kf,
                     unsigned* key) {
    if (n_lm <= 0 || n_kf <= 0) return false;
    static const bool avx2 = __builtin_cpu_supports("avx2");
    if (avx2) return obs_keys_avx2(n_obs, lm, kf, cam, n_lm, n_kf, key);
    unsigned bad = 0;
    for (int i = 0; i < n_obs; ++i) {
        const unsigned l = (unsigned)lm[i], k = (unsigned)kf[i], c = cam[i];
        bad |= (unsigned)(l >= (unsigned)n_lm) | (unsigned)(k >= (unsigned)n_kf) | (unsigned)(c > 1);
        key[i] = l << 6 | k << 1 | c;
    }
    return !bad;
}

static void masks_of_runs(int a, int b, const unsigned* key, unsigned long long* m2) {
    const int n = b - a;
    if (n <= 0) return;
    int cut[5];
    cut[0] = a;
    cut[4] = b;
    for (int q = 1; q < 4; ++q) {
        int c = std::max(a + (int)((long long)q * n / 4), cut[q - 1]);
        while (c > a && c < b && (key[c] >> 6) == (key[c - 1] >> 6)) ++c;
        cut[q] = c;
    }
    int len = n;
    for (int q = 0; q < 4; ++q) len = std::min(len, cut[q + 1] - cut[q]);
    unsigned cl[4] = {~0u, ~0u, ~0u, ~0u};
    unsigned long long cm[4] = {0, 0, 0, 0};
    auto step = [&](int q, int i) {
        const unsigned kj = key[i], l = kj >> 6;
        const unsigned long long bit = 1ull << (kj & 63);
        cm[q] = l == cl[q] ? (cm[q] | bit) : bit;
        cl[q] = l;
        __atomic_store_n(m2 + l, cm[q], __ATOMIC_RELAXED);
    };
    for (int j = 0; j < len; ++j) {
        step(0, cut[0] + j);
        step(1, cut[1] + j);
        step(2, cut[2] + j);
        step(3, cut[3] + j);
    }
    for (int q = 0; q < 4; ++q)
        for (int i = cut[q] + len; i < cut[q + 1]; ++i) step(q, i);
}

__attribute__((target("popcnt"))) static long long mask_bits(int n_lm, const unsigned long long* m2) {
    long long bits = 0;
    for (int l = 0; l < n_lm; ++l) bits += __builtin_popcountll(m2[l]);
    return bits;
}

static bool obs_masks_runs(int n_obs, const unsigned* key, int n_lm, unsigned long long* m2) {
    std::memset(m2, 0, sizeof(unsigned long long) * (size_t)n_lm);
    masks_of_runs(0, n_obs, key, m2);
    return mask_bits(n_lm, m2) == n_obs;
}

class HostPool {
  public:
    using Fn = void (*)(void*, int);

    HostPool(int helpers, int spin_us) : spin_ns_((long long)spin_us * 1000) {
        for (int i = 0; i < helpers; ++i) threads_.emplace_back([this] { helper(); });
    }
    ~HostPool() {
        {
            std::lock_guard<std::mutex> lk(m_);
            stop_.store(true, std::memory_order_seq_cst);
        }
        cv_.notify_all();
        for (auto& t : threads_) t.join();
    }
    int helpers() const { return (int)threads_.size(); }

    bool try_run(int n, Fn fn, void* ctx) {
        std::unique_lock<std::mutex> own(run_m_, std::try_to_lock);
        if (!own.owns_lock()) return false;
        if (n <= 0) return true;
        fn_.store(fn, std::memory_order_relaxed);
        ctx_.store(ctx, std::memory_order_relaxed);
        done_.store(0, std::memory_order_relaxed);
        gen_ = (gen_ + 1) & 0xffffffffu;
        word_.store(pack(gen_, (unsigned)n, 0), std::memory_order_seq_cst);
        if (parked_.load(std::memory_order_seq_cst) > 0) {
            std::lock_guard<std::mutex> lk(m_);
            cv_.notify_all();
        }
        work(gen_);
        while (done_.load(std::memory_order_acquire) < n) _mm_pause();
        return true;
    }

  private:
    static uint64_t pack(uint32_t g, unsigned n, unsigned next) {
        return (uint64_t)g << 32 | (uint64_t)(n & 0xffff) << 16 | (next & 0xffff);
    }
    static uint32_t gen_of(uint64_t v) { return (uint32_t)(v >> 32); }
    static unsigned n_of(uint64_t v) { return (unsigned)(v >> 16) & 0xffff; }
    static unsigned next_of(uint64_t v) { return (unsigned)v & 0xffff; }

    void work(uint32_t g) {
        uint64_t v = word_.load(std::memory_order_acquire);
        while (gen_of(v) == g && next_of(v) < n_of(v)) {
            Fn fn = fn_.load(std::memory_order_relaxed);
            void* ctx = ctx_.load(std::memory_order_relaxed);
            if (word_.compare_exchange_weak(v, v + 1, std::memory_order_acq_rel, std::memory_order_acquire)) {
                fn(ctx, (int)next_of(v));
                done_.fetch_add(1, std::memory_order_release);
                v = word_.load(std::memory_order_acquire);
            }
        }
    }

    void helper() {
        uint32_t seen = 0;
        for (;;) {
            const auto t0 = std::chrono::steady_clock::now();
            uint64_t v;
            for (;;) {
                if (stop_.load(std::memory_order_relaxed)) return;
                v = word_.load(std::memory_order_acquire);
                if (gen_of(v) != seen) break;
                _mm_pause();
                if (std::chrono::duration_cast<std::chrono::nanoseconds>(std::chrono::steady_clock::now() - t0)
                        .count() > spin_ns_) {
                    std::unique_lock<std::mutex> lk(m_);
                    parked_.fetch_add(1, std::memory_order_seq_cst);
                    cv_.wait(lk, [&] {
                        return stop_.load(std::memory_order_seq_cst) ||
                               gen_of(word_.load(std::memory_order_seq_cst)) != seen;
                    });
                    parked_.fetch_sub(1, std::memory_order_seq_cst);
                    if (stop_.load(std::memory_order_relaxed)) return;
                }
            }
            seen = gen_of(v);
            work(seen);
        }
    }

    std::vector<std::thread> threads_;
    std::atomic<uint64_t> word_{0};
    std::atomic<Fn> fn_{nullptr};
    std::atomic<void*> ctx_{nullptr};
    std::atomic<int> done_{0};
    std::atomic<int> parked_{0};
    std::atomic<bool> stop_{false};
    std::mutex m_, run_m_;
    std::condition_variable cv_;
    uint32_t gen_ = 0;
    long long spin_ns_;
};

struct ObsJob {
    const int32_t *lm, *kf;
    const uint8_t* cam;
    const double* uv;
    int n_lm, n_kf;
    unsigned* key;
    unsigned long long* m2;
    float* uv32;
    const int* cut;
    std::atomic<int> bad{0};
    std::atomic<int> wide{0};

    static void chunk(void* p, int c) {
        ObsJob& J = *static_cast<ObsJob*>(p);
        const int a = J.cut[c], b = J.cut[c + 1];
        if (!obs_keys(b - a, J.lm + a, J.kf + a, J.cam + a, J.n_lm, J.n_kf, J.key + a))
            J.bad.store(1, std::memory_order_relaxed);
        else
            masks_of_runs(a, b, J.key, J.m2);
        if (J.uv32 && !uv_narrow(2 * (size_t)(b - a), J.uv + 2 * (size_t)a, J.uv32 + 2 * (size_t)a))
            J.wide.store(1, std::memory_order_relaxed);
    }
};

static HostPool* shared_pool() {
    static HostPool* pool = [] {
        const char* tv = std::getenv("RSVIO_BA_HOST_THREADS");
        const char* sv = std::getenv("RSVIO_BA_HOST_SPIN_US");
        const int nt = tv ? std::max(0, std::min(15, std::atoi(tv))) : 0;
        const int sp = sv ? std::max(0, std::atoi(sv)) : 2000;
        return nt > 0 ? new HostPool(nt, sp) : nullptr;
    }();
    return pool;
}

#ifndef RSVIO_OBS_CHUNK
#define RSVIO_OBS_CHUNK 3072
#endif
constexpr int kObsChunk = RSVIO_OBS_CHUNK;

static bool observation_pass(int n_obs, const int32_t* lm, const int32_t* kf, const uint8_t* cam,
                             const double* uv, int n_lm, int n_kf, unsigned* key, unsigned long long* m2,
                             float* uv32, bool* narrowed) {
    if (n_lm <= 0 || n_kf <= 0) return false;
    HostPool* pool = n_obs >= 2 * kObsChunk ? shared_pool() : nullptr;
    std::memset(m2, 0, sizeof(unsigned long long) * (size_t)n_lm);
    if (pool) {
        const int nc = std::min((n_obs + kObsChunk - 1) / kObsChunk, 0xffff);
        int cut_s[64];
        std::vector<int> cut_v;
        int* cut = cut_s;
        if (nc + 1 > 64) {
            cut_v.resize(nc + 1);
            cut = cut_v.data();
        }
        cut[0] = 0;
        cut[nc] = n_obs;
        for (int q = 1; q < nc; ++q) {
            int c = std::max((int)((long long)q * n_obs / nc), cut[q - 1]);
            while (c > 0 && c < n_obs && lm[c] == lm[c - 1]) ++c;
            cut[q] = c;
        }
        ObsJob J;
        J.lm = lm; J.kf = kf; J.cam = cam; J.uv = uv; J.n_lm = n_lm; J.n_kf = n_kf;
        J.key = key; J.m2 = m2; J.uv32 = uv32; J.cut = cut;
        if (pool->try_run(nc, &ObsJob::chunk, &J)) {
            *narrowed = uv32 && !J.wide.load(std::memory_order_relaxed);
            if (J.bad.load(std::memory_order_relaxed)) return false;
            return mask_bits(n_lm, m2) == n_obs;
        }
    }
    *narrowed = uv32 && uv_narrow(2 * (size_t)n_obs, uv, uv32);
    if (!obs_keys(n_obs, lm, kf, cam, n_lm, n_kf, key)) return false;
    masks_of_runs(0, n_obs, key, m2);
    return mask_bits(n_lm, m2) == n_obs;
}

}
```

Before: 4889.

## Cache host tables, fuse wave packing into observation pass, prefetch slot data in descriptor kernels

Several changes land together. The host now caches the free-keyframe and pair tables across calls when the fixed-keyframe pattern is unchanged, and adds a WavePack helper so wave packing can happen inside the single-threaded observation pass. The arena is laid out by capacity, so buffer addresses stay stable and the recorded graph is reused more often; graph-hit detection now compares several entry pointers. New descriptor-mode kernels take the slot pointers as direct arguments and issue the slot loads before the dead-wave check, hiding the dependent descriptor loads. This adds complexity, new env flags and extra capacity-sized allocations.

```diff
diff --git a/rs-vio_amd/csrc/ba.hip b/rs-vio_amd/csrc/ba.hip
--- a/rs-vio_amd/csrc/ba.hip
+++ b/rs-vio_amd/csrc/ba.hip
@@ -618,11 +618,38 @@
         build_pairs_body(G, Pr, S, pairs, b - nb_slots);
 }
 
+__device__ __forceinline__ void desc_touch1(const void* p) { __asm__ volatile("" ::"s"(p)); }
+template <class... T>
+__device__ __forceinline__ void desc_touch(const T*... p) {
+    (desc_touch1(p), ...);
+}
+
+struct SlotEntry {
+    const int4* hdr;
+    const double2* uv;
+    const double* raws[2];
+    const LmState* st;
+    int cap_slots;
+    int skip, bound;
+    __device__ __forceinline__ bool dead(int w) const { return (skip | (w >= bound)) != 0; }
+};
+
+template <bool PRE = false>
 __device__ void linearize_body(const Geometry& G, const Prob& Pr, const Work& Wk, int w, int with_reset,
-                               double lambda0) {
+                               double lambda0, const SlotEntry* E = nullptr) {
     __shared__ double sh[10][64];
     const int lane = threadIdx.x;
     const int s = 64 * w + lane;
+    int4 e0, e1;
+    double2 euv[2];
+    if constexpr (PRE) {
+        const int sc = min(s, E->cap_slots - 1);
+        e0 = E->hdr[2 * sc]; e1 = E->hdr[2 * sc + 1];
+        euv[0] = E->uv[2 * sc]; euv[1] = E->uv[2 * sc + 1];
+        desc_touch(Wk.pose_init, Wk.pw_init, Wk.st, Wk.pose[0], Wk.pose[1], Wk.pw[0], Wk.pw[1]);
+        __asm__ volatile("" ::"v"(e0.x), "v"(e1.x), "v"(euv[0].x), "v"(euv[1].x));
+        if (E->dead(w)) return;
+    }
     if (with_reset) {
         const int nt = G.n_wave * 64;
         for (int i = s; i < 7 * G.n_kf; i += nt) {
@@ -644,8 +671,8 @@
     }
     const double* pose0 = with_reset ? Wk.pose_init : Wk.pose[0];
     const double* pw0 = with_reset ? Wk.pw_init : Wk.pw[0];
-    const int4 h0 = Pr.slot_hdr[2 * s], h1 = Pr.slot_hdr[2 * s + 1];
-    const double2 uvq[2] = {Pr.slot_uv[2 * s], Pr.slot_uv[2 * s + 1]};
+    const int4 h0 = PRE ? e0 : Pr.slot_hdr[2 * s], h1 = PRE ? e1 : Pr.slot_hdr[2 * s + 1];
+    const double2 uvq[2] = {PRE ? euv[0] : Pr.slot_uv[2 * s], PRE ? euv[1] : Pr.slot_uv[2 * s + 1]};
     STAMP(11);
     const bool act = h1.y > 0;
     const int kf = h0.x, l = h0.y, first = act ? h0.z : lane, nk = act ? h0.w : 1;
@@ -671,7 +698,7 @@
     STAMP(14);
 }
 
-__global__ __launch_bounds__(64) void ba_linearize(Geometry G, Prob Pr, Work Wk, double lambda0) {
+__global__ __launch_bounds__(64) void ba_linearize(Prob Pr, Work Wk, double lambda0, Geometry G) {
     linearize_body(G, Pr, Wk, blockIdx.x, 1, lambda0);
 }
 
@@ -1051,8 +1078,8 @@
     RTSTAMP(2);
 }
 
-__global__ __launch_bounds__(kSchurThreads) void ba_schur_chunks(Geometry G, Prob Pr, Work Wk, LmArgs la,
-                                                                  int pre_reduced) {
+__global__ __launch_bounds__(kSchurThreads) void ba_schur_chunks(Prob Pr, Work Wk, LmArgs la, int pre_reduced,
+                                                                  Geometry G) {
     schur_chunks_body(G, Pr, Wk, la, pre_reduced, blockIdx.x);
 }
 
@@ -2716,15 +2743,18 @@
     STAMP(5);
 }
 
-template <bool FUSED>
+template <bool FUSED, bool PRE = false>
 __device__ void k6_body(const Geometry& G, const Prob& Pr, const Work& Wk, int w, int lane, double (*sh)[64],
                         double (*shp)[64], double (*shs)[64], const P2P* PP = nullptr,
                         unsigned long long gen = 0, unsigned long long* k6tag = nullptr,
-                        unsigned long long* k6part = nullptr) {
+                        unsigned long long* k6part = nullptr, const SlotEntry* E = nullptr) {
     const int s = 64 * w + lane;
-    const int4 h0 = Pr.slot_hdr[2 * s], h1 = Pr.slot_hdr[2 * s + 1];
-    const double2 uvq[2] = {Pr.slot_uv[2 * s], Pr.slot_uv[2 * s + 1]};
-    const LmState* st = Wk.st;
+    const int sc = PRE ? min(s, E->cap_slots - 1) : s;
+    const int4* hdrp = PRE ? E->hdr : Pr.slot_hdr;
+    const double2* uvp = PRE ? E->uv : Pr.slot_uv;
+    const int4 h0 = hdrp[2 * sc], h1 = hdrp[2 * sc + 1];
+    const double2 uvq[2] = {uvp[2 * sc], uvp[2 * sc + 1]};
+    const LmState* st = PRE ? E->st : Wk.st;
     const bool act = h1.y > 0;
     const int kf = h0.x, l = h0.y, first = act ? h0.z : lane, nk = act ? h0.w : 1;
     const bool fr = h1.x >= 0;
@@ -2732,12 +2762,26 @@
     double recb[2][18], Lmb[2][10], pcb[2][3], p7b[2][7], d6[6];
 #pragma unroll
     for (int b = 0; b < 2; ++b) {
-        const double2* wr = reinterpret_cast<const double2*>(Wk.raws[b] + (size_t)s * kRawF);
+        const double2* wr = reinterpret_cast<const double2*>((PRE ? E->raws[b] : Wk.raws[b]) + (size_t)sc * kRawF);
 #pragma unroll
         for (int i = 0; i < 9; ++i) {
             const double2 x = wr[i];
             recb[b][2 * i] = x.x; recb[b][2 * i + 1] = x.y;
         }
+    }
+    const int done = st->done, solve_ok = st->solve_ok, cur = st->cur;
+    const double lambda = st->lambda;
+    if constexpr (PRE) {
+        desc_touch(Wk.rawl[0], Wk.rawl[1], Wk.pw[0], Wk.pw[1], Wk.pose[0], Wk.pose[1], Wk.dc);
+#pragma unroll
+        for (int b = 0; b < 2; ++b)
+#pragma unroll
+            for (int i = 0; i < 18; ++i) __asm__ volatile("" ::"v"(recb[b][i]));
+        __asm__ volatile("" ::"v"(h0.x), "v"(h1.x), "v"(uvq[0].x), "v"(uvq[1].x));
+        if (E->dead(w)) return;
+    }
+#pragma unroll
+    for (int b = 0; b < 2; ++b) {
         const double2* lr = reinterpret_cast<const double2*>(Wk.rawl[b] + (size_t)lc * kLmF);
 #pragma unroll
         for (int i = 0; i < 5; ++i) {
@@ -2751,8 +2795,6 @@
     }
 #pragma unroll
     for (int i = 0; i < 6; ++i) d6[i] = Wk.dc[6 * fc + i];
-    const int done = st->done, solve_ok = st->solve_ok, cur = st->cur;
-    const double lambda = st->lambda;
 #pragma unroll
     for (int b = 0; b < 2; ++b) {
 #pragma unroll
@@ -2875,7 +2917,7 @@
     RTSTAMP(8);
 }
 
-__global__ __launch_bounds__(64) void ba_backsub_relinearize(Geometry G, Prob Pr, Work Wk) {
+__global__ __launch_bounds__(64) void ba_backsub_relinearize(Prob Pr, Work Wk, Geometry G) {
     __shared__ double sh[10][64];
     __shared__ double shp[3][64];
     __shared__ double shs[4][64];
@@ -3191,12 +3233,6 @@
     int skip;
 };
 
-__device__ __forceinline__ void desc_touch1(const void* p) { __asm__ volatile("" ::"s"(p)); }
-template <class... T>
-__device__ __forceinline__ void desc_touch(const T*... p) {
-    (desc_touch1(p), ...);
-}
-
 
 __global__ __launch_bounds__(64) void bab_linearize(const WinDesc* __restrict__ D, double lambda0) {
     const WinDesc& d = D[blockIdx.y];
@@ -3261,6 +3297,30 @@
     const Prob Pr = d.Pr;
     const Work& Wk = d.W[wi];
     lm_decide_body(d.G, Pr, Wk, 0, la, host, htick, hout);
+}
+
+__global__ __launch_bounds__(64) void bad_linearize(const WinDesc* __restrict__ D, int cap_slots, const int4* hdr,
+                                                    const double2* uv, double lambda0) {
+    const WinDesc& d = D[0];
+    const int skip = d.skip, bound = d.G.n_wave;
+    const Prob Pr = d.Pr;
+    const Work& Wk = d.W[2];
+    const SlotEntry E{hdr, uv, {nullptr, nullptr}, nullptr, cap_slots, skip, bound};
+    linearize_body<true>(d.G, Pr, Wk, blockIdx.x, 1, lambda0, &E);
+}
+
+__global__ __launch_bounds__(64) void bad_backsub_relinearize(const WinDesc* __restrict__ D, int wi, int cap_slots,
+                                                              const int4* hdr, const double2* uv, const double* raws0,
+                                                              const double* raws1, const LmState* st) {
+    const WinDesc& d = D[0];
+    const int skip = d.skip, bound = d.G.n_wave;
+    const Prob Pr = d.Pr;
+    const Work& Wk = d.W[wi];
+    const SlotEntry E{hdr, uv, {raws0, raws1}, st, cap_slots, skip, bound};
+    __shared__ double sh[10][64];
+    __shared__ double shp[3][64];
+    __shared__ double shs[4][64];
+    k6_body<false, true>(d.G, Pr, Wk, blockIdx.x, threadIdx.x, sh, shp, shs, nullptr, 0, nullptr, nullptr, &E);
 }
 
 __global__ __launch_bounds__(64) void bab_lm_decide(const WinDesc* __restrict__ D, int wi, LmArgs la, LmState* host) {
@@ -3398,10 +3458,6 @@
 
 using rsvio_obs::observation_pass;
 
-__attribute__((target("popcnt"))) static inline int slot_count(unsigned long long m) {
-    return __builtin_popcountll((m | (m >> 1)) & kEvenBits);
-}
-
 struct BundleAdjuster {
     rsvio_ba_params P{};
     hipStream_t stream = nullptr;
@@ -3416,7 +3472,7 @@
         rsvio_lm_cfg cfg{};
         bool exp = false, stale = false;
         int nf = -1, coll = -1, wcap = 0, chunk = -1;
-        const void* dptr = nullptr;
+        const void* args[8] = {};
         hipEvent_t ev_launch = nullptr;
     };
     GraphSlot gv, gd;
@@ -3477,6 +3533,13 @@
     int p2p_share = 1;
     bool p2p_fold4() const { return fold_lvl == 4 && p2p_fold(); }
     const WinDesc* dptr() const { return reinterpret_cast<const WinDesc*>(d_arena.p + lay.desc); }
+    void entry_args(const void* (&a)[8]) const {
+        const Prob pr = prob();
+        const Work w0 = work(0), w1 = work(1);
+        a[0] = dptr(); a[1] = pr.slot_hdr; a[2] = pr.slot_uv; a[3] = w0.raws[0]; a[4] = w0.raws[1];
+        a[5] = w0.st; a[6] = w1.st;
+        a[7] = reinterpret_cast<const void*>((uintptr_t)cap_slots());
+    }
     void fill_desc(WinDesc& d) const {
         d = WinDesc{};
         d.G = G;
@@ -3512,12 +3575,15 @@
         ++solves_of_problem;
         GraphSlot& sl = dm ? gd : gv;
         if (dm && (G.huber_delta != desc_huber || G.chol != desc_chol)) refresh_desc();
-        const int wcap = (G.n_wave + G.n_wave / 4 + kGrp - 1) / kGrp * kGrp;
+        const int wcap = wave_grid(G.n_wave);
+        if (dm && (size_t)wcap > cap_wave) throw std::logic_error("descriptor mode: grid past the slot buffers");
         const bool k_ok = sl.k == k || (dm && sl.k > k && sl.k <= k + 2);
         const bool topo = sl.exec && k_ok && same_cfg(sl.cfg, cfg) && sl.exp == export_on && sl.nf == G.n_free &&
                           sl.coll == coll;
-        const bool hit = topo && (dm ? (sl.dptr == dptr() && sl.chunk == G.n_chunk && G.n_wave <= sl.wcap &&
-                                        2 * G.n_wave > sl.wcap)
+        const void* ea[8] = {};
+        if (dm) entry_args(ea);
+        const bool hit = topo && (dm ? (std::equal(ea, ea + 8, sl.args) && sl.chunk == G.n_chunk &&
+                                        G.n_wave <= sl.wcap && 2 * G.n_wave > sl.wcap)
                                      : !sl.stale);
         if (hit) k = sl.k;
         if (!hit) {
@@ -3585,7 +3651,7 @@
             sl.stale = false;
             sl.wcap = wcap;
             sl.chunk = G.n_chunk;
-            sl.dptr = dm ? static_cast<const void*>(dptr()) : nullptr;
+            std::copy(ea, ea + 8, sl.args);
         }
         settled = false;
         RSVIO_HIP(hipGraphLaunch(sl.exec, stream));
@@ -3598,9 +3664,13 @@
     HostBuf<uint8_t> h_arena;
     bool up_pending = false;
     struct ArenaLayout {
-        size_t desc, pose_init, pw_init, free_idx, pb_fa, pb_fb, dmap, mask, lm_base, wave_fill, wave_lm, key, ouv, upload;
-        size_t hdr, uv, pairs, total;
+        size_t hdr, uv, pairs, staged;
+        size_t free_idx, pb_fa, pb_fb, dmap, desc, lm_base, wave_fill, wave_lm, pose_init, pw_init, mask, key, ouv, upload;
+        size_t total;
     } lay{};
+    size_t cap_wave = 0, cap_pairs = 0;
+    int cap_slots() const { return (int)(64 * cap_wave); }
+    static int wave_grid(int n_wave) { return (n_wave + n_wave / 4 + kGrp - 1) / kGrp * kGrp; }
     bool prof_env = false;
     bool prof_slow = false;
     std::string prof_maps;
@@ -3613,6 +3683,12 @@
     bool state_export = false, export_on = false;
     bool state_fresh = false;
     std::vector<int> hs_free, hs_pb_fa, hs_pb_fb;
+    bool tab_valid = false;
+    int tab_nkf = 0, tab_nfree = 0;
+    uint8_t tab_fixed[kMaxFree + 1] = {};
+    bool tab_cache = true;
+    bool fold_pack = false;
+    bool early_state = false;
     DevBuf<double> d_raws, d_rawl, d_partA, d_partD, d_cpart, d_sys, d_dc, d_trial4;
     DevBuf<int> d_singular;
     size_t n_pad = 0;
@@ -3682,6 +3758,12 @@
         if (stage_kernel) early_env = false;
         const char* ssv = std::getenv("RSVIO_BA_STAGE_SPLIT");
         stage_split = stage_kernel && !(ssv && ssv[0] == '0');
+        const char* tcv = std::getenv("RSVIO_BA_TABLE_CACHE");
+        tab_cache = !(tcv && tcv[0] == '0');
+        const char* fpv = std::getenv("RSVIO_BA_FOLD_PACK");
+        fold_pack = fpv && fpv[0] == '1';
+        const char* esv = std::getenv("RSVIO_BA_EARLY_STATE");
+        early_state = esv && esv[0] == '1';
         const char* kv = std::getenv("RSVIO_K5");
         if (kv && std::strcmp(kv, "gj1") == 0) k5_variant = 1;
         if (kv && std::strcmp(kv, "pipe4") == 0) k5_variant = 0;
@@ -3731,7 +3813,7 @@
         w.pw[0] = d_pw2.p; w.pw[1] = d_pw2.p + 3 * (size_t)std::max(G.n_lm, 1);
         w.pose_init = reinterpret_cast<const double*>(d_arena.p + lay.pose_init);
         w.pw_init = reinterpret_cast<const double*>(d_arena.p + lay.pw_init);
-        w.raws[0] = d_raws.p; w.raws[1] = d_raws.p + (size_t)kRawF * std::max<size_t>(n_pad, 1);
+        w.raws[0] = d_raws.p; w.raws[1] = d_raws.p + (size_t)kRawF * std::max<size_t>(64 * cap_wave, 1);
         w.rawl[0] = d_rawl.p; w.rawl[1] = d_rawl.p + (size_t)kLmF * std::max(G.n_lm, 1);
         w.singular = d_singular.p;
         w.p2p_err = coll == 2 ? d_p2p_err.p : nullptr;
@@ -3755,11 +3837,11 @@
                 RSVIO_HIP(hipMemsetAsync(d_cpart.p, 0, sizeof(double) * d_cpart.n, stream));
             }
         }
-        grow(d_raws, (size_t)2 * kRawF * std::max<size_t>(n_pad, 1));
+        grow(d_raws, (size_t)2 * kRawF * std::max<size_t>(64 * cap_wave, 1));
         grow(d_rawl, (size_t)2 * kLmF * std::max(n_lm, 1));
         grow(d_singular, 1);
-        grow(d_partA, (size_t)kPartA * std::max(n_wave, 1));
-        grow(d_partD, (size_t)kPartD * std::max(n_wave, 1));
+        grow(d_partA, (size_t)kPartA * std::max<size_t>(std::max<size_t>(cap_wave, n_wave), 1));
+        grow(d_partD, (size_t)kPartD * std::max<size_t>(std::max<size_t>(cap_wave, n_wave), 1));
         grow(d_sys, (size_t)36 * n_pb + 12 * n_free + 2);
         grow(d_dc, (size_t)6 * n_free);
         grow(d_trial4, 4);
@@ -3808,36 +3890,47 @@
             n_obs > P.max_observations)
             throw std::invalid_argument("problem exceeds the handle's capacities");
         auto& free_idx = hs_free;
-        free_idx.assign(n_kf, -1);
-        int n_free = 0;
-        for (int k = 0; k < n_kf; ++k)
-            if (!kf_fixed[k]) free_idx[k] = n_free++;
-        if (n_free > kMaxFree) throw std::invalid_argument("too many free keyframes");
-        if (n_free < 1) throw std::invalid_argument("no free keyframe");
         auto &pb_fa = hs_pb_fa, &pb_fb = hs_pb_fb;
-        pb_fa.clear();
-        pb_fb.clear();
-        for (int a = 0; a < n_free; ++a)
-            for (int b = a; b < n_free; ++b) {
-                pb_fa.push_back(a);
-                pb_fb.push_back(b);
-            }
+        bool tab_hit = tab_valid && tab_cache && tab_nkf == n_kf;
+        for (int k = 0; tab_hit && k < n_kf; ++k) tab_hit = tab_fixed[k] == (kf_fixed[k] ? 1 : 0);
+        if (!tab_hit) {
+            tab_valid = false;
+            free_idx.assign(n_kf, -1);
+            int nf = 0;
+            for (int k = 0; k < n_kf; ++k)
+                if (!kf_fixed[k]) free_idx[k] = nf++;
+            if (nf > kMaxFree) throw std::invalid_argument("too many free keyframes");
+            if (nf < 1) throw std::invalid_argument("no free keyframe");
+            pb_fa.clear();
+            pb_fb.clear();
+            for (int a = 0; a < nf; ++a)
+                for (int b = a; b < nf; ++b) {
+                    pb_fa.push_back(a);
+                    pb_fb.push_back(b);
+                }
+            tab_nkf = n_kf;
+            tab_nfree = nf;
+            for (int k = 0; k < n_kf; ++k) tab_fixed[k] = kf_fixed[k] ? 1 : 0;
+        }
+        const int n_free = tab_nfree;
         const int n_pb = (int)pb_fa.size();
         const int n_chunk = kGrp * n_pb;
         auto al = [](size_t b) { return (b + 255) & ~(size_t)255; };
         const size_t nl1 = (size_t)std::max(n_lm, 1);
+        const size_t cap_kf = (size_t)P.max_keyframes, cap_nf = std::min<size_t>(cap_kf, kMaxFree),
+                     cap_pb = cap_nf * (cap_nf + 1) / 2;
         ArenaLayout L{};
         size_t off = 0;
+        L.free_idx = off;  off += al(sizeof(int) * cap_kf);
+        L.pb_fa = off;     off += al(sizeof(int) * cap_pb);
+        L.pb_fb = off;     off += al(sizeof(int) * cap_pb);
+        L.dmap = off;      off += al(sizeof(int) * (36 * cap_pb + 12 * cap_nf));
         L.desc = off;      off += al(sizeof(WinDesc));
-        L.pose_init = off; off += al(sizeof(double) * 7 * (size_t)n_kf);
-        L.pw_init = off;   off += al(sizeof(double) * 3 * nl1);
-        L.free_idx = off;  off += al(sizeof(int) * (size_t)n_kf);
-        L.pb_fa = off;     off += al(sizeof(int) * (size_t)n_pb);
-        L.pb_fb = off;     off += al(sizeof(int) * (size_t)n_pb);
-        L.dmap = off;      off += al(sizeof(int) * ((size_t)36 * n_pb + 12 * n_free));
         L.lm_base = off;   off += al(sizeof(int) * nl1);
         L.wave_fill = off; off += al(sizeof(int) * nl1);
         L.wave_lm = off;   off += al(sizeof(int) * (nl1 + 1));
+        L.pose_init = off; off += al(sizeof(double) * 7 * (size_t)n_kf);
+        L.pw_init = off;   off += al(sizeof(double) * 3 * nl1);
         L.mask = off;      off += al(sizeof(unsigned long long) * nl1);
         L.key = off;       off += al(sizeof(unsigned) * std::max(n_obs, 1));
         L.ouv = off;       off += al(sizeof(double2) * std::max(n_obs, 1));
@@ -3854,9 +3947,16 @@
         mark();
         auto* m2 = reinterpret_cast<unsigned long long*>(hb + L.mask);
         auto* key = reinterpret_cast<unsigned*>(hb + L.key);
+        const bool want_env = n_free > 10;
+        rsvio_obs::WavePack wp;
+        wp.begin(reinterpret_cast<int*>(hb + L.lm_base), reinterpret_cast<int*>(hb + L.wave_fill),
+                 reinterpret_cast<int*>(hb + L.wave_lm), free_idx.data(), n_kf, want_env);
+        bool packed = false;
         bool uv32 = false;
         if (!observation_pass(n_obs, obs_lm, obs_kf, obs_cam, obs_uv, n_lm, n_kf, key, m2,
-                              uv_env ? reinterpret_cast<float*>(hb + L.ouv) : nullptr, &uv32)) {
+                              uv_env ? reinterpret_cast<float*>(hb + L.ouv) : nullptr, &uv32, fold_pack ? &wp : nullptr,
+                              &packed)) {
+            packed = false;
             std::memset(m2, 0, sizeof(unsigned long long) * (size_t)n_lm);
             int cl = -1;
             unsigned long long cm = 0;
@@ -3879,93 +3979,97 @@
             uv32 = uv_env && rsvio_obs::uv_narrow(2 * (size_t)n_obs, obs_uv, reinterpret_cast<float*>(hb + L.ouv));
         }
         if (!uv32) std::memcpy(hb + L.ouv, obs_uv, sizeof(double2) * (size_t)n_obs);
+        L.total = L.upload;
         L.upload = L.ouv + al((uv32 ? sizeof(float2) : sizeof(double2)) * std::max(n_obs, 1));
-        if (d_arena.n < L.upload) {
-            d_arena.alloc(2 * L.upload);
-        }
+        auto copy_state = [&] {
+            std::memcpy(hb + L.pose_init, pose7, sizeof(double) * 7 * (size_t)n_kf);
+            if (n_lm) std::memcpy(hb + L.pw_init, pW, sizeof(double) * 3 * (size_t)n_lm);
+        };
+        if (early_state) copy_state();
+        size_t hole = 0;
+        auto place = [&] {
+            const size_t cpad = std::max<size_t>(64 * cap_wave, 1);
+            size_t o = 0;
+            L.hdr = o;   o += al(sizeof(int4) * 2 * cpad);
+            L.uv = o;    o += al(sizeof(double2) * 2 * cpad);
+            L.pairs = o; o += al(sizeof(int4) * std::max<size_t>(cap_pairs, 1));
+            hole = o;
+        };
+        int n_wave = 0, stride = 1;
+        auto close_pack = [&] {
+            stride = wp.finish(n_lm);
+            n_wave = wp.n_wave;
+            n_pad = (size_t)64 * n_wave;
+            bool grown = false;
+            const size_t need_w = (size_t)wave_grid(n_wave), need_p = (size_t)n_chunk * stride;
+            if (need_w > cap_wave) {
+                cap_wave = std::max(need_w, cap_wave + cap_wave / 2);
+                grown = true;
+            }
+            if (need_p > cap_pairs) {
+                cap_pairs = std::max(need_p + need_p / 4, cap_pairs + cap_pairs / 2);
+                grown = true;
+            }
+            if (grown) place();
+            return grown;
+        };
+        place();
+        if (packed) close_pack();
+        auto fit_arena = [&] {
+            if (d_arena.n >= hole + L.total) return false;
+            d_arena.alloc(hole + L.total + L.total / 4);
+            tab_valid = tab_hit = false;
+            return true;
+        };
+        fit_arena();
         settled = false;
         auto stage = [&](size_t off0, size_t off1) {
             const int nw = (int)((off1 - off0) / 16);
             if (nw <= 0) return;
             hipLaunchKernelGGL(ba_stage_in, dim3((nw + 511) / 512), dim3(256), 0, stream,
                                reinterpret_cast<const uint4*>(static_cast<const uint8_t*>(h_arena_dev) + off0),
-                               reinterpret_cast<uint4*>(d_arena.p + off0), nw);
+                               reinterpret_cast<uint4*>(d_arena.p + hole + off0), nw);
             RSVIO_HIP(hipGetLastError());
         };
-        if (stage_split) stage(L.mask, L.upload);
-        if (early_env)
-            RSVIO_HIP(hipMemcpyAsync(d_arena.p + L.mask, hb + L.mask, L.upload - L.mask, hipMemcpyHostToDevice, stream));
+        const size_t early0 = early_state ? L.pose_init : L.mask;
+        auto stage_early = [&] {
+            if (stage_split) stage(early0, L.upload);
+            if (early_env)
+                RSVIO_HIP(hipMemcpyAsync(d_arena.p + hole + early0, hb + early0, L.upload - early0, hipMemcpyHostToDevice,
+                                         stream));
+        };
+        stage_early();
         mark();
-        auto* lm_base = reinterpret_cast<int*>(hb + L.lm_base);
-        auto* wave_fill = reinterpret_cast<int*>(hb + L.wave_fill);
-        auto* wave_lm = reinterpret_cast<int*>(hb + L.wave_lm);
-        int n_wave = 0, fill = 0;
-        int gl[kGrp] = {0, 0, 0, 0, 0, 0, 0, 0};
-        const bool want_env = n_free > 10;
-        unsigned long long freebits = 0;
-        for (int k = 0; k < n_kf; ++k)
-            if (free_idx[k] >= 0) freebits |= 1ull << (2 * k);
-        int cand[kMaxFree];
-        for (int k = 0; k < kMaxFree; ++k) cand[k] = -1;
-        for (int l = 0; l < n_lm; ++l) {
-            const int ns = slot_count(m2[l]);
-            if (!ns) {
-                lm_base[l] = -1;
-                continue;
-            }
-            if (want_env) {
-                const unsigned long long kb = (m2[l] | (m2[l] >> 1)) & freebits;
-                if (kb) {
-                    const int a = free_idx[__builtin_ctzll(kb) >> 1], b = free_idx[(63 - __builtin_clzll(kb)) >> 1];
-                    cand[a] = std::max(cand[a], b);
-                }
-            }
-            if (n_wave == 0 || fill + ns > 64) {
-                if (n_wave) wave_fill[n_wave - 1] = fill;
-                wave_lm[n_wave] = l;
-                ++n_wave;
-                fill = 0;
-            }
-            lm_base[l] = 64 * (n_wave - 1) + fill;
-            gl[(n_wave - 1) % kGrp] += 1;
-            fill += ns;
-        }
-        if (n_wave) wave_fill[n_wave - 1] = fill;
-        wave_lm[n_wave] = n_lm;
-        int stride = 1;
-        for (int x = 0; x < kGrp; ++x) stride = std::max(stride, gl[x]);
-        n_pad = (size_t)64 * n_wave;
+        if (!packed) {
+            wp.restart();
+            wp.pack(m2, n_lm);
+            const bool moved = close_pack();
+            if (fit_arena() || moved) stage_early();
+        }
         if (coll == 2 && fold_lvl == 2 && n_wave > kP2PWaves)
             throw std::invalid_argument("shard exceeds the folded P2P trial exchange (16384 waves): RSVIO_P2P_FOLD=1");
         mark();
-        L.hdr = off;   off += al(sizeof(int4) * 2 * std::max<size_t>(n_pad, 1));
-        L.uv = off;    off += al(sizeof(double2) * 2 * std::max<size_t>(n_pad, 1));
-        L.pairs = off; off += al(sizeof(int4) * (size_t)n_chunk * stride);
-        L.total = off;
-        if (d_arena.n < L.total) {
-            d_arena.alloc(L.total + L.total / 4);
-            if (stage_split) stage(L.mask, L.upload);
-            if (early_env)
-                RSVIO_HIP(hipMemcpyAsync(d_arena.p + L.mask, hb + L.mask, L.upload - L.mask, hipMemcpyHostToDevice,
-                                         stream));
-        }
+        if (hole != lay.staged) tab_valid = tab_hit = false;
         lay = L;
-        std::memcpy(hb + L.pose_init, pose7, sizeof(double) * 7 * (size_t)n_kf);
-        if (n_lm) std::memcpy(hb + L.pw_init, pW, sizeof(double) * 3 * (size_t)n_lm);
-        std::memcpy(hb + L.free_idx, free_idx.data(), sizeof(int) * (size_t)n_kf);
-        std::memcpy(hb + L.pb_fa, pb_fa.data(), sizeof(int) * (size_t)n_pb);
-        std::memcpy(hb + L.pb_fb, pb_fb.data(), sizeof(int) * (size_t)n_pb);
-        if (n_free <= 10)
-            mf_dense_map(n_free, n_pb, pb_fa.data(), pb_fb.data(), reinterpret_cast<int*>(hb + L.dmap));
-        else
-            mf_dense_map(n_free, n_pb, pb_fa.data(), pb_fb.data(), reinterpret_cast<int*>(hb + L.dmap),
-                         6 * bk_template_nf(n_free), kBkLd);
+        lay.staged = hole;
+        for (size_t* f : {&lay.free_idx, &lay.pb_fa, &lay.pb_fb, &lay.dmap, &lay.desc, &lay.lm_base, &lay.wave_fill,
+                          &lay.wave_lm, &lay.pose_init, &lay.pw_init, &lay.mask, &lay.key, &lay.ouv, &lay.upload,
+                          &lay.total})
+            *f += hole;
+        if (!early_state) copy_state();
+        if (!tab_hit) {
+            std::memcpy(hb + L.free_idx, free_idx.data(), sizeof(int) * (size_t)n_kf);
+            std::memcpy(hb + L.pb_fa, pb_fa.data(), sizeof(int) * (size_t)n_pb);
+            std::memcpy(hb + L.pb_fb, pb_fb.data(), sizeof(int) * (size_t)n_pb);
+            if (n_free <= 10)
+                mf_dense_map(n_free, n_pb, pb_fa.data(), pb_fb.data(), reinterpret_cast<int*>(hb + L.dmap));
+            else
+                mf_dense_map(n_free, n_pb, pb_fa.data(), pb_fb.data(), reinterpret_cast<int*>(hb + L.dmap),
+                             6 * bk_template_nf(n_free), kBkLd);
+        }
         G.n_kf = n_kf; G.n_free = n_free; G.n_lm = n_lm; G.n_obs = n_obs; G.n_slot = (int)n_pad;
         G.n_pb = n_pb; G.n_wave = n_wave; G.n_chunk = n_chunk; G.pair_stride = stride;
-        for (int k = 0, run = -1; k < kMaxFree; ++k) {
-            run = std::max(run, cand[k]);
-            G.env[k] = (unsigned char)(k >= n_free ? k : want_env ? std::max(k, run) : n_free - 1);
-        }
+        wp.envelope(n_free, G.env);
         G.env_on = want_env ? 1 : 0;
         for (int c = 0; c < 2; ++c)
             for (int i = 0; i < 16; ++i) G.TCB[c].m[i] = TCB2[16 * c + i];
@@ -3973,27 +4077,34 @@
         fill_desc(hdesc);
         std::memcpy(hb + L.desc, &hdesc, sizeof(WinDesc));
         mark();
+        const size_t late0 = tab_hit ? L.desc : 0;
         if (stage_kernel) {
-            stage(0, stage_split ? L.mask : L.upload);
+            if (stage_split) {
+                stage(late0, early0);
+            } else {
+                stage(late0, L.upload);
+            }
         } else {
-            RSVIO_HIP(hipMemcpyAsync(d_arena.p, hb, early_env ? L.mask : L.upload, hipMemcpyHostToDevice, stream));
-        }
+            RSVIO_HIP(hipMemcpyAsync(d_arena.p + hole + late0, hb + late0, (early_env ? early0 : L.upload) - late0,
+                                     hipMemcpyHostToDevice, stream));
+        }
+        tab_valid = true;
         up_pending = true;
         {
             SlotSrc S;
-            S.mask = reinterpret_cast<const unsigned long long*>(d_arena.p + L.mask);
-            S.lm_base = reinterpret_cast<const int*>(d_arena.p + L.lm_base);
-            S.wave_fill = reinterpret_cast<const int*>(d_arena.p + L.wave_fill);
-            S.key = reinterpret_cast<const unsigned*>(d_arena.p + L.key);
-            S.uv = reinterpret_cast<const double2*>(d_arena.p + L.ouv);
+            S.mask = reinterpret_cast<const unsigned long long*>(d_arena.p + lay.mask);
+            S.lm_base = reinterpret_cast<const int*>(d_arena.p + lay.lm_base);
+            S.wave_fill = reinterpret_cast<const int*>(d_arena.p + lay.wave_fill);
+            S.key = reinterpret_cast<const unsigned*>(d_arena.p + lay.key);
+            S.uv = reinterpret_cast<const double2*>(d_arena.p + lay.ouv);
             S.uv32 = uv32 ? 1 : 0;
-            S.wave_lm = reinterpret_cast<const int*>(d_arena.p + L.wave_lm);
+            S.wave_lm = reinterpret_cast<const int*>(d_arena.p + lay.wave_lm);
             S.nb_lm = (n_lm + 255) / 256;
             S.nb_pad = (int)((n_pad + 255) / 256);
             const int nb = S.nb_lm + S.nb_pad + (n_obs + 255) / 256;
             hipLaunchKernelGGL(ba_build_layout, dim3(nb + n_chunk), dim3(256), 0, stream, G, prob(), S, nb,
-                               reinterpret_cast<int4*>(d_arena.p + L.hdr), reinterpret_cast<double2*>(d_arena.p + L.uv),
-                               reinterpret_cast<int4*>(d_arena.p + L.pairs));
+                               reinterpret_cast<int4*>(d_arena.p + lay.hdr), reinterpret_cast<double2*>(d_arena.p + lay.uv),
+                               reinterpret_cast<int4*>(d_arena.p + lay.pairs));
             RSVIO_HIP(hipGetLastError());
         }
         mark();
@@ -4009,7 +4120,7 @@
                 fprintf(stderr, "[rsvio] set_problem us: checks+layout %.1f upload wait %.1f observations %.1f waves %.1f "
                         "tables %.1f enqueue %.1f grow %.1f (upload %zu B, arena %zu B); minor faults %ld %ld %ld %ld "
                         "%ld %ld %ld\n",
-                        tms[0], tms[1], tms[2], tms[3], tms[4], tms[5], tms[6], L.upload, L.total, flt[0], flt[1],
+                        tms[0], tms[1], tms[2], tms[3], tms[4], tms[5], tms[6], L.upload, lay.total, flt[0], flt[1],
                         flt[2], flt[3], flt[4], flt[5], flt[6]);
             if (prof_slow && (tot > 1000.0 || ftot > 100)) {
                 std::string maps;
@@ -4062,7 +4173,7 @@
     void enqueue_start(double lambda0) {
         settled = false;
         if (G.n_wave)
-            hipLaunchKernelGGL(ba_linearize, dim3(G.n_wave), dim3(64), 0, stream, G, prob(), work_at(0), lambda0);
+            hipLaunchKernelGGL(ba_linearize, dim3(G.n_wave), dim3(64), 0, stream, prob(), work_at(0), lambda0, G);
         else
             enqueue_reset(lambda0);
         RSVIO_HIP(hipGetLastError());
@@ -4071,8 +4182,8 @@
     void enqueue_linear_system(int it, const LmArgs& la, bool materialise) {
         const Prob pr = prob();
         const Work wk = work(it);
-        hipLaunchKernelGGL(ba_schur_chunks, dim3(G.n_chunk), dim3(kSchurThreads), 0, stream, G, pr, wk, la,
-                           sharded() ? 1 : 0);
+        hipLaunchKernelGGL(ba_schur_chunks, dim3(G.n_chunk), dim3(kSchurThreads), 0, stream, pr, wk, la,
+                           sharded() ? 1 : 0, G);
         RSVIO_HIP(hipGetLastError());
         if (!sharded() && !materialise) {
             if (wide_combine()) {
@@ -4146,8 +4257,8 @@
                 hipLaunchKernelGGL(ba_schur_chunks_p2p, dim3(G.n_chunk), dim3(kSchurThreads), 0, stream, G, pr, wk,
                                    lm_args(cfg), p2p, d_xgen.p, d_p2p_err.p, p2p_fold4() ? 4 : 2);
             else
-                hipLaunchKernelGGL(ba_schur_chunks, dim3(G.n_chunk), dim3(kSchurThreads), 0, stream, G, pr, wk,
-                                   lm_args(cfg), 1);
+                hipLaunchKernelGGL(ba_schur_chunks, dim3(G.n_chunk), dim3(kSchurThreads), 0, stream, pr, wk,
+                                   lm_args(cfg), 1, G);
             RSVIO_HIP(hipGetLastError());
             switch (G.n_free) {
 #define RSVIO_CAMP(NF) \
@@ -4188,7 +4299,7 @@
             RSVIO_HIP(hipGetLastError());
             return;
         }
-        if (G.n_wave) hipLaunchKernelGGL(ba_backsub_relinearize, dim3(G.n_wave), dim3(64), 0, stream, G, pr, wk);
+        if (G.n_wave) hipLaunchKernelGGL(ba_backsub_relinearize, dim3(G.n_wave), dim3(64), 0, stream, pr, wk, G);
         RSVIO_HIP(hipGetLastError());
         if (coll == 2) {
             hipLaunchKernelGGL(ba_p2p_trial, dim3(1), dim3(256), 0, stream, G, pr, wk, p2p, d_xgen.p, d_p2p_err.p);
@@ -4214,7 +4325,9 @@
     }
 
     void enqueue_start_d(double lambda0, int wcap) {
-        hipLaunchKernelGGL(bab_linearize, dim3(wcap, 1), dim3(64), 0, stream, dptr(), lambda0);
+        const Prob pr = prob();
+        hipLaunchKernelGGL(bad_linearize, dim3(wcap, 1), dim3(64), 0, stream, dptr(), cap_slots(), pr.slot_hdr, pr.slot_uv,
+                           lambda0);
         RSVIO_HIP(hipGetLastError());
     }
     void enqueue_iteration_d(const rsvio_lm_cfg& cfg, int it, int wcap) {
@@ -4230,7 +4343,13 @@
             default: throw std::logic_error("descriptor mode: more than 10 free keyframes");
         }
         RSVIO_HIP(hipGetLastError());
-        hipLaunchKernelGGL(bab_backsub_relinearize, dim3(wcap, 1), dim3(64), 0, stream, dptr(), wi);
+        {
+            const Prob pr = prob();
+            const Work wk = work(it);
+            hipLaunchKernelGGL(bad_backsub_relinearize, dim3(wcap, 1), dim3(64), 0, stream, dptr(), wi, cap_slots(),
+                               pr.slot_hdr, pr.slot_uv, static_cast<const double*>(wk.raws[0]),
+                               static_cast<const double*>(wk.raws[1]), static_cast<const LmState*>(wk.st));
+        }
         RSVIO_HIP(hipGetLastError());
     }
     void enqueue_decide_d(const rsvio_lm_cfg& cfg, int it) {
diff --git a/rs-vio_amd/csrc/obs_pass.hpp b/rs-vio_amd/csrc/obs_pass.hpp
--- a/rs-vio_amd/csrc/obs_pass.hpp
+++ b/rs-vio_amd/csrc/obs_pass.hpp
@@ -260,12 +260,101 @@
 #endif
 constexpr int kObsChunk = RSVIO_OBS_CHUNK;
 
+constexpr int kPackGrp = 8;
+constexpr int kPackMaxFree = 20;
+constexpr unsigned long long kPackEven = 0x5555555555555555ull;
+
+struct WavePack {
+    int *lm_base = nullptr, *wave_fill = nullptr, *wave_lm = nullptr;
+    const int* free_idx = nullptr;
+    unsigned long long freebits = 0;
+    bool want_env = false;
+    int n_wave = 0, fill = 0, next_l = 0;
+    int gl[kPackGrp];
+    int cand[kPackMaxFree];
+    long long bits = 0;
+
+    void begin(int* lb, int* wf, int* wl, const int* fidx, int n_kf, bool env) {
+        lm_base = lb; wave_fill = wf; wave_lm = wl; free_idx = fidx; want_env = env;
+        freebits = 0;
+        for (int k = 0; k < n_kf; ++k)
+            if (fidx[k] >= 0) freebits |= 1ull << (2 * k);
+        restart();
+    }
+    void restart() {
+        n_wave = fill = next_l = 0;
+        bits = 0;
+        for (int x = 0; x < kPackGrp; ++x) gl[x] = 0;
+        for (int k = 0; k < kPackMaxFree; ++k) cand[k] = -1;
+    }
+    __attribute__((target("popcnt"))) void pack(const unsigned long long* m2, int l1) {
+        for (int l = next_l; l < l1; ++l) {
+            const unsigned long long m = m2[l];
+            const int ns = __builtin_popcountll((m | (m >> 1)) & kPackEven);
+            if (!ns) {
+                lm_base[l] = -1;
+                continue;
+            }
+            bits += __builtin_popcountll(m);
+            if (want_env) {
+                const unsigned long long kb = (m | (m >> 1)) & freebits;
+                if (kb) {
+                    const int a = free_idx[__builtin_ctzll(kb) >> 1], b = free_idx[(63 - __builtin_clzll(kb)) >> 1];
+                    cand[a] = std::max(cand[a], b);
+                }
+            }
+            if (n_wave == 0 || fill + ns > 64) {
+                if (n_wave) wave_fill[n_wave - 1] = fill;
+                wave_lm[n_wave] = l;
+                ++n_wave;
+                fill = 0;
+            }
+            lm_base[l] = 64 * (n_wave - 1) + fill;
+            gl[(n_wave - 1) % kPackGrp] += 1;
+            fill += ns;
+        }
+        next_l = std::max(next_l, l1);
+    }
+    int finish(int n_lm) {
+        if (n_wave) wave_fill[n_wave - 1] = fill;
+        wave_lm[n_wave] = n_lm;
+        int stride = 1;
+        for (int x = 0; x < kPackGrp; ++x) stride = std::max(stride, gl[x]);
+        return stride;
+    }
+    void envelope(int n_free, unsigned char* env) const {
+        for (int k = 0, run = -1; k < kPackMaxFree; ++k) {
+            run = std::max(run, cand[k]);
+            env[k] = (unsigned char)(k >= n_free ? k : want_env ? std::max(k, run) : n_free - 1);
+        }
+    }
+};
+
 static bool observation_pass(int n_obs, const int32_t* lm, const int32_t* kf, const uint8_t* cam,
                              const double* uv, int n_lm, int n_kf, unsigned* key, unsigned long long* m2,
-                             float* uv32, bool* narrowed) {
+                             float* uv32, bool* narrowed, WavePack* wp = nullptr, bool* packed = nullptr) {
+    if (packed) *packed = false;
     if (n_lm <= 0 || n_kf <= 0) return false;
     HostPool* pool = n_obs >= 2 * kObsChunk ? shared_pool() : nullptr;
     std::memset(m2, 0, sizeof(unsigned long long) * (size_t)n_lm);
+    if (wp && packed && !pool) {
+        *narrowed = uv32 && uv_narrow(2 * (size_t)n_obs, uv, uv32);
+        for (int a = 0; a < n_obs;) {
+            int b = a + kObsChunk < n_obs ? a + kObsChunk : n_obs;
+            while (b < n_obs && lm[b] == lm[b - 1]) ++b;
+            if (!obs_keys(b - a, lm + a, kf + a, cam + a, n_lm, n_kf, key + a)) return false;
+            masks_of_runs(a, b, key, m2);
+            const int bound = b < n_obs ? lm[b] : n_lm;
+            if (bound > wp->next_l && bound <= n_lm) wp->pack(m2, bound);
+            a = b;
+        }
+        wp->pack(m2, n_lm);
+        if (wp->bits == n_obs) {
+            *packed = true;
+            return true;
+        }
+        return mask_bits(n_lm, m2) == n_obs;
+    }
     if (pool) {
         const int nc = std::min((n_obs + kObsChunk - 1) / kObsChunk, 0xffff);
         int cut_s[64];
```

After: 5013, median of 6. About the same (+2.5%).
